# mpieva/mapping-iterative-assembler

Hardware: AMD Instinct MI355X
Metric: reads aligned/sec per iteration (16.5kb mito ref, 100bp reads) (higher is better)
Workload: dtype int32; 1 GPU; configs[1]: 1000000 synthetic 100 bp reads per GPU vs mt311 (16619 bp, circular), matrix flat; step = reiterate_assembly + pop_smp + cull + consensus; pass-1 coordinates = true positions; reads_per_gpu=1000000, total_reads=1000000, consensus_len=16619, bytes_per_read=182

## Files before the change

### mapping-iterative-assembler_amd/csrc/align_route.h

```cpp
#pragma once
#include <stdint.h>

namespace mia {

constexpr int ROUTE_QCH = 8, ROUTE_MAXW = 64;

struct AlignRouteIn {
  int64_t n = 0;
  int max_len = 0, wrap = 0, L = 0;
  int64_t plane_words = 0;
  int64_t kh_entries = 0;
  bool flat = false, ref_mostly_bases = true, ref_few_n = true, bx_ok = false, explicit_win = false, deferred = false, pend_encode = false;
  bool own_umax = false;
  int64_t rejects = 0;
  int use_filter = 1, use_banddp = 1, use_bx = 1, use_lanes = 1, use_fine = 1, use_quick = 1;
  bool bx_serial = false, plan_split = true, use_direct_open = true, no_prep_fuse = false;
  uint32_t ext_events = 31u, dbg = 0, bx_dbg = 0;
};

struct AlignRoute {
  int64_t plane_words = 0;
  int nwords = 0;
  bool bx = false, run_filter = false, fused_prep = false, filtered = false, kocc = false, banded = false;
  bool want_bits = false, new_flow = false, split = false, fork_by_launch = false, fine = false;
  bool many_rejects = false;
  bool planner_head_first = false, direct_open = false;
  int maxw = 0;
  bool quick = false, quick_lds = false, one_launch = false, fork_at_quick = false;
  int qch = 4;
  int quick_phase = 0;
  int full_first = 0, full_last = 0;
  int grid_cap = 0;
  bool three_streams = false, two_streams = false;
  bool values_aside = false;
  bool trace_signals = false;
  bool planner_aside = false;
  bool use_plain = false;
  bool plan_count_late = false;
};

inline unsigned align_route_plan_grid(const AlignRoute& r, int phase, int64_t n) {
  const int64_t g = (n + 255) / 256, cap = (phase == 2 || phase == 3) ? 1024 : r.grid_cap;
  return (unsigned)(cap && g > cap ? cap : g);
}

inline AlignRoute align_route(const AlignRouteIn& in) {
  AlignRoute r;
  const int64_t n = in.n;
  r.nwords = (in.max_len + 63) >> 6;
  r.plane_words = in.plane_words;
  const bool filter_ok = in.flat && in.use_filter && in.ref_mostly_bases;
  r.bx = in.bx_ok && in.use_bx && (in.ref_mostly_bases || in.kh_entries > 0) && in.wrap <= (1 << 22) && !(in.dbg & 128u);
  r.run_filter = filter_ok && !r.bx;
  r.fused_prep = in.pend_encode && r.bx && !in.no_prep_fuse;
  r.filtered = r.run_filter || r.bx;
  r.kocc = r.filtered && in.wrap <= (1 << 22) && !r.bx;
  r.banded = r.bx || (r.filtered && in.use_banddp && r.kocc && !(in.dbg & 128u));
  const bool many = !in.ref_mostly_bases || in.rejects * 20 > n;
  r.many_rejects = r.bx && many;
  r.use_plain = !r.banded || r.many_rejects;
  r.plan_count_late = true;
  if (!r.bx) return r;

  r.want_bits = in.use_quick && (in.kh_entries <= 0 || in.ref_few_n);
  r.new_flow = in.use_lanes && !in.bx_serial && !(in.dbg & 256u) && !in.explicit_win;
  r.split = in.plan_split;
  r.fork_by_launch = (in.ext_events & 1u) && r.new_flow;
  r.fine = r.split && in.use_fine && (in.use_fine > 1 || !in.flat || n >= 4000000 || many);
  r.planner_head_first = r.new_flow && in.deferred && many;
  r.direct_open = r.new_flow && in.deferred && in.use_direct_open && !many && !(in.bx_dbg & (4u | 8u));
  r.maxw = (in.use_lanes && (r.fine || in.use_fine >= 2)) ? ROUTE_MAXW : 32;
  r.quick = r.split && r.new_flow && r.want_bits && !(in.bx_dbg & 32u) && in.own_umax &&
            (!r.fine || n >= 2000000 || in.use_quick > 1);
  r.fork_at_quick = r.quick && r.direct_open && !r.fine;
  r.quick_lds = r.quick && r.plane_words * 24 <= 38 * 1024;
  r.quick_phase = r.quick ? (r.quick_lds ? 5 : 4) : 0;
  r.qch = (r.quick && n >= 4000000 && r.plane_words * 24 <= 16 * 1024) ? ROUTE_QCH : 4;
  r.one_launch = r.quick && !r.fine;
  r.full_first = r.one_launch ? 6 : r.split ? 1 : 0;
  r.full_last = r.one_launch ? 6 : r.split ? (r.fine ? 3 : 2) : 0;
  r.grid_cap = r.one_launch ? 256 : 0;
  r.three_streams = r.new_flow;
  r.two_streams = !r.new_flow && !(in.dbg & 256u);
  r.values_aside = r.three_streams && !(in.deferred && !r.fork_at_quick);
  r.trace_signals = r.three_streams && (in.ext_events & 2u) && !(in.bx_dbg & 8u);
  r.planner_aside = r.three_streams && in.deferred;
  r.plan_count_late = !r.planner_head_first && !r.direct_open;
  return r;
}

}
```

### mapping-iterative-assembler_amd/csrc/mia_hip.hip

```cpp
#include <hip/hip_runtime.h>
#include <atomic>
#include <hip/hip_ext.h>
#include <stdio.h>
#include <stdlib.h>
#include <string.h>

#include <algorithm>
#include <cmath>
#include <chrono>
#include <optional>
#include <string>
#include <thread>
#include <tuple>
#include <vector>

#include "../../include/mia_hip.h"
#include "dev_buf.h"
#include "dev_pool.h"
#include "mia_comm.h"
#include "mia_consensus_kernels.h"
#include "mia_kernels.h"
#include "bandx_kernels.h"
#include "align_route.h"
#include "pass1_route.h"
#include "mia_pass1_kernels.h"
#include "mia_myers_kernels.h"
#include "mia_trim_kernels.h"
#include "mia_peak_kernels.h"
#include "mia_iter_kernels.h"
#include "mia_ma_region_kernels.h"
#include "mia_ma_ace_kernels.h"
#include "mia_ma_sam_kernels.h"
#include "mia_ma_profile_kernels.h"
#include "mia_ma_ends_kernels.h"
#include "mia_ma_cols_kernels.h"
#include "mia_ma_dedup_kernels.h"
#include "mia_ma_damage_kernels.h"
#include "mia_ma_mask_kernels.h"

using namespace mia;

enum Stage { STG_TRACE = 0, STG_PLAIN, STG_FILTER, STG_BAND, STG_BX_PLAN, STG_BX_VALUES, STG_BX_TRACE, STG_TALLY, STG_PASS1, STG_MA_SELECT, STG_MA_RENDER, STG_MA_ACE_LAYOUT, STG_MA_ACE_RENDER, STG_MA_MASK_BOUNDS, STG_MA_MASK_LAYOUT, STG_MA_MASK_APPLY, STG_MA_SAM_LAYOUT, STG_MA_SAM_RENDER, STG_MA_DAMAGE_HITS, STG_MA_DAMAGE_MOLECULES, STG_MA_PROFILE, STG_MA_DEDUP_KEYS, STG_MA_DEDUP_SORT, STG_MA_DEDUP_RUNS, STG_MA_DEDUP_NEXT, STG_MA_DEDUP_ANCHORS, STG_MA_DEDUP_CLUSTERS, STG_MA_TALLY, STG_MA_COLS, STG_MA_ENDS, STG_COUNT };
static const char* const STAGE_NAMES[STG_COUNT] = {"k_align_quad", "k_align_quad_plain", "k_diag_filter", "k_band_align", "k_bx_plan",
                                                   "k_bx_values", "k_bx_trace", "k_tally_binned", "k_pass1", "k_ma_region_select",
                                                   "k_ma_region_render", "k_ma_ace_layout", "k_ma_ace_render", "k_ma_mask_bounds", "k_ma_mask_layout", "k_ma_mask_apply", "k_ma_sam_layout",
                                                   "k_ma_sam_render", "k_ma_damage_hits", "k_ma_damage_molecules", "k_ma_profile", "k_ma_dedup_keys", "k_ma_dedup_sort", "k_ma_dedup_runs",
                                                   "k_ma_dedup_next", "k_ma_dedup_anchors", "k_ma_dedup_clusters", "k_ma_tally", "k_ma_cols", "k_ma_ends"};

constexpr int OPEN_WGS = 1024;
constexpr int64_t OPEN_SLAB_BYTES = (int64_t)MAX_READ * 64 * 12;
constexpr int CTRL_BINS = 0;
constexpr int CTRL_HDR = (3 * N_BINS + 2 + 1) & ~1;
constexpr int CTRL_FILTER = CTRL_HDR + PH_WORDS;
constexpr int CTRL_LKN = CTRL_FILTER + 4, CTRL_CULLF = CTRL_LKN + 1, CTRL_NEV = CTRL_CULLF + 1, CTRL_TFLAGS = CTRL_NEV + 1;
constexpr int CTRL_GENN = CTRL_TFLAGS + 2;
constexpr int CTRL_BXC = (CTRL_GENN + 1 + 63) & ~63;
constexpr int CTRL_WORDS = CTRL_BXC + BXC_WORDS;
constexpr int CTRL_C0 = CTRL_BINS + 3 * N_BINS, CTRL_CN = CTRL_WORDS - CTRL_C0;

#ifdef MIA_HIP_ALT_PATHS
static inline const char* alt_env(const char* name) { return getenv(name); }
#define ALT_KERNEL(k) ((const void*)(k))
#else
static inline const char* alt_env(const char*) { return nullptr; }
#define ALT_KERNEL(k) ((const void*)nullptr)
#endif
static inline std::optional<int> alt_int(const char* name) {
  const char* v = alt_env(name);
  return v ? std::optional<int>(atoi(v)) : std::nullopt;
}

struct mia_hip_ctx {
  int device = 0;
  int cus = 1;
  std::string err;
  DevPool pool;
  unsigned char* h_pin = nullptr; static constexpr size_t PIN_BYTES = 1 << 20, PIN_MISC = 64 << 10;
  DevBuf<int32_t> d_ctrl;
  uint32_t dbg = 0;

  hipStream_t stream = nullptr;
  hipStream_t stream2 = nullptr; hipEvent_t ev_fork = nullptr, ev_join = nullptr;
  hipStream_t stream3 = nullptr; hipEvent_t ev_join3 = nullptr;
  uint32_t ext_events = 31u; bool align_end_signalled = false;
  bool spin_wait = true;
  uint32_t stage_mask = ~0u;
  struct StageTimer { std::vector<std::pair<hipEvent_t, hipEvent_t>> pending; double ms = 0; int64_t launches = 0; };
  StageTimer stg[STG_COUNT];
  std::vector<std::pair<hipEvent_t, hipEvent_t>> ev_free;

  DevBuf<int32_t> d_pssm;
  int max_abs = 0;
  int max_pos = 0;
  bool have_pssm = false;
  bool flat = false;
  PackSet packs;
  ReadSet rs{};
  DevBuf<uint8_t> d_packed; DevBuf<uint32_t> d_roff; DevBuf<uint16_t> d_len;
  DevBuf<uint8_t> d_rc, d_sk;
  DevBuf<int32_t> d_as, d_ae, d_score, d_refstart;
  DevBuf<int16_t> d_abr; DevBuf<uint32_t> d_status; DevBuf<int16_t> d_cols;
  int max_len = 0;
  int min_len = 0;
  std::vector<int32_t> h_len;
  DevBuf<uint64_t> d_rplanes; int rplane_words = 0;
  DevBuf<int32_t> d_umax; bool umax_valid = false;
  DevBuf<uint8_t> d_ref; int L = 0, wrap = 0; int explicit_win = 0; bool have_ref = false; bool aligned = false;
  bool ref_mostly_bases = true;
  bool ref_few_n = true;
  int64_t kh_entries = 0;

  DevBuf<int32_t> d_bin_of, d_list, d_wide_list, d_retry_list;
  int32_t* d_bins = nullptr;
  int32_t* d_plan_hdr = nullptr;
  bool deferred = false;
  DevBuf<unsigned char> d_slabs[N_CPL];
  DevBuf<unsigned char> d_slabs_retry[3];
  DevBuf<unsigned char> d_quad_slabs;
  int quad_wgs = 0;
  int grid_wgs = 0;
  int window_wgs[N_CPL] = {0, 0, 0};
  int64_t plain_retried = 0, plain_total = 0;
  bool wide_to_caller = false;
  DevBuf<int32_t> d_scratch; DevBuf<int64_t> d_scratch_off;
  DevBuf<int32_t> d_open_list; DevBuf<unsigned char> d_slabs_open; bool use_direct_open = true; int64_t direct_open_steps = 0;

  int use_filter = 1;
  DevBuf<int32_t> d_kocc_cnt, d_kocc_pos;
  DevBuf<uint64_t> d_planes;
  uint32_t* d_filter_n = nullptr; int64_t filter_proven = 0, filter_seen = 0;
  int use_banddp = 1;
  DevBuf<int32_t> d_left_list;
  DevBuf<uint32_t> d_band_slabs;
  int64_t band_done = 0;

  bool bx_ok = false;
  int use_bx = 1, use_lanes = 1; bool bx_serial = false; uint32_t bx_dbg = 0;
  DevBuf<int32_t> d_bx_sub, d_bx_mrow; DevBuf<int16_t> d_bx_loss, d_bx_dl;
  int32_t bx_min_m = 0, bx_max_m = 0;
  DevBuf<uint32_t> d_refnib;
  DevBuf<uint32_t> d_khash; DevBuf<int32_t> d_khash_ovf;
  DevBuf<KbPair> d_kbits;
  int use_quick = 1; int64_t quick_steps = 0;
  DevBuf<uint32_t> d_prep_bar; uint32_t prep_bar_count = 0; bool no_prep_fuse = false;
  DevBuf<uint32_t> d_bx_plan; DevBuf<int32_t> d_bx_expect, d_bx_lists;
  DevBuf<BxCandRec> d_bx_cand; bool plan_split = true;
  DevBuf<BxCandRec> d_bx_cand2; int use_fine = 1;
  uint32_t* d_bx_ctr = nullptr;
  DevBuf<uint32_t> d_bx_slabs;
  int bx_values_wgs = 0, bx_trace_wgs = 0;
  DevBuf<uint32_t> d_bx_slabs_late; int bx_late_wgs = 0;
  DevBuf<uint32_t> d_bx_slabs_late2;
  DevBuf<int32_t> d_retry2;
  bool diag_scripts_missing = false;
  int64_t bx_seen = 0, bx_done[3] = {0, 0, 0};
  int64_t bx_launches = 0;
  uint32_t bx_last[BXC_COUNTERS] = {0};

  DevBuf<int64_t> d_slot, d_partial, d_total;
  DevBuf<uint8_t> d_slot_dropped, d_drop_f, d_drop_b; int64_t n_slots = 0;
  DevBuf<int64_t> d_back_slot;
  DevBuf<int64_t> d_front_slot0;
  DevBuf<int32_t> d_link_act;
  RecInfo ri{};
  DevBuf<int32_t> d_ri_flen, d_ri_blen, d_ri_actf, d_ri_trec;
  SlotInfo si{};
  DevBuf<int32_t> d_si_reclen, d_si_recact, d_si_mult; DevBuf<unsigned long long> d_si_writer;
  Links lk{};
  DevBuf<int64_t> d_lk_rec;
  int64_t* d_links_all = nullptr; int32_t n_links_all = 0;
  int32_t* d_n_links_all = nullptr; int64_t links_cap_all = 0; DevBuf<int32_t> d_n_links_gathered;
  DevBuf<int32_t> d_link_len;
  uint32_t* d_cull_flags = nullptr;
  DevBuf<uint32_t> d_cull_sync;
  DevBuf<unsigned long long> d_sums;
  int64_t read_base = 0;
  int64_t slot_base = 0;
  bool culled = false, links_applied = false;
  std::vector<DevBuf<int64_t>> owned_links;
  bool cull_scan = false, tail_scans = false;
  bool cull_with_records = true;
  int64_t pre_cull_records = 0, pre_cull_links = 0; bool pre_cull_valid = false;

  TallyBuf tb{}; DevBuf<int32_t> d_tb_tally, d_ins_off, d_ins_total; DevBuf<uint64_t> d_tb_events;
  DevBuf<int32_t> d_ins_tally; DevBuf<char> d_calls, d_ins_calls;
  int64_t ins_tally_cap = 0;
  int32_t n_events_host = 0; bool tallied = false;
  int64_t ins_total_host = 0;
  bool consensus_done = false;
  bool fake_event_overflow = false;
  bool no_linear_tally = false, sort2_unpacked = false;
  bool tally_linear = false;
  int tally_pk_bias = -1;
  int use_binned_tally = 1;
  DevBuf<int32_t> d_bucket, d_order;
  int bucket_clean_nb = -1;
  int buckets_queued = 0;
  bool no_side_buckets = false;
  DevBuf<int32_t> d_tally_slabs;
  DevBuf<int32_t> d_gen_list;
  bool tally_defer = true;
  bool tally_strand_split = true;
  bool tally_rall = true;
  bool tally_runs = true;
  DevBuf<int32_t> d_order2; DevBuf<uint8_t> d_okey; DevBuf<int32_t> d_sort2;

  bool in_iterate = false;
  const int32_t* abort_if = nullptr;
  bool spec_ok = false, spec_pending = false, spec_filtered = false, spec_bx = false, spec_plain = false;
  int64_t spec_redone = 0;
  bool no_spec = false;
  bool spec_force = false; DevBuf<int32_t> d_one;
  bool pend_encode = false; int32_t pend_L = 0, pend_wl = 0, pend_total = 0;
  bool zero_copy = true;
  const double* dev_cut = nullptr; DevBuf<double> d_cut_buf;
  DevBuf<char> d_ascii; const char* ascii_src = nullptr;
  DevBuf<char> d_cons;
  DevBuf<int32_t> d_cons_pos;
  unsigned char* h_pin2 = nullptr; size_t pin2_bytes = 0;
  int64_t iter_fallbacks = 0;

  double pass1_ms = 0; int64_t pass1_filtered = 0, pass1_anchored = 0;
  double myers_kernel_ms = 0; bool myers_no_lanes = false, myers_no_ond = false;
  int64_t trim_escapes = 0;
  int64_t trim_launches = 0, trim_scratch_bytes = 0;
  bool trim_exact = false;
  bool ma_resident = false; int64_t ma_n = 0, ma_n_ins = 0; int32_t ma_L = 0;
  DevBuf<int32_t> d_ma_start, d_ma_gaps, d_ma_ipos, d_ma_rec_ins, d_ma_ins_list;
  DevBuf<int64_t> d_ma_coff, d_ma_ioff, d_ma_colmap, d_ma_rows;
  DevBuf<char> d_ma_seq, d_ma_ib, d_ma_text;
  DevBuf<unsigned long long> d_ma_ctl;
  struct MaOut {
    bool region_done = false, ace_done = false, sam_done = false, prof_done = false, ends_done = false, cols_done = false, damage_done = false, mask_done = false;
    int32_t first = 0, last = -1; int64_t rows = 0, width = 0, ace_bytes = 0, sam_bytes = 0;
  } ma_out;
  bool ma_ace_gaps_ok = false, ma_ace_cols_ok = false;
  DevBuf<int64_t> d_ace_g, d_ace_af, d_ace_len, d_ace_off; DevBuf<char> d_ace_body;
  bool ma_sam_gaps_ok = false;
  DevBuf<char> d_sam_ref, d_sam_body; DevBuf<int64_t> d_sam_cum, d_sam_cig, d_sam_off; DevBuf<int32_t> d_sam_nm;
  DevBuf<unsigned long long> d_sam_ctl;
  DevBuf<uint8_t> d_ma_rev, d_prof_use; DevBuf<char> d_ma_smp, d_prof_ref; DevBuf<unsigned long long> d_prof_bins;
  int64_t ma_cols = 0; int64_t ma_prof_bins[MA_PROF_BINS] = {0};
  DevBuf<uint8_t> d_ends_seg; DevBuf<unsigned long long> d_ends_bins;
  int64_t ma_ends_bins[MA_ENDS_BINS] = {0};
  DevBuf<uint32_t> d_cols_tab; DevBuf<unsigned long long> d_cols_out;
  std::vector<int32_t> ma_cols_tab;
  struct MaDedup {
    bool done = false; int64_t n = 0, molecules = 0, clusters = 0, orphans = 0;
    DevBuf<int32_t> d_start, d_end, d_score; DevBuf<uint8_t> d_rc, d_keep; DevBuf<int64_t> d_mate, d_rep;
    DevBuf<unsigned long long> d_key[2], d_runkey, d_best, d_ctl, d_hist;
    DevBuf<uint32_t> d_val[2], d_jump[2], d_counts, d_runid, d_first, d_mark, d_cluster, d_anchor;
    int64_t hist[MA_DEDUP_HIST] = {0};
  } dedup;

  struct MaDamage {
    DevBuf<int64_t> d_mate; DevBuf<uint32_t> d_hit; DevBuf<uint8_t> d_pos, d_keep; DevBuf<unsigned long long> d_bins;
    int64_t bins[MA_DMG_BINS] = {0};
  } damage;

  struct MaMask {
    DevBuf<uint32_t> d_lohi; DevBuf<int32_t> d_rec, d_ipos; DevBuf<int64_t> d_off; DevBuf<char> d_seq, d_smp; DevBuf<uint8_t> d_pair_keep;
    DevBuf<unsigned long long> d_ctl, d_bins;
    int64_t bins[MA_MASK_BINS] = {0}, cols_kept = 0; int32_t mode = 0;
  } mask;

  mia_hip_collectives coll{}; bool comm = false; int comm_ranks = 1, comm_rank = 0; std::string coll_name;
  DevBuf<unsigned long long> d_gather;
  std::vector<int64_t> h_gather;
  int64_t ev_pad = 0;
  DevBuf<int64_t> d_lstage, d_lmine, d_lall;
  DevBuf<int32_t> d_scores_all;
};

static void read_alt_switches(mia_hip_ctx* ctx) {
  auto on = [](const char* name) { const char* v = alt_env(name); return v && atoi(v) != 0; };
  if (on("MIA_HIP_NO_DIAG_FILTER")) { ctx->use_filter = 0; ctx->use_bx = 0; }
  if (on("MIA_HIP_NO_BAND_DP")) { ctx->use_banddp = 0; ctx->use_bx = 0; }
  if (on("MIA_HIP_NO_BANDX")) ctx->use_bx = 0;
  if (on("MIA_HIP_NO_LANES")) ctx->use_lanes = 0;
  if (on("MIA_HIP_BX_SERIAL")) ctx->bx_serial = true;
  if (on("MIA_HIP_NO_PLAN_SPLIT")) ctx->plan_split = false;
  if (on("MIA_HIP_NO_FINE")) ctx->use_fine = 0;
  if (const char* v = alt_env("MIA_HIP_FINE")) ctx->use_fine = atoi(v);
  if (on("MIA_HIP_NO_QUICK_PLAN")) ctx->use_quick = 0;
  if (const char* v = alt_env("MIA_HIP_QUICK_PLAN")) ctx->use_quick = atoi(v);
  if (on("MIA_HIP_NO_DIRECT_OPEN")) ctx->use_direct_open = false;
  if (on("MIA_HIP_NO_PREP_FUSE")) ctx->no_prep_fuse = true;
  if (on("MIA_HIP_NO_SPEC")) ctx->no_spec = true;
  if (on("MIA_HIP_SPEC_TEST")) ctx->spec_force = true;
  if (on("MIA_HIP_NO_SIDE_BUCKETS")) ctx->no_side_buckets = true;
  if (on("MIA_HIP_NO_ZERO_COPY")) ctx->zero_copy = false;
  if (on("MIA_HIP_NO_EXT_EVENTS")) ctx->ext_events = 0u;
  if (on("MIA_HIP_FAKE_EVENT_OVERFLOW")) ctx->fake_event_overflow = true;
  if (on("MIA_HIP_CULL_SCAN")) ctx->cull_scan = true;
  if (on("MIA_HIP_TAIL_SCANS")) ctx->tail_scans = true;
  if (on("MIA_HIP_NO_CULL_RECORDS")) ctx->cull_with_records = false;
  if (on("MIA_HIP_NO_BINNED_TALLY")) ctx->use_binned_tally = 0;
  if (on("MIA_HIP_NO_LINEAR_TALLY")) ctx->no_linear_tally = true;
  if (on("MIA_HIP_SORT2_UNPACKED")) ctx->sort2_unpacked = true;
  if (on("MIA_HIP_TALLY_INLINE")) ctx->tally_defer = false;
  if (const char* v = alt_env("MIA_HIP_STRAND_SPLIT")) ctx->tally_strand_split = atoi(v) != 0;
  if (on("MIA_HIP_NO_TALLY_RUNS")) ctx->tally_runs = false;
  if (on("MIA_HIP_NO_TALLY_RALL")) ctx->tally_rall = false;
  if (on("MIA_HIP_MYERS_NO_LANES")) ctx->myers_no_lanes = true;
  if (on("MIA_HIP_MYERS_NO_OND")) ctx->myers_no_ond = true;
  if (on("MIA_HIP_TRIM_EXACT")) ctx->trim_exact = true;
  if (const char* v = alt_env("MIA_HIP_DEBUG_SKIP")) ctx->dbg = (uint32_t)atoi(v);
  if (const char* v = alt_env("MIA_HIP_BX_DEBUG")) ctx->bx_dbg = (uint32_t)atoi(v);
}

#define HIPCHK(call)                                                                                   \
  do {                                                                                                 \
    hipError_t e_ = (call);                                                                            \
    if (e_ != hipSuccess) {                                                                            \
      ctx->err = std::string(#call) + ": " + hipGetErrorString(e_);                                    \
      return MIA_HIP_ERR_DEVICE;                                                                       \
    }                                                                                                  \
  } while (0)

static int dev_nomem(mia_hip_ctx* ctx, hipError_t e) {
  if (e == hipSuccess) return MIA_HIP_OK;
  ctx->err = std::string("hipMalloc: ") + hipGetErrorString(e);
  return MIA_HIP_ERR_NOMEM;
}
template <class T>
static int dev_alloc(mia_hip_ctx* ctx, DevBuf<T>& b, int64_t n) { return dev_nomem(ctx, b.alloc(n)); }
template <class T>
static int dev_ensure(mia_hip_ctx* ctx, DevBuf<T>& b, int64_t need, int64_t alloc_elems) { return dev_nomem(ctx, b.ensure(need, alloc_elems)); }
template <class T>
static int dev_ensure(mia_hip_ctx* ctx, DevBuf<T>& b, int64_t need) { return dev_nomem(ctx, b.ensure(need, need)); }

template <class T>
static int pool_take(mia_hip_ctx* ctx, PoolLease<T>& lease, size_t n) { return dev_nomem(ctx, lease.take(ctx->pool, n)); }

extern "C" const char* mia_hip_last_error(const mia_hip_ctx* ctx) { return ctx ? ctx->err.c_str() : "null context"; }

extern "C" int mia_hip_create(mia_hip_ctx** out, int device_index) {
  if (!out) return MIA_HIP_ERR_ARG;
  *out = nullptr;
  int ndev = 0;
  if (hipGetDeviceCount(&ndev) != hipSuccess || ndev <= 0) return MIA_HIP_ERR_DEVICE;
  if (device_index < 0 || device_index >= ndev) return MIA_HIP_ERR_ARG;
  mia_hip_ctx* ctx = new mia_hip_ctx();
  ctx->device = device_index;
  const unsigned evf = hipEventDisableTiming;
  if (hipSetDevice(device_index) != hipSuccess || hipStreamCreateWithFlags(&ctx->stream, hipStreamNonBlocking) != hipSuccess ||
      hipStreamCreateWithFlags(&ctx->stream2, hipStreamNonBlocking) != hipSuccess || hipStreamCreateWithFlags(&ctx->stream3, hipStreamNonBlocking) != hipSuccess ||
      hipEventCreateWithFlags(&ctx->ev_join3, evf) != hipSuccess ||
      hipEventCreateWithFlags(&ctx->ev_fork, evf) != hipSuccess || hipEventCreateWithFlags(&ctx->ev_join, evf) != hipSuccess) {
    delete ctx;
    return MIA_HIP_ERR_DEVICE;
  }
  {
    hipDeviceProp_t prop;
    if (hipGetDeviceProperties(&prop, device_index) != hipSuccess) { delete ctx; return MIA_HIP_ERR_DEVICE; }
    ctx->cus = prop.multiProcessorCount > 0 ? prop.multiProcessorCount : 1;
    ctx->grid_wgs = prop.multiProcessorCount * 32;
    ctx->quad_wgs = prop.multiProcessorCount * 16;
    read_alt_switches(ctx);
    if (const char* sw = getenv("MIA_HIP_SPIN_WAIT")) ctx->spin_wait = atoi(sw) != 0;
  }
  if (dev_alloc(ctx, ctx->d_pssm, 2 * PSSM_WORDS) || dev_alloc(ctx, ctx->d_ctrl, CTRL_WORDS) ||
      dev_alloc(ctx, ctx->d_total, 1) || dev_alloc(ctx, ctx->d_ins_total, 1) ||
      dev_alloc(ctx, ctx->d_bx_sub, 2 * BX_SUB_WORDS) || dev_alloc(ctx, ctx->d_bx_mrow, 2 * 31 * 4) || dev_alloc(ctx, ctx->d_bx_loss, BX_LOSS_WORDS) ||
      dev_alloc(ctx, ctx->d_bx_dl, BX_DL_WORDS) ||
      dev_alloc(ctx, ctx->d_cut_buf, 2)) {
    delete ctx;
    return MIA_HIP_ERR_NOMEM;
  }
  ctx->d_bins = ctx->d_ctrl + CTRL_BINS;
  ctx->d_plan_hdr = ctx->d_ctrl + CTRL_HDR;
  ctx->d_filter_n = reinterpret_cast<uint32_t*>(ctx->d_ctrl + CTRL_FILTER);
  ctx->lk.n = ctx->d_ctrl + CTRL_LKN;
  ctx->d_cull_flags = reinterpret_cast<uint32_t*>(ctx->d_ctrl + CTRL_CULLF);
  ctx->tb.n_events = ctx->d_ctrl + CTRL_NEV;
  ctx->tb.flags = reinterpret_cast<uint32_t*>(ctx->d_ctrl + CTRL_TFLAGS);
  ctx->d_bx_ctr = reinterpret_cast<uint32_t*>(ctx->d_ctrl + CTRL_BXC);
  if (hipMemset(ctx->d_ctrl, 0, CTRL_WORDS * 4) != hipSuccess) { delete ctx; return MIA_HIP_ERR_DEVICE; }
  {
    const int32_t one = 1;
    if (dev_alloc(ctx, ctx->d_one, 1) || hipMemcpy(ctx->d_one, &one, 4, hipMemcpyHostToDevice) != hipSuccess) { delete ctx; return MIA_HIP_ERR_DEVICE; }
    if (dev_alloc(ctx, ctx->d_prep_bar, 1) || hipMemset(ctx->d_prep_bar, 0, 4) != hipSuccess) { delete ctx; return MIA_HIP_ERR_DEVICE; }
  }
  if (hipHostMalloc((void**)&ctx->h_pin, mia_hip_ctx::PIN_BYTES, hipHostMallocDefault) != hipSuccess) ctx->h_pin = nullptr;
  if (ctx->h_pin) memset(ctx->h_pin, 0, mia_hip_ctx::PIN_MISC);
  else ctx->no_prep_fuse = true;
  *out = ctx;
  return MIA_HIP_OK;
}

extern "C" int mia_hip_comm_destroy(mia_hip_ctx* ctx);
extern "C" void mia_hip_destroy(mia_hip_ctx* ctx) {
  if (!ctx) return;
  (void)hipSetDevice(ctx->device);
  (void)hipStreamSynchronize(ctx->stream);
  (void)mia_hip_comm_destroy(ctx);
  if (ctx->h_pin) (void)hipHostFree(ctx->h_pin);
  if (ctx->h_pin2) (void)hipHostFree(ctx->h_pin2);
  for (auto& e : ctx->ev_free) { (void)hipEventDestroy(e.first); (void)hipEventDestroy(e.second); }
  for (auto& t : ctx->stg) for (auto& e : t.pending) { (void)hipEventDestroy(e.first); (void)hipEventDestroy(e.second); }
  (void)hipStreamDestroy(ctx->stream);
  if (ctx->stream2) (void)hipStreamDestroy(ctx->stream2);
  if (ctx->stream3) (void)hipStreamDestroy(ctx->stream3);
  if (ctx->ev_join3) (void)hipEventDestroy(ctx->ev_join3);
  if (ctx->ev_fork) (void)hipEventDestroy(ctx->ev_fork);
  if (ctx->ev_join) (void)hipEventDestroy(ctx->ev_join);
  delete ctx;
}

extern "C" int mia_hip_sync(mia_hip_ctx* ctx) {
  if (!ctx) return MIA_HIP_ERR_ARG;
  HIPCHK(hipSetDevice(ctx->device));
  HIPCHK(hipStreamSynchronize(ctx->stream));
  return MIA_HIP_OK;
}

extern "C" int mia_hip_set_pssm(mia_hip_ctx* ctx, const int32_t* fwd, const int32_t* rc) {
  if (!ctx || !fwd || !rc) return MIA_HIP_ERR_ARG;
  HIPCHK(hipSetDevice(ctx->device));
  int m = 0;
  for (int i = 0; i < PSSM_WORDS; i++) {
    int a = fwd[i] < 0 ? -fwd[i] : fwd[i], b = rc[i] < 0 ? -rc[i] : rc[i];
    if (a > m) m = a;
    if (b > m) m = b;
  }
  if (m > 32000) { ctx->err = "PSSM entries beyond +-32000 do not fit the int16 substitution table"; return MIA_HIP_ERR_RANGE; }
  ctx->max_abs = m;
  {
    int lo = 0, hi = 0;
    for (int k = 0; k < PSSM_WORDS; k++) { lo = std::min(lo, std::min((int)fwd[k], (int)rc[k])); hi = std::max(hi, std::max((int)fwd[k], (int)rc[k])); }
    ctx->tally_pk_bias = -lo + hi <= 2047 ? -lo : -1;
  }
  ctx->max_pos = 0;
  for (int i = 0; i < PSSM_WORDS; i++) { if (fwd[i] > ctx->max_pos) ctx->max_pos = fwd[i]; if (rc[i] > ctx->max_pos) ctx->max_pos = rc[i]; }
  const int cpls[N_CPL] = {4, 8, 12};
  for (int c = 0; c < N_CPL; c++) ctx->packs.ok[c] = make_pack_params(64 * cpls[c], m, &ctx->packs.p[c]) ? 1 : 0;
  HIPCHK(hipMemcpyAsync(ctx->d_pssm, fwd, PSSM_WORDS * 4, hipMemcpyHostToDevice, ctx->stream));
  HIPCHK(hipMemcpyAsync(ctx->d_pssm + PSSM_WORDS, rc, PSSM_WORDS * 4, hipMemcpyHostToDevice, ctx->stream));
  HIPCHK(hipStreamSynchronize(ctx->stream));
  ctx->have_pssm = true;
  ctx->flat = pssm_is_flat(fwd, rc);
  ctx->tally_linear = true;
  for (int d = 0; d < 2 * PSSM_DEPTH + 1; d++)
    for (int x = 0; x < 4; x++)
      for (int b = 0; b < 5; b++)
        if (fwd[(d * 5 + x) * 5 + b] != fwd[x * 5 + b] || rc[(d * 5 + x) * 5 + b] != fwd[x * 5 + b]) ctx->tally_linear = false;
  if (ctx->no_linear_tally) ctx->tally_linear = false;
  {
    std::vector<int32_t> sub(2 * BX_SUB_WORDS, 0), mrow(2 * 31 * 4, 0);
    std::vector<int16_t> loss(BX_LOSS_WORDS, 0), dl(BX_DL_WORDS, 0);
    ctx->bx_ok = bx_make_tables(fwd, rc, sub.data(), mrow.data(), loss.data(), dl.data(), &ctx->bx_min_m, &ctx->bx_max_m);
    if (ctx->bx_ok) {
      for (int k = 0; k < BX_SUB_WORDS; k++) sub[(size_t)BX_SUB_WORDS + k] = sub[(size_t)k] * 256;
      HIPCHK(hipMemcpyAsync(ctx->d_bx_sub, sub.data(), sub.size() * 4, hipMemcpyHostToDevice, ctx->stream));
      HIPCHK(hipMemcpyAsync(ctx->d_bx_mrow, mrow.data(), mrow.size() * 4, hipMemcpyHostToDevice, ctx->stream));
      HIPCHK(hipMemcpyAsync(ctx->d_bx_loss, loss.data(), loss.size() * 2, hipMemcpyHostToDevice, ctx->stream));
      HIPCHK(hipMemcpyAsync(ctx->d_bx_dl, dl.data(), dl.size() * 2, hipMemcpyHostToDevice, ctx->stream));
      HIPCHK(hipStreamSynchronize(ctx->stream));
    }
    ctx->umax_valid = false;
    if (ctx->bx_ok && ctx->d_umax && ctx->rs.n > 0) {
      hipLaunchKernelGGL(k_bx_umax, dim3((unsigned)((ctx->rs.n + 255) / 256)), dim3(256), 0, ctx->stream, ctx->rs, ctx->d_bx_mrow, ctx->d_umax);
      HIPCHK(hipGetLastError());
      ctx->umax_valid = true;
    }
  }
  return MIA_HIP_OK;
}

static inline uint8_t base_code(char b) {
  switch (b) { case 'A': return 0; case 'C': return 1; case 'G': return 2; case 'T': return 3; default: return 4; }
}

static void pack_reads(int64_t n, const char* bases, const int64_t* offsets, const uint32_t* roff, const uint16_t* len, uint8_t* packed) {
  uint8_t lut[256];
  for (int c = 0; c < 256; c++) lut[c] = base_code((char)c);
  auto range = [&](int64_t lo, int64_t hi) {
    for (int64_t i = lo; i < hi; i++) {
      const unsigned char* s = reinterpret_cast<const unsigned char*>(bases) + offsets[i];
      uint8_t* d = packed + roff[i];
      const int l = len[i];
      int k = 0;
      for (; k + 1 < l; k += 2) d[k >> 1] = (uint8_t)(lut[s[k]] | (lut[s[k + 1]] << 4));
      if (k < l) d[k >> 1] = lut[s[k]];
    }
  };
  int T = (int)std::thread::hardware_concurrency();
  if (const char* e = getenv("MIA_HIP_THREADS")) T = atoi(e);
  T = std::max(1, std::min(std::min(T, 32), (int)(n / 16384) + 1));
  if (T == 1) { range(0, n); return; }
  std::vector<std::thread> th;
  for (int t = 1; t < T; t++) th.emplace_back(range, n * t / T, n * (t + 1) / T);
  range(0, n / T);
  for (auto& x : th) x.join();
}

extern "C" int mia_hip_upload_reads(mia_hip_ctx* ctx, int64_t n, const char* bases, const int64_t* offsets, const uint8_t* rc,
                                    const uint8_t* strand_known, const int32_t* as, const int32_t* ae) {
  if (!ctx || n < 0 || (n > 0 && (!bases || !offsets || !rc || !strand_known || !as || !ae))) return MIA_HIP_ERR_ARG;
  if (n >= (int64_t)1 << 31) { ctx->err = "more than 2^31 reads per context"; return MIA_HIP_ERR_ARG; }
  HIPCHK(hipSetDevice(ctx->device));
  std::vector<uint32_t> roff((size_t)n);
  std::vector<uint16_t> len((size_t)n);
  uint64_t total = 0;
  int max_len = 1;
  for (int64_t i = 0; i < n; i++) {
    int64_t l = offsets[i + 1] - offsets[i];
    if (l < 1 || l > MIA_HIP_MAX_READ) { ctx->err = "read length outside 1..256 (INIT_ALN_SEQ_LEN)"; return MIA_HIP_ERR_ARG; }
    roff[i] = (uint32_t)total;
    len[i] = (uint16_t)l;
    if (l > max_len) max_len = (int)l;
    total += (uint64_t)(((l + 1) / 2 + 3) & ~3);
    if (total >= ((uint64_t)1 << 32)) { ctx->err = "packed read store exceeds 4 GiB per context"; return MIA_HIP_ERR_ARG; }
  }
  std::vector<uint8_t> packed((size_t)total + 8, 0);
  pack_reads(n, bases, offsets, roff.data(), len.data(), packed.data());
  ctx->max_len = max_len;
  ctx->min_len = max_len;
  ctx->h_len.assign(len.begin(), len.end());
  for (int64_t i = 0; i < n; i++) if ((int)len[(size_t)i] < ctx->min_len) ctx->min_len = len[(size_t)i];
  const int stride = (max_len + 3) & ~3;
  int nomem = 0;
  nomem |= dev_alloc(ctx, ctx->d_packed, packed.size());
  nomem |= dev_alloc(ctx, ctx->d_roff, n);
  nomem |= dev_alloc(ctx, ctx->d_len, n);
  nomem |= dev_alloc(ctx, ctx->d_rc, n);
  nomem |= dev_alloc(ctx, ctx->d_sk, n);
  nomem |= dev_alloc(ctx, ctx->d_as, n);
  nomem |= dev_alloc(ctx, ctx->d_ae, n);
  nomem |= dev_alloc(ctx, ctx->d_score, n);
  nomem |= dev_alloc(ctx, ctx->d_refstart, n);
  nomem |= dev_alloc(ctx, ctx->d_abr, n);
  nomem |= dev_alloc(ctx, ctx->d_status, n);
  nomem |= dev_alloc(ctx, ctx->d_cols, n * stride);
  nomem |= dev_alloc(ctx, ctx->d_bin_of, n);
  nomem |= dev_alloc(ctx, ctx->d_umax, n);
  ctx->rplane_words = (max_len + 63) >> 6;
  nomem |= dev_alloc(ctx, ctx->d_rplanes, n * 2 * ctx->rplane_words + 2);
  nomem |= dev_alloc(ctx, ctx->d_list, n + 4 * N_BINS);
  nomem |= dev_alloc(ctx, ctx->d_wide_list, n);
  nomem |= dev_alloc(ctx, ctx->d_retry_list, n);
  nomem |= dev_alloc(ctx, ctx->d_slot, n);
  nomem |= dev_alloc(ctx, ctx->d_partial, (size_t)(n / 256 + n / 4096 + 8));
  nomem |= dev_alloc(ctx, ctx->d_drop_f, n);
  nomem |= dev_alloc(ctx, ctx->d_drop_b, n);
  nomem |= dev_alloc(ctx, ctx->d_slot_dropped, 2 * n + 16);
  ctx->n_slots = ctx->d_slot_dropped.cap;
  nomem |= dev_alloc(ctx, ctx->d_back_slot, n) | dev_alloc(ctx, ctx->d_front_slot0, n);
  nomem |= dev_alloc(ctx, ctx->d_ri_flen, n) | dev_alloc(ctx, ctx->d_ri_blen, n) | dev_alloc(ctx, ctx->d_ri_actf, n) |
         dev_alloc(ctx, ctx->d_ri_trec, n * 16);
  const int64_t slot_cap = 2 * n + 16;
  nomem |= dev_alloc(ctx, ctx->d_si_reclen, slot_cap) | dev_alloc(ctx, ctx->d_si_recact, slot_cap) | dev_alloc(ctx, ctx->d_si_writer, slot_cap) |
         dev_alloc(ctx, ctx->d_si_mult, slot_cap);
  ctx->lk.cap = (int32_t)std::min<int64_t>(n + 16, (int64_t)1 << 20);
  if (ctx->lk.cap > (int32_t)LINK_NONE - 1) ctx->lk.cap = (int32_t)LINK_NONE - 1;
  nomem |= dev_alloc(ctx, ctx->d_lk_rec, (size_t)ctx->lk.cap * 4);
  ctx->ri.flen = ctx->d_ri_flen; ctx->ri.blen = ctx->d_ri_blen; ctx->ri.actf = ctx->d_ri_actf; ctx->ri.trec = ctx->d_ri_trec;
// ... 196 lines not shown
  if (plain_launches) *plain_launches = ctx->stg[STG_PLAIN].launches;
  if (reads_in) *reads_in = ctx->plain_total;
  if (reads_retried) *reads_retried = ctx->plain_retried;
  if (reset) { ctx->stg[STG_PLAIN].ms = 0; ctx->stg[STG_PLAIN].launches = 0; ctx->plain_total = 0; ctx->plain_retried = 0; }
  return MIA_HIP_OK;
}

template <int CPL>
static hipError_t launch_window(mia_hip_ctx* ctx, int ci, const int32_t* list, int count, const int32_t* dev_range = nullptr, hipStream_t on = nullptr,
                                bool own_slabs = false, hipEvent_t stop = nullptr) {
  const int64_t slab = (int64_t)MAX_READ * 64 * CPL;
  if (!ctx->window_wgs[ci]) {
    int occ = 0;
    const int cus = ctx->cus;
    if (hipOccupancyMaxActiveBlocksPerMultiprocessor(&occ, (const void*)k_align_window<CPL>, 64, 0) != hipSuccess || occ < 1) occ = 1;
    const int per_cu = ctx->grid_wgs / cus;
    ctx->window_wgs[ci] = cus * (occ < per_cu ? occ : per_cu);
  }
  int grid = (dev_range || count >= ctx->window_wgs[ci]) ? ctx->window_wgs[ci] : count;
  unsigned char* slabs = nullptr;
  if (own_slabs) {
    grid = std::min(grid, 1024);
    if (!ctx->d_slabs_retry[ci] && dev_alloc(ctx, ctx->d_slabs_retry[ci], slab * 1024)) return hipErrorOutOfMemory;
    slabs = ctx->d_slabs_retry[ci];
  } else {
    if (!ctx->d_slabs[ci] && dev_alloc(ctx, ctx->d_slabs[ci], slab * ctx->grid_wgs)) return hipErrorOutOfMemory;
    slabs = ctx->d_slabs[ci];
  }
  RefInfo ref{ctx->d_ref, ctx->L, ctx->wrap, ctx->explicit_win};
  if (stage_begin(ctx, STG_TRACE, on)) return hipErrorOutOfMemory;
  launch_k(k_align_window<CPL>, dim3(grid), dim3(64), 0, on ? on : ctx->stream, stop, ctx->rs, ref, ctx->d_pssm, ctx->packs.p[ci], list,
           count, slabs, slab, ctx->d_wide_list, ctx->d_bins + 3 * N_BINS, ctx->dbg, dev_range);
  stage_end(ctx, STG_TRACE, on);
  return hipGetLastError();
}

static hipError_t launch_window_class(mia_hip_ctx* ctx, int ci, const int32_t* list, int count, const int32_t* dev_range = nullptr, hipStream_t on = nullptr,
                                      bool own_slabs = false, hipEvent_t stop = nullptr) {
  return ci == 0 ? launch_window<4>(ctx, ci, list, count, dev_range, on, own_slabs, stop)
       : ci == 1 ? launch_window<8>(ctx, ci, list, count, dev_range, on, own_slabs, stop)
                 : launch_window<12>(ctx, ci, list, count, dev_range, on, own_slabs, stop);
}

static int align_all(mia_hip_ctx* ctx);
static bool tally_is_binned(const mia_hip_ctx* ctx);
static int comm_pre_cull_enqueue(mia_hip_ctx* ctx, const int32_t* d_wide_count);
static bool comm_pre_cull_collect(mia_hip_ctx* ctx);

extern "C" int mia_hip_realign(mia_hip_ctx* ctx, const char* new_ref, int32_t ref_len, int circular) {
  if (!ctx || !new_ref || ref_len <= 0) return MIA_HIP_ERR_ARG;
  if (!ctx->have_pssm || !ctx->d_packed) { ctx->err = "set_pssm and upload_reads must precede realign"; return MIA_HIP_ERR_STATE; }
  HIPCHK(hipSetDevice(ctx->device));
  const int L = ref_len, wl = circular ? (L < MAX_READ ? L : MAX_READ) : 0, wrap = L + wl;
  std::vector<uint8_t> codes((size_t)wrap + 64, 4);
  int64_t n_other = 0;
  for (int i = 0; i < L; i++) { codes[i] = base_code(new_ref[i]); n_other += codes[i] > 3; }
  for (int i = 0; i < wl; i++) codes[L + i] = codes[i];
  ctx->ref_mostly_bases = n_other * 50 <= L;
  ctx->ref_few_n = n_other * 500 <= L;
  ctx->kh_entries = 0;
  if (n_other) {
    ctx->kh_entries = kh_wild_entries(codes.data(), wrap, BX_WILD);
    if (ctx->kh_entries > ((int64_t)1 << 24)) ctx->kh_entries = 0;
  }
  if (dev_ensure(ctx, ctx->d_ref, (int64_t)codes.size(), (int64_t)codes.size() * 2)) return MIA_HIP_ERR_NOMEM;
  if (ctx->h_pin && codes.size() <= mia_hip_ctx::PIN_BYTES - mia_hip_ctx::PIN_MISC) {
    HIPCHK(hipStreamSynchronize(ctx->stream));
    memcpy(ctx->h_pin + mia_hip_ctx::PIN_MISC, codes.data(), codes.size());
    HIPCHK(hipMemcpyAsync(ctx->d_ref, ctx->h_pin + mia_hip_ctx::PIN_MISC, codes.size(), hipMemcpyHostToDevice, ctx->stream));
  } else {
    HIPCHK(hipMemcpyAsync(ctx->d_ref, codes.data(), codes.size(), hipMemcpyHostToDevice, ctx->stream));
  }
  ctx->L = L; ctx->wrap = wrap; ctx->have_ref = true; ctx->explicit_win = 0;
  return align_all(ctx);
}

static int run_wide(mia_hip_ctx* ctx, const RefInfo& ref, int32_t n_wide) {
    if (ctx->wide_to_caller) {
      hipLaunchKernelGGL(k_mark_status, dim3((n_wide + 255) / 256), dim3(256), 0, ctx->stream, ctx->d_wide_list, n_wide, ctx->rs.status, ST_ESCAPE);
      HIPCHK(hipGetLastError());
      return MIA_HIP_OK;
    }
    std::vector<int32_t> wl((size_t)n_wide), as((size_t)n_wide), ae((size_t)n_wide);
    std::vector<uint16_t> ln((size_t)n_wide);
    HIPCHK(hipMemcpy(wl.data(), ctx->d_wide_list, (size_t)n_wide * 4, hipMemcpyDeviceToHost));
    std::vector<int64_t> soff((size_t)n_wide);
    int64_t total = 0;
    for (int t = 0; t < n_wide; t++) {
      HIPCHK(hipMemcpy(&as[t], ctx->rs.as + wl[t], 4, hipMemcpyDeviceToHost));
      HIPCHK(hipMemcpy(&ae[t], ctx->rs.ae + wl[t], 4, hipMemcpyDeviceToHost));
      HIPCHK(hipMemcpy(&ln[t], ctx->rs.len + wl[t], 2, hipMemcpyDeviceToHost));
      int s, n1;
      read_window(ref, as[t], ae[t], ln[t], &s, &n1);
      soff[t] = total;
      total += (int64_t)ln[t] * n1 + 5 * (int64_t)n1 + 16;
    }
    if (dev_ensure(ctx, ctx->d_scratch, total) || dev_ensure(ctx, ctx->d_scratch_off, n_wide)) return MIA_HIP_ERR_NOMEM;
    HIPCHK(hipMemcpyAsync(ctx->d_scratch_off, soff.data(), (size_t)n_wide * 8, hipMemcpyHostToDevice, ctx->stream));
    hipLaunchKernelGGL(k_align_wide, dim3((n_wide + 63) / 64), dim3(64), 0, ctx->stream, ctx->rs, ref, ctx->d_pssm, ctx->d_wide_list,
                       n_wide, ctx->d_scratch_off, ctx->d_scratch);
    HIPCHK(hipGetLastError());
    HIPCHK(hipStreamSynchronize(ctx->stream));
  return MIA_HIP_OK;
}

static void encode_now(mia_hip_ctx* ctx) {
  if (!ctx->pend_encode) return;
  ctx->pend_encode = false;
  hipLaunchKernelGGL(k_ref_encode, dim3((unsigned)((ctx->pend_total + 255) / 256)), dim3(256), 0, ctx->stream, ctx->ascii_src, ctx->pend_L, ctx->pend_wl,
                     ctx->d_ref, ctx->pend_total);
}

static void align_counters_collect(mia_hip_ctx* ctx, const int32_t* hb, bool filtered, bool bx, bool plain) {
  constexpr int C0 = CTRL_C0;
  const int32_t* h_hdr = hb + (CTRL_HDR - C0);
  const uint32_t* h_filter = reinterpret_cast<const uint32_t*>(hb + (CTRL_FILTER - C0));
  const uint32_t* h_bxc = reinterpret_cast<const uint32_t*>(hb + (CTRL_BXC - C0));
  ctx->filter_seen += ctx->rs.n;
  if (filtered) {
    ctx->filter_proven += h_filter[0];
    ctx->band_done += h_filter[2];
    if (bx) {
      ctx->filter_proven += h_bxc[BXC_DONE_PLAN * BXC_STRIDE];
      for (int k = 0; k < 3; k++) ctx->bx_done[k] += h_bxc[(BXC_DONE_PLAN + k) * BXC_STRIDE];
      ctx->bx_seen += h_bxc[BXC_SEEN * BXC_STRIDE];
    }
  }
  for (int k = 0; k < BXC_COUNTERS; k++) ctx->bx_last[k] = bx ? h_bxc[k * BXC_STRIDE] : 0;
  if (bx) ctx->bx_last[BXC_CUR_VALUES] = h_filter[1];
  if (plain) ctx->plain_retried += h_hdr[PH_RETRIED_PLAIN];
}

static_assert(ROUTE_QCH == BX_QCH && ROUTE_MAXW == BX_MAXW, "align_route.h carries copies of the two");
static_assert(P1_ROUTE_WILD == BX_WILD, "pass1_route.h carries a copy");

struct AlignCall {
  AlignRoute r;
  RefInfo ref; RefPlanes rp{nullptr, nullptr, nullptr}; KmerOcc ko{nullptr, nullptr}; KmerHash kh{};
  uint32_t kslots = 0; int64_t nib_words = 0;
  BxDev bd; int64_t slab_words = 0;
  int gb = 0;
  int32_t *d_count, *d_off, *d_cursor, *d_wide_count;
  hipStream_t ps = nullptr;
  bool pending_join = false;
  bool planner_end_signalled = false;
  bool dbg_steps = false;
};

static AlignRouteIn align_route_in(const mia_hip_ctx* ctx) {
  AlignRouteIn in;
  in.n = ctx->rs.n; in.max_len = ctx->max_len; in.wrap = ctx->wrap; in.L = ctx->L; in.kh_entries = ctx->kh_entries;
  in.plane_words = plane_words((int64_t)ctx->wrap + 64);
  in.flat = ctx->flat; in.ref_mostly_bases = ctx->ref_mostly_bases; in.ref_few_n = ctx->ref_few_n; in.bx_ok = ctx->bx_ok;
  in.explicit_win = ctx->explicit_win != 0; in.deferred = ctx->deferred; in.pend_encode = ctx->pend_encode;
  in.own_umax = ctx->umax_valid && ctx->rs.roff == ctx->d_roff;
  for (int k = 1; k < BXF_KINDS; k++) in.rejects += ctx->bx_last[BXC_FAIL0 + k];
  in.use_filter = ctx->use_filter; in.use_banddp = ctx->use_banddp; in.use_bx = ctx->use_bx; in.use_lanes = ctx->use_lanes;
  in.use_fine = ctx->use_fine; in.use_quick = ctx->use_quick; in.bx_serial = ctx->bx_serial; in.plan_split = ctx->plan_split;
  in.use_direct_open = ctx->use_direct_open; in.no_prep_fuse = ctx->no_prep_fuse;
  in.ext_events = ctx->ext_events; in.dbg = ctx->dbg; in.bx_dbg = ctx->bx_dbg;
  return in;
}

static void align_ck(mia_hip_ctx* ctx, const AlignCall& c, const char* what) {
  if (!c.dbg_steps) return;
  hipError_t e = hipStreamSynchronize(c.ps);
  fprintf(stderr, "[align_all deferred] %s: %s\n", what, hipGetErrorString(e)); fflush(stderr);
}

static int align_ensure_buffers(mia_hip_ctx* ctx, AlignCall& c) {
  const AlignRoute& r = c.r;
  const int64_t n = ctx->rs.n;
  const int wrap = ctx->wrap;
  if (!r.filtered) return MIA_HIP_OK;
  if (dev_ensure(ctx, ctx->d_planes, r.plane_words * 3)) return MIA_HIP_ERR_NOMEM;
  if (r.kocc && !ctx->d_kocc_cnt && (dev_alloc(ctx, ctx->d_kocc_cnt, DF_KTAB) || dev_alloc(ctx, ctx->d_kocc_pos, (int64_t)DF_KTAB * DF_KCAP)))
    return MIA_HIP_ERR_NOMEM;
  if (((r.run_filter && r.banded) || r.quick) && dev_ensure(ctx, ctx->d_left_list, n)) return MIA_HIP_ERR_NOMEM;
  if (!r.bx) {
    c.slab_words = (int64_t)ctx->max_len * BAND_ROW_WORDS;
    const int64_t words = c.slab_words * std::min<int64_t>((n + 63) / 64, 3072);
    return r.banded ? dev_ensure(ctx, ctx->d_band_slabs, words) : MIA_HIP_OK;
  }
  c.nib_words = bx_nib_words((int64_t)wrap + 64);
  if (dev_ensure(ctx, ctx->d_refnib, c.nib_words, c.nib_words * 2)) return MIA_HIP_ERR_NOMEM;
  c.kslots = kh_slots_for_entries(wrap, ctx->kh_entries);
  if (dev_ensure(ctx, ctx->d_khash, (int64_t)c.kslots * 4) || dev_ensure(ctx, ctx->d_khash_ovf, (int64_t)c.kslots * 2)) return MIA_HIP_ERR_NOMEM;
  if (r.want_bits && !ctx->d_kbits && dev_alloc(ctx, ctx->d_kbits, KB_WORDS)) return MIA_HIP_ERR_NOMEM;
  if (dev_ensure(ctx, ctx->d_bx_plan, n) || dev_ensure(ctx, ctx->d_bx_expect, n) || dev_ensure(ctx, ctx->d_bx_lists, n * 4 * BX_NCLS)) return MIA_HIP_ERR_NOMEM;
  if (!ctx->bx_values_wgs) {
    int occ = 0;
    if (hipOccupancyMaxActiveBlocksPerMultiprocessor(&occ, ctx->use_lanes ? (const void*)k_bxl_values : ALT_KERNEL(k_bx_values), 256, 0) != hipSuccess || occ < 1) occ = 1;
    ctx->bx_values_wgs = ctx->cus * std::min(occ, 4);
    if (hipOccupancyMaxActiveBlocksPerMultiprocessor(&occ, ctx->use_lanes ? (const void*)k_bxl_trace : ALT_KERNEL(k_bx_trace), 256, 0) != hipSuccess || occ < 1) occ = 1;
    ctx->bx_trace_wgs = ctx->cus * std::min(occ, 4);
  }
  c.slab_words = ctx->use_lanes ? (int64_t)((ctx->max_len + 3) & ~3) * BXL_SLAB_ROW_WORDS : (int64_t)ctx->max_len * BX_SLAB_ROW_WORDS;
  const int64_t trace_words = c.slab_words * ctx->bx_trace_wgs * 4;
  if (dev_ensure(ctx, ctx->d_bx_slabs, trace_words)) return MIA_HIP_ERR_NOMEM;
  if (r.new_flow) {
    if (dev_ensure(ctx, ctx->d_retry2, n)) return MIA_HIP_ERR_NOMEM;
    if (!ctx->bx_late_wgs) ctx->bx_late_wgs = ctx->cus;
    const int64_t late_words = (int64_t)((ctx->max_len + 3) & ~3) * BXL_SLAB_ROW_WORDS * ctx->bx_late_wgs * 4;
    if (dev_ensure(ctx, ctx->d_bx_slabs_late, late_words) || dev_ensure(ctx, ctx->d_bx_slabs_late2, late_words)) return MIA_HIP_ERR_NOMEM;
  }
  if (r.split && dev_ensure(ctx, ctx->d_bx_cand, n)) return MIA_HIP_ERR_NOMEM;
  if (r.fine && dev_ensure(ctx, ctx->d_bx_cand2, n)) return MIA_HIP_ERR_NOMEM;
  if (r.direct_open) {
    if (dev_ensure(ctx, ctx->d_open_list, n)) return MIA_HIP_ERR_NOMEM;
    if (!ctx->d_slabs_open && dev_alloc(ctx, ctx->d_slabs_open, OPEN_SLAB_BYTES * OPEN_WGS)) return MIA_HIP_ERR_NOMEM;
  }
  return MIA_HIP_OK;
}

static int align_ref_prep(mia_hip_ctx* ctx, AlignCall& c) {
  const AlignRoute& r = c.r;
  const int wrap = ctx->wrap;
  const int64_t words = r.plane_words, pstride = ctx->d_planes.cap / 3;
  if (!r.fused_prep) {
    encode_now(ctx);
    HIPCHK(hipMemsetAsync(ctx->d_ctrl, 0, (size_t)CTRL_WORDS * 4, ctx->stream));
  }
  if (!r.filtered) return MIA_HIP_OK;
  c.rp = RefPlanes{ctx->d_planes, ctx->d_planes + pstride, ctx->d_planes + 2 * pstride};
  if (!r.fused_prep)
    hipLaunchKernelGGL(k_ref_planes, dim3((unsigned)((words + 3) / 4 < 4096 ? (words + 3) / 4 : 4096)), dim3(256), 0, ctx->stream, ctx->d_ref, (int64_t)wrap + 64, words,
                       ctx->d_planes, ctx->d_planes + pstride, ctx->d_planes + 2 * pstride);
  if (r.kocc) {
    HIPCHK(hipMemsetAsync(ctx->d_kocc_cnt, 0, (size_t)DF_KTAB * 4, ctx->stream));
    hipLaunchKernelGGL(k_kmer_occ, dim3((unsigned)((wrap + 255) / 256)), dim3(256), 0, ctx->stream, ctx->d_ref, (int64_t)wrap, ctx->d_kocc_cnt, ctx->d_kocc_pos, 0);
    c.ko.cnt = ctx->d_kocc_cnt; c.ko.pos = ctx->d_kocc_pos;
  }
  if (!r.bx) return MIA_HIP_OK;
  const int64_t nw = c.nib_words;
  const uint32_t kslots = c.kslots;
  if (!r.fused_prep)
    hipLaunchKernelGGL(k_ref_nibbles, dim3((unsigned)((nw + 255) / 256)), dim3(256), 0, ctx->stream, ctx->d_ref, (int64_t)wrap, nw, ctx->d_refnib);
  c.kh = KmerHash{ctx->d_khash, ctx->d_khash_ovf, kslots - 1, kh_shift_for(kslots), ctx->kh_entries > 0 ? BX_WILD : 0};
  const KmerHash& kh = c.kh;
  if (!r.fused_prep) {
    HIPCHK(hipMemsetAsync(ctx->d_khash, 0xFF, (size_t)kslots * 16, ctx->stream));
    hipLaunchKernelGGL(k_kmer_hash, dim3((unsigned)((wrap + 255) / 256)), dim3(256), 0, ctx->stream, ctx->d_ref, (int64_t)wrap, ctx->d_khash, ctx->d_khash_ovf,
                       kh.mask, kh.shift, kh.wild);
    if (r.want_bits) {
      HIPCHK(hipMemsetAsync(ctx->d_kbits, 0, (size_t)KB_WORDS * sizeof(KbPair), ctx->stream));
      hipLaunchKernelGGL(k_kmer_bits, dim3((unsigned)((ctx->L + 255) / 256)), dim3(256), 0, ctx->stream, ctx->d_ref, (int64_t)wrap, (int64_t)ctx->L, ctx->d_kbits);
    }
    return MIA_HIP_OK;
  }
  RefPrep rp2;
  rp2.ascii = ctx->ascii_src; rp2.L = ctx->pend_L; rp2.wl = ctx->pend_wl; rp2.total = ctx->pend_total; rp2.codes = ctx->d_ref;
  rp2.ctrl = ctx->d_ctrl; rp2.ctrl_words = CTRL_WORDS;
  rp2.kslot = ctx->d_khash; rp2.kovf = ctx->d_khash_ovf; rp2.kslots = kslots; rp2.kmask = kh.mask; rp2.kshift = kh.shift; rp2.kwild = kh.wild;
  rp2.plane_words = words; rp2.plo = ctx->d_planes; rp2.phi = ctx->d_planes + pstride; rp2.pok = ctx->d_planes + 2 * pstride;
  rp2.nib_words = nw; rp2.nib = ctx->d_refnib;
  const int64_t want = ((int64_t)wrap + (kh.wild > 0 ? 63 : 255)) / (kh.wild > 0 ? 64 : 256);
  const unsigned grid = (unsigned)std::max<int64_t>(1, std::min<int64_t>(want, ctx->cus));
  rp2.bar = ctx->d_prep_bar; rp2.bar_target = ctx->prep_bar_count + grid;
  rp2.stuck = ctx->h_pin ? reinterpret_cast<uint32_t*>(ctx->h_pin + (62 << 10)) : nullptr;
  rp2.kbits = r.want_bits ? ctx->d_kbits : nullptr;
  hipLaunchKernelGGL(k_ref_prep, dim3(grid), dim3(256), 0, ctx->stream, rp2);
  HIPCHK(hipGetLastError());
  ctx->prep_bar_count += grid;
  ctx->pend_encode = false;
  return MIA_HIP_OK;
}

static void align_bx_dev(mia_hip_ctx* ctx, AlignCall& c) {
  const AlignRoute& r = c.r;
  BxDev& bd = c.bd;
  bd.tab.sub = ctx->d_bx_sub; bd.tab.mrow = ctx->d_bx_mrow; bd.tab.loss = ctx->d_bx_loss; bd.tab.dl = ctx->d_bx_dl;
  bd.dbg = ctx->bx_dbg & (3u | 32u | 64u | 128u | 512u);
  bd.retry = ctx->d_retry2; bd.retry_n = ctx->d_plan_hdr + PH_RETRY2 + 1;
  bd.listed_mark = r.new_flow ? -5 : 0;
  bd.tab.min_m = ctx->bx_min_m; bd.tab.max_m = ctx->bx_max_m;
  bd.tab.maxw = r.maxw;
  bd.sub256 = ctx->d_bx_sub + BX_SUB_WORDS;
  bd.refnib = ctx->d_refnib;
  bd.umax = (ctx->umax_valid && ctx->rs.roff == ctx->d_roff) ? ctx->d_umax : nullptr;
  bd.rplanes = bd.umax ? ctx->d_rplanes : nullptr;
  bd.rplane_words = ctx->rplane_words;
  bd.plan = ctx->d_bx_plan; bd.expect = ctx->d_bx_expect; bd.lists = ctx->d_bx_lists; bd.list_stride = ctx->d_bx_lists.cap / (4 * BX_NCLS); bd.ctr = ctx->d_bx_ctr;
  bd.cand = r.split ? ctx->d_bx_cand : nullptr; bd.cand_n = ctx->d_bx_ctr + (size_t)BXC_CAND * BXC_STRIDE;
  bd.cand2 = r.fine ? ctx->d_bx_cand2 : nullptr; bd.cand2_n = ctx->d_bx_ctr + (size_t)BXC_CAND2 * BXC_STRIDE;
  bd.open = r.direct_open ? ctx->d_open_list : nullptr; bd.open_n = ctx->d_bx_ctr + (size_t)BXC_OPEN * BXC_STRIDE;
  bd.qlist = r.quick ? ctx->d_left_list : nullptr; bd.qlist_n = ctx->d_filter_n + 1; bd.mark_all = 0; bd.to_late = 0; bd.qch = r.qch;
  bd.kb = KmerBits{r.quick ? ctx->d_kbits : nullptr, ctx->L};
  bd.plane_words = (int32_t)(r.quick_lds ? r.plane_words : 0);
}

using PlanKernel = decltype(&k_bx_plan<1, 0>);
template <int PH>
static PlanKernel plan_kernel_nw(int nwords) {
  switch (nwords) { case 1: return k_bx_plan<1, PH>; case 2: return k_bx_plan<2, PH>; case 3: return k_bx_plan<3, PH>; default: return k_bx_plan<4, PH>; }
}
static PlanKernel plan_kernel(int nwords, int phase) {
  switch (phase) {
    case 0: return plan_kernel_nw<0>(nwords); case 1: return plan_kernel_nw<1>(nwords); case 2: return plan_kernel_nw<2>(nwords); case 3: return plan_kernel_nw<3>(nwords);
    case 4: return plan_kernel_nw<4>(nwords); case 5: return plan_kernel_nw<5>(nwords); default: return plan_kernel_nw<6>(nwords);
  }
}

static int align_plan_launches(mia_hip_ctx* ctx, AlignCall& c) {
  const AlignRoute& r = c.r;
  const int64_t n = ctx->rs.n, wrap = ctx->wrap;
  BxDev& bd = c.bd;
  const dim3 pb(256);
  const uint32_t* in_n = (const uint32_t*)(ctx->d_filter_n + 1);
  ctx->diag_scripts_missing = true;
  if (r.direct_open) ctx->direct_open_steps++;
  if (r.quick) ctx->quick_steps++;
  if (stage_begin(ctx, STG_BX_PLAN)) return MIA_HIP_ERR_NOMEM;
  if (r.quick) {
    const dim3 pg((unsigned)((n + 256 * bd.qch - 1) / (256 * bd.qch)));
    const size_t lds = (size_t)(bx_quick_lds_words(bd.qch) * 8 + (r.quick_phase == 5 ? r.plane_words * 24 : 0));
    launch_k(plan_kernel(r.nwords, r.quick_phase), pg, pb, lds, ctx->stream, (r.fork_at_quick && r.fork_by_launch) ? ctx->ev_fork : nullptr, ctx->rs, c.ref, c.rp, c.kh, wrap, bd,
             (const int32_t*)nullptr, in_n, n, ctx->d_bin_of);
    bd.mark_all = 1;
    if (r.fork_at_quick) {
      if (!r.fork_by_launch) HIPCHK(hipEventRecord(ctx->ev_fork, ctx->stream));
      bd.to_late = 1;
    }
  }
  const int32_t* in_list = r.quick ? ctx->d_left_list : nullptr;
  for (int phase = r.full_first; phase <= r.full_last; phase++) {
    hipEvent_t done = (r.fork_by_launch && phase == r.full_last && !r.planner_head_first && !r.fork_at_quick) ? ctx->ev_fork : nullptr;
    launch_k(plan_kernel(r.nwords, phase), dim3(align_route_plan_grid(r, phase, n)), pb, 0, ctx->stream, done, ctx->rs, c.ref, c.rp, c.kh, wrap, bd, in_list, in_n, n, ctx->d_bin_of);
  }
  bd.to_late = 0;
  stage_end(ctx, STG_BX_PLAN);
  HIPCHK(hipGetLastError());
  if (r.planner_head_first) {
    hipLaunchKernelGGL(k_plan_count, dim3(c.gb), dim3(256), 0, ctx->stream, ctx->rs, c.ref, ctx->packs, 1, 1, 1, ctx->d_bin_of, c.d_count, ctx->d_filter_n);
    hipLaunchKernelGGL(k_plan_scan, dim3(1), dim3(512), 0, ctx->stream, c.d_count, c.d_off, ctx->d_plan_hdr, 0, ctx->d_list);
    launch_k(k_plan_fill, dim3(c.gb), dim3(256), 0, ctx->stream, r.fork_by_launch ? ctx->ev_fork : nullptr, n, (const int32_t*)ctx->d_bin_of, (const int32_t*)c.d_off, c.d_cursor, ctx->d_list);
    HIPCHK(hipGetLastError());
  }
  return MIA_HIP_OK;
}

static int align_band_dps(mia_hip_ctx* ctx, AlignCall& c) {
  const AlignRoute& r = c.r;
  const BxDev& bd = c.bd;
  hipStream_t vs = r.values_aside ? ctx->stream2 : ctx->stream;
  if (r.fork_at_quick) {
    if (stage_launch(ctx, STG_BX_VALUES, k_bxl_trace_late2, dim3((unsigned)ctx->bx_late_wgs), dim3(256), 0, ctx->stream, ctx->rs, c.ref, bd, ctx->d_bx_slabs_late2, c.slab_words, ctx->d_bin_of))
      return MIA_HIP_ERR_NOMEM;
  }
  if (!r.fork_by_launch && !r.fork_at_quick) HIPCHK(hipEventRecord(ctx->ev_fork, ctx->stream));
  HIPCHK(hipStreamWaitEvent(ctx->stream2, ctx->ev_fork, 0));
  HIPCHK(hipStreamWaitEvent(ctx->stream3, ctx->ev_fork, 0));
  if (stage_begin(ctx, STG_BX_TRACE, ctx->stream3)) return MIA_HIP_ERR_NOMEM;
  if (!(ctx->bx_dbg & 8u))
    launch_k(k_bxl_trace, dim3((unsigned)ctx->bx_trace_wgs), dim3(256), 0, ctx->stream3, r.trace_signals ? ctx->ev_join3 : nullptr, ctx->rs, c.ref, bd, ctx->d_bx_slabs, c.slab_words, ctx->d_bin_of);
  stage_end(ctx, STG_BX_TRACE, ctx->stream3);
  if (!r.trace_signals) HIPCHK(hipEventRecord(ctx->ev_join3, ctx->stream3));
  if (!(ctx->bx_dbg & 4u)) {
    if (stage_launch(ctx, STG_BX_VALUES, k_bxl_values, dim3((unsigned)ctx->bx_values_wgs), dim3(256), 0, vs, ctx->rs, c.ref, bd, ctx->d_bin_of)) return MIA_HIP_ERR_NOMEM;
    if (stage_launch(ctx, STG_BX_VALUES, k_bxl_trace_late, dim3((unsigned)ctx->bx_late_wgs), dim3(256), 0, vs, ctx->rs, c.ref, bd, ctx->d_bx_slabs_late, c.slab_words, ctx->d_bin_of))
      return MIA_HIP_ERR_NOMEM;
  }
  if (r.values_aside) HIPCHK(hipEventRecord(ctx->ev_join, ctx->stream2));
  HIPCHK(hipGetLastError());
  c.pending_join = true;
  return MIA_HIP_OK;
}

static int align_band_dps_serial(mia_hip_ctx* ctx, AlignCall& c) {
  const BxDev& bd = c.bd;
  HIPCHK(hipEventRecord(ctx->ev_fork, ctx->stream));
  HIPCHK(hipStreamWaitEvent(ctx->stream2, ctx->ev_fork, 0));
  if (stage_begin(ctx, STG_BX_TRACE, ctx->stream2)) return MIA_HIP_ERR_NOMEM;
  if (ctx->bx_dbg & 8u) {}
  else if (ctx->use_lanes) hipLaunchKernelGGL(k_bxl_trace, dim3((unsigned)ctx->bx_trace_wgs), dim3(256), 0, ctx->stream2, ctx->rs, c.ref, bd, ctx->d_bx_slabs, c.slab_words, ctx->d_bin_of);
#ifdef MIA_HIP_ALT_PATHS
  else hipLaunchKernelGGL(k_bx_trace, dim3((unsigned)ctx->bx_trace_wgs), dim3(256), 0, ctx->stream2, ctx->rs, c.ref, bd, ctx->d_bx_slabs, c.slab_words, ctx->d_bin_of);
#endif
  stage_end(ctx, STG_BX_TRACE, ctx->stream2);
  HIPCHK(hipEventRecord(ctx->ev_join, ctx->stream2));
  if (stage_begin(ctx, STG_BX_VALUES)) return MIA_HIP_ERR_NOMEM;
  if (ctx->bx_dbg & 4u) {}
  else if (ctx->use_lanes) hipLaunchKernelGGL(k_bxl_values, dim3((unsigned)ctx->bx_values_wgs), dim3(256), 0, ctx->stream, ctx->rs, c.ref, bd, ctx->d_bin_of);
#ifdef MIA_HIP_ALT_PATHS
  else hipLaunchKernelGGL(k_bx_values, dim3((unsigned)ctx->bx_values_wgs), dim3(256), 0, ctx->stream, ctx->rs, c.ref, bd, ctx->d_bin_of);
#endif
  stage_end(ctx, STG_BX_VALUES);
  HIPCHK(hipStreamWaitEvent(ctx->stream, ctx->ev_join, 0));
  HIPCHK(hipGetLastError());
  return MIA_HIP_OK;
}

static int align_round1(mia_hip_ctx* ctx, AlignCall& c) {
  const AlignRoute& r = c.r;
  const int64_t n = ctx->rs.n, wrap = ctx->wrap;
  if (r.run_filter) {
    if (stage_begin(ctx, STG_FILTER)) return MIA_HIP_ERR_NOMEM;
    hipLaunchKernelGGL(k_diag_filter, dim3((unsigned)((n + 255) / 256)), dim3(256), 0, ctx->stream, ctx->rs, c.ref, c.rp, c.ko, wrap, ctx->d_bin_of, ctx->dbg,
                       r.banded ? ctx->d_left_list : nullptr, ctx->d_filter_n + 1);
    stage_end(ctx, STG_FILTER);
    HIPCHK(hipGetLastError());
  }
  if (!r.banded) return MIA_HIP_OK;
  const int grid = (int)std::min<int64_t>((n + 63) / 64, 3072);
  if (stage_begin(ctx, STG_BAND)) return MIA_HIP_ERR_NOMEM;
  hipLaunchKernelGGL(k_band_align, dim3(grid), dim3(64), 0, ctx->stream, ctx->rs, c.ref, c.rp, c.ko, wrap, ctx->d_left_list, ctx->d_filter_n + 1,
                     ctx->d_band_slabs, c.slab_words, ctx->d_bin_of, ctx->d_filter_n + 2, ctx->d_filter_n + 3, ctx->dbg);
  stage_end(ctx, STG_BAND);
  HIPCHK(hipGetLastError());
  return MIA_HIP_OK;
}

static int bx_join_and_retry(mia_hip_ctx* ctx, AlignCall& c) {
  if (!c.pending_join) return MIA_HIP_OK;
  c.pending_join = false;
  const int32_t* range = ctx->d_plan_hdr + PH_RETRY2;
  const int cols = ctx->max_len + 2 * REALIGN_BUFFER + 2;
  const bool aside = c.r.planner_aside;
  if (c.r.values_aside) HIPCHK(hipStreamWaitEvent(ctx->stream, ctx->ev_join, 0));
  HIPCHK(hipStreamWaitEvent(ctx->stream, ctx->ev_join3, 0));
  hipEvent_t stop = (aside && (ctx->ext_events & 8u)) ? ctx->ev_fork : nullptr;
  ctx->align_end_signalled = stop != nullptr;
  if (c.r.direct_open) {
    if (stage_begin(ctx, STG_TRACE)) return MIA_HIP_ERR_NOMEM;
    launch_k(k_align_open, dim3(OPEN_WGS), dim3(64), 0, ctx->stream, stop, ctx->rs, c.ref, (const int32_t*)ctx->d_pssm, ctx->packs, (const int32_t*)ctx->d_open_list,
             (const uint32_t*)(ctx->d_bx_ctr + (size_t)BXC_OPEN * BXC_STRIDE), ctx->d_slabs_open, (int64_t)OPEN_SLAB_BYTES, ctx->d_wide_list, c.d_wide_count, ctx->dbg,
             (const int32_t*)ctx->d_retry2, (const uint32_t*)(range + 1));
    stage_end(ctx, STG_TRACE);
    hipError_t e = hipGetLastError();
    if (e != hipSuccess) { ctx->err = std::string("k_align_open launch: ") + hipGetErrorString(e); return MIA_HIP_ERR_DEVICE; }
    return MIA_HIP_OK;
  }
  hipError_t e = launch_window_class(ctx, cols <= 64 * 4 ? 0 : cols <= 64 * 8 ? 1 : 2, ctx->d_retry2, 0, range, nullptr, aside, stop);
  if (e != hipSuccess) { ctx->err = std::string("k_align_window (band retry list) launch: ") + hipGetErrorString(e); return MIA_HIP_ERR_DEVICE; }
  if (aside) {
    if (!c.planner_end_signalled) HIPCHK(hipEventRecord(ctx->ev_join, ctx->stream2));
    HIPCHK(hipStreamWaitEvent(ctx->stream, ctx->ev_join, 0));
  }
  return MIA_HIP_OK;
}

static int align_window_classes(mia_hip_ctx* ctx, AlignCall& c) {
  for (int ci = 0; ci < N_CPL; ci++) {
    hipError_t e = launch_window_class(ctx, ci, ctx->d_list, 0, ctx->d_plan_hdr + PH_WIN + 2 * ci, c.ps);
    if (e != hipSuccess) { ctx->err = std::string("k_align_window launch: ") + hipGetErrorString(e); return MIA_HIP_ERR_DEVICE; }
  }
  align_ck(ctx, c, "window classes");
  return MIA_HIP_OK;
}

static int align_planner_deferred(mia_hip_ctx* ctx, AlignCall& c) {
  const AlignRoute& r = c.r;
  const int64_t n = ctx->rs.n;
  hipStream_t ps = c.ps;
  int32_t* hdr = ctx->d_plan_hdr;
  align_ck(ctx, c, "plan_count");
  if (r.direct_open) return MIA_HIP_OK;
  if (!r.planner_head_first) {
    hipLaunchKernelGGL(k_plan_scan, dim3(1), dim3(512), 0, ps, c.d_count, c.d_off, hdr, 0, ctx->d_list);
    hipLaunchKernelGGL(k_plan_fill, dim3(c.gb), dim3(256), 0, ps, n, ctx->d_bin_of, c.d_off, c.d_cursor, ctx->d_list);
  }
  align_ck(ctx, c, "memsets");
  hipLaunchKernelGGL(k_wide_seed, dim3(1), dim3(256), 0, ps, ctx->d_list, hdr, ctx->d_wide_list, c.d_wide_count,
                     r.use_plain ? c.d_count : (int32_t*)nullptr, c.d_cursor);
  align_ck(ctx, c, "scan fill seed");
  const size_t quad_lds = (size_t)Q_G * q_sub_bytes(ctx->max_len) + 16;
  if (r.use_plain) {
    if (stage_begin(ctx, STG_PLAIN, ps)) return MIA_HIP_ERR_NOMEM;
    hipLaunchKernelGGL(k_align_quad_plain, dim3(ctx->quad_wgs), dim3(64), quad_lds, ps, ctx->rs, c.ref, ctx->d_pssm, ctx->d_list, 0, ctx->d_bin_of,
                       (const int32_t*)(hdr + PH_QUAD));
    stage_end(ctx, STG_PLAIN, ps);
    align_ck(ctx, c, "quad plain");
    if (int rcw = align_window_classes(ctx, c)) return rcw;
    hipLaunchKernelGGL(k_plan_recount, dim3(c.gb), dim3(256), 0, ps, n, ctx->d_bin_of, c.d_count);
    hipLaunchKernelGGL(k_plan_scan, dim3(1), dim3(512), 0, ps, c.d_count, c.d_off, hdr, 1, ctx->d_list);
    hipLaunchKernelGGL(k_plan_fill, dim3(c.gb), dim3(256), 0, ps, n, ctx->d_bin_of, c.d_off, c.d_cursor, ctx->d_list);
    align_ck(ctx, c, "replan");
  }
  const int64_t slab = (int64_t)Q_G * MAX_READ * Q_TRACE_STRIDE;
  if (!ctx->d_quad_slabs && dev_alloc(ctx, ctx->d_quad_slabs, slab * ctx->quad_wgs)) return MIA_HIP_ERR_NOMEM;
  if (c.dbg_steps) {
    int32_t hh[PH_WORDS];
    (void)hipMemcpy(hh, hdr, sizeof hh, hipMemcpyDeviceToHost);
    fprintf(stderr, "[align_all deferred] hdr:");
    for (int k = 0; k < PH_WORDS; k++) fprintf(stderr, " %d", hh[k]);
    fprintf(stderr, "  n=%lld max_len=%d quad_lds=%zu\n", (long long)n, ctx->max_len, quad_lds);
  }
  if (stage_begin(ctx, STG_TRACE, ps)) return MIA_HIP_ERR_NOMEM;
  hipLaunchKernelGGL(k_align_quad, dim3(ctx->quad_wgs), dim3(64), quad_lds, ps, ctx->rs, c.ref, ctx->d_pssm, ctx->packs.p[0], ctx->d_list, 0,
                     ctx->d_quad_slabs, slab, ctx->d_wide_list, c.d_wide_count, ctx->d_retry_list, hdr + PH_RETRY + 1, 1, ctx->dbg,
                     (const int32_t*)(hdr + PH_QUAD));
  stage_end(ctx, STG_TRACE, ps);
  HIPCHK(hipGetLastError());
  align_ck(ctx, c, "quad trace");
  if (!r.use_plain) { if (int rcw = align_window_classes(ctx, c)) return rcw; }
  const bool sig = r.planner_aside && c.pending_join && (ctx->ext_events & 4u);
  hipError_t e = launch_window_class(ctx, 0, ctx->d_retry_list, 0, hdr + PH_RETRY, ps, false, sig ? ctx->ev_join : nullptr);
  c.planner_end_signalled = sig && e == hipSuccess;
  if (e != hipSuccess) { ctx->err = std::string("k_align_window retry launch: ") + hipGetErrorString(e); return MIA_HIP_ERR_DEVICE; }
  return MIA_HIP_OK;
}

static int align_close(mia_hip_ctx* ctx) {
  ctx->aligned = true; ctx->culled = false; ctx->tallied = false; ctx->pre_cull_valid = false;
  return MIA_HIP_OK;
}

static int align_finish_deferred(mia_hip_ctx* ctx, AlignCall& c) {
  const AlignRoute& r = c.r;
  align_ck(ctx, c, "retry");
  if (int rcj = bx_join_and_retry(ctx, c)) return rcj;
  align_ck(ctx, c, "band join");
  constexpr int C0 = CTRL_C0, CN = CTRL_CN;
  std::vector<int32_t> pageable;
  int32_t* hb;
  if (ctx->h_pin) hb = reinterpret_cast<int32_t*>(ctx->h_pin);
  else { pageable.resize(CN); hb = pageable.data(); }
  const bool pre_cull = ctx->in_iterate && ctx->comm;
  if (pre_cull) { if (int rcp = comm_pre_cull_enqueue(ctx, c.d_wide_count)) return rcp; }
  const bool spec = ctx->spec_ok && ctx->h_pin && !pre_cull && !c.dbg_steps;
  if (!(spec && ctx->zero_copy)) HIPCHK(hipMemcpyAsync(hb, ctx->d_ctrl + C0, (size_t)CN * 4, hipMemcpyDeviceToHost, ctx->stream));
  if (spec) {
    ctx->spec_pending = true; ctx->spec_filtered = r.filtered; ctx->spec_bx = r.bx; ctx->spec_plain = r.use_plain;
    ctx->abort_if = ctx->spec_force ? ctx->d_one : c.d_wide_count;
    return align_close(ctx);
  }
  HIPCHK(hipStreamSynchronize(ctx->stream));
  align_counters_collect(ctx, hb, r.filtered, r.bx, r.use_plain);
  const int32_t n_wide = hb[0];
  if (n_wide > 0) { if (int rcw = run_wide(ctx, c.ref, n_wide)) return rcw; }
  if (pre_cull && comm_pre_cull_collect(ctx)) {
    if (int rcp = comm_pre_cull_enqueue(ctx, nullptr)) return rcp;
    HIPCHK(hipStreamSynchronize(ctx->stream));
    (void)comm_pre_cull_collect(ctx);
  }
  return align_close(ctx);
}

struct HostPlan {
  int32_t local_buf[4 * N_BINS + 16];
  int32_t *h_count, *h_off, *h_count2, *h_off2, *h_misc;
  std::vector<uint32_t> bxc_pageable;
  uint32_t* h_bxc;
  bool bx_counters_later = false;
  int n_quads = 0, quad_begin = 0;
  bool wide_known = false;
};

static void host_take_bx_counters(mia_hip_ctx* ctx, const HostPlan& h) {
  ctx->filter_proven += h.h_bxc[BXC_DONE_PLAN * BXC_STRIDE];
  for (int k = 0; k < 3; k++) ctx->bx_done[k] += h.h_bxc[(BXC_DONE_PLAN + k) * BXC_STRIDE];
  ctx->bx_seen += h.h_bxc[BXC_SEEN * BXC_STRIDE];
  for (int k = 0; k < BXC_COUNTERS; k++) ctx->bx_last[k] = h.h_bxc[k * BXC_STRIDE];
}

static int align_planner_host_fill(mia_hip_ctx* ctx, AlignCall& c, HostPlan& h) {
  const AlignRoute& r = c.r;
  const int64_t n = ctx->rs.n;
  int32_t* hb = ctx->h_pin ? reinterpret_cast<int32_t*>(ctx->h_pin) : h.local_buf;
  h.h_count = hb; h.h_off = hb + N_BINS; h.h_count2 = hb + 2 * N_BINS; h.h_off2 = hb + 3 * N_BINS; h.h_misc = hb + 4 * N_BINS;
  int32_t *h_count = h.h_count, *h_off = h.h_off, *h_misc = h.h_misc;
  h_misc[0] = 0;
  h_misc[6] = 0;
  if (ctx->h_pin) h.h_bxc = reinterpret_cast<uint32_t*>(ctx->h_pin + (24 << 10));
  else { h.bxc_pageable.resize(BXC_WORDS); h.h_bxc = h.bxc_pageable.data(); }
  for (int k = 0; k < BXC_COUNTERS; k++) h.h_bxc[k * BXC_STRIDE] = 0;
  if (r.filtered) {
    HIPCHK(hipMemcpyAsync(&h_misc[0], ctx->d_filter_n, 4, hipMemcpyDeviceToHost, ctx->stream));
    HIPCHK(hipMemcpyAsync(&h_misc[6], ctx->d_filter_n + 2, 4, hipMemcpyDeviceToHost, ctx->stream));
    if (r.bx) HIPCHK(hipMemcpyAsync(h.h_bxc, ctx->d_bx_ctr, BXC_WORDS * 4, hipMemcpyDeviceToHost, ctx->stream));
  }
  HIPCHK(hipMemcpyAsync(h_count, c.d_count, (size_t)N_BINS * 4, hipMemcpyDeviceToHost, ctx->stream));
  HIPCHK(hipStreamSynchronize(ctx->stream));
  ctx->filter_proven += (uint32_t)h_misc[0];
  ctx->band_done += (uint32_t)h_misc[6];
  ctx->filter_seen += n;
  h.bx_counters_later = c.pending_join;
  if (!h.bx_counters_later) host_take_bx_counters(ctx, h);
  int run = 0;
  for (int b = 0; b < N_BINS; b++) {
    h_off[b] = run;
    run += b >= BIN_QUAD0 ? ((h_count[b] + 3) & ~3) : h_count[b];
  }
  h.quad_begin = h_off[BIN_QUAD0]; h.n_quads = (run - h.quad_begin) / 4;
  if (h.n_quads > 0) HIPCHK(hipMemsetAsync(ctx->d_list + h.quad_begin, 0xFF, (size_t)(run - h.quad_begin) * 4, ctx->stream));
  HIPCHK(hipMemcpyAsync(c.d_off, h_off, (size_t)N_BINS * 4, hipMemcpyHostToDevice, ctx->stream));
  hipLaunchKernelGGL(k_plan_fill, dim3(c.gb), dim3(256), 0, ctx->stream, n, ctx->d_bin_of, c.d_off, c.d_cursor, ctx->d_list);
  const int n_wide0 = h_count[BIN_WIDE];
  if (n_wide0 > 0) {
    HIPCHK(hipMemcpyAsync(ctx->d_wide_list, ctx->d_list + h_off[BIN_WIDE], (size_t)n_wide0 * 4, hipMemcpyDeviceToDevice, ctx->stream));
    HIPCHK(hipMemcpyAsync(c.d_wide_count, &h_count[BIN_WIDE], 4, hipMemcpyHostToDevice, ctx->stream));
  }
  for (int ci = 0; ci < N_CPL; ci++) {
    if (h_count[ci] == 0) continue;
    hipError_t e = launch_window_class(ctx, ci, ctx->d_list + h_off[ci], h_count[ci]);
    if (e != hipSuccess) { ctx->err = std::string("k_align_window launch: ") + hipGetErrorString(e); return MIA_HIP_ERR_DEVICE; }
  }
  return MIA_HIP_OK;
}

static int align_planner_host_plain(mia_hip_ctx* ctx, AlignCall& c, HostPlan& h) {
  const int64_t n = ctx->rs.n;
  if (h.n_quads > 0) {
    const int grid = h.n_quads < ctx->quad_wgs ? h.n_quads : ctx->quad_wgs;
    const size_t quad_lds = (size_t)Q_G * q_sub_bytes(ctx->max_len) + 16;
    if (stage_begin(ctx, STG_PLAIN)) return MIA_HIP_ERR_NOMEM;
    hipLaunchKernelGGL(k_align_quad_plain, dim3(grid), dim3(64), quad_lds, ctx->stream, ctx->rs, c.ref, ctx->d_pssm, ctx->d_list + h.quad_begin,
                       h.n_quads, ctx->d_bin_of, (const int32_t*)nullptr);
    stage_end(ctx, STG_PLAIN);
    HIPCHK(hipGetLastError());
  }
  HIPCHK(hipMemsetAsync(c.d_count, 0, (size_t)N_BINS * 4, ctx->stream));
  HIPCHK(hipMemsetAsync(c.d_cursor, 0, (size_t)N_BINS * 4, ctx->stream));
  hipLaunchKernelGGL(k_plan_recount, dim3(c.gb), dim3(256), 0, ctx->stream, n, ctx->d_bin_of, c.d_count);
  HIPCHK(hipMemcpyAsync(h.h_count2, c.d_count, (size_t)N_BINS * 4, hipMemcpyDeviceToHost, ctx->stream));
  HIPCHK(hipStreamSynchronize(ctx->stream));
  int run2 = 0;
  for (int b = 0; b < N_BINS; b++) { h.h_off2[b] = run2; run2 += b >= BIN_QUAD0 ? ((h.h_count2[b] + 3) & ~3) : 0; }
  ctx->plain_total += (int64_t)h.n_quads * 4;
  for (int b = BIN_QUAD0; b < N_BINS; b++) ctx->plain_retried += h.h_count2[b];
  h.n_quads = run2 / 4;
  h.quad_begin = 0;
  if (h.n_quads > 0) {
    HIPCHK(hipMemsetAsync(ctx->d_list, 0xFF, (size_t)run2 * 4, ctx->stream));
    HIPCHK(hipMemcpyAsync(c.d_off, h.h_off2, (size_t)N_BINS * 4, hipMemcpyHostToDevice, ctx->stream));
    hipLaunchKernelGGL(k_plan_fill, dim3(c.gb), dim3(256), 0, ctx->stream, n, ctx->d_bin_of, c.d_off, c.d_cursor, ctx->d_list);
  }
  return MIA_HIP_OK;
}

static int align_planner_host_trace(mia_hip_ctx* ctx, AlignCall& c, HostPlan& h) {
  const int64_t slab = (int64_t)Q_G * MAX_READ * Q_TRACE_STRIDE;
  const int grid = h.n_quads < ctx->quad_wgs ? h.n_quads : ctx->quad_wgs;
  if (!ctx->d_quad_slabs && dev_alloc(ctx, ctx->d_quad_slabs, slab * ctx->quad_wgs)) return MIA_HIP_ERR_NOMEM;
  const size_t quad_lds = (size_t)Q_G * q_sub_bytes(ctx->max_len) + 16;
  if (stage_begin(ctx, STG_TRACE)) return MIA_HIP_ERR_NOMEM;
  hipLaunchKernelGGL(k_align_quad, dim3(grid), dim3(64), quad_lds, ctx->stream, ctx->rs, c.ref, ctx->d_pssm, ctx->packs.p[0], ctx->d_list + h.quad_begin,
                     h.n_quads, ctx->d_quad_slabs, slab, ctx->d_wide_list, c.d_wide_count, ctx->d_retry_list, c.d_wide_count + 1, 1,
                     ctx->dbg, (const int32_t*)nullptr);
  stage_end(ctx, STG_TRACE);
  HIPCHK(hipGetLastError());
  HIPCHK(hipMemcpyAsync(&h.h_misc[2], c.d_wide_count, 8, hipMemcpyDeviceToHost, ctx->stream));
  HIPCHK(hipStreamSynchronize(ctx->stream));
  const int32_t n_retry = h.h_misc[3];
  if (n_retry > 0) {
    hipError_t e = launch_window_class(ctx, 0, ctx->d_retry_list, n_retry);
    if (e != hipSuccess) { ctx->err = std::string("k_align_window retry launch: ") + hipGetErrorString(e); return MIA_HIP_ERR_DEVICE; }
  } else {
    h.wide_known = true;
  }
  return MIA_HIP_OK;
}

static int align_planner_host(mia_hip_ctx* ctx, AlignCall& c) {
  const AlignRoute& r = c.r;
  HostPlan h;
  if (int rc = align_planner_host_fill(ctx, c, h)) return rc;
  if ((h.n_quads > 0 || r.filtered) && r.use_plain) { if (int rc = align_planner_host_plain(ctx, c, h)) return rc; }
  if (h.n_quads > 0) { if (int rc = align_planner_host_trace(ctx, c, h)) return rc; }
  if (c.pending_join) { if (int rcj = bx_join_and_retry(ctx, c)) return rcj; h.wide_known = false; }
  if (!h.wide_known) {
    HIPCHK(hipMemcpyAsync(&h.h_misc[2], c.d_wide_count, 4, hipMemcpyDeviceToHost, ctx->stream));
    if (h.bx_counters_later) HIPCHK(hipMemcpyAsync(h.h_bxc, ctx->d_bx_ctr, BXC_WORDS * 4, hipMemcpyDeviceToHost, ctx->stream));
    HIPCHK(hipStreamSynchronize(ctx->stream));
    if (h.bx_counters_later) host_take_bx_counters(ctx, h);
  }
  const int32_t n_wide = h.h_misc[2];
  if (n_wide > 0) { if (int rcw = run_wide(ctx, c.ref, n_wide)) return rcw; }
  return align_close(ctx);
}

static int align_all(mia_hip_ctx* ctx) {
  const int64_t n = ctx->rs.n;
  if (!ctx->spec_ok) { ctx->spec_pending = false; ctx->abort_if = nullptr; }
  ctx->align_end_signalled = false;
  ctx->buckets_queued = 0;
  if (n == 0) { ctx->aligned = true; return MIA_HIP_OK; }
  AlignCall c;
  c.r = align_route(align_route_in(ctx));
  const AlignRoute& r = c.r;
  c.ref = RefInfo{ctx->d_ref, ctx->L, ctx->wrap, ctx->explicit_win};
  c.d_count = ctx->d_bins; c.d_off = ctx->d_bins + N_BINS; c.d_cursor = ctx->d_bins + 2 * N_BINS; c.d_wide_count = ctx->d_bins + 3 * N_BINS;
  c.gb = (int)((n + (int64_t)256 * PLAN_PER - 1) / ((int64_t)256 * PLAN_PER));
  c.dbg_steps = ctx->deferred && alt_env("MIA_HIP_ITER_DEBUG") != nullptr;
  if (int rc = align_ensure_buffers(ctx, c)) return rc;
  if (int rc = align_ref_prep(ctx, c)) return rc;
  if (r.bx) {
    align_bx_dev(ctx, c);
    if (int rc = align_plan_launches(ctx, c)) return rc;
    if (r.three_streams) { if (int rc = align_band_dps(ctx, c)) return rc; }
    else if (r.two_streams) { if (int rc = align_band_dps_serial(ctx, c)) return rc; }
    ctx->bx_launches++;
  } else if (r.filtered) {
    if (int rc = align_round1(ctx, c)) return rc;
  }
  c.ps = r.planner_aside ? ctx->stream2 : ctx->stream;
  if (r.plan_count_late)
    hipLaunchKernelGGL(k_plan_count, dim3(c.gb), dim3(256), 0, c.ps, ctx->rs, c.ref, ctx->packs, 1, (int)r.filtered, (int)(r.filtered && r.use_plain), ctx->d_bin_of,
                       c.d_count, ctx->d_filter_n);
  if (!ctx->deferred) return align_planner_host(ctx, c);
  if (int rc = align_planner_deferred(ctx, c)) return rc;
  return align_finish_deferred(ctx, c);
}

extern "C" int mia_hip_align_windows(mia_hip_ctx* ctx, const char* ref, int64_t ref_len, const int64_t* win_start, const int32_t* win_len) {
  if (!ctx || !ref || !win_start || !win_len || ref_len <= 0) return MIA_HIP_ERR_ARG;
  if (!ctx->have_pssm || !ctx->d_packed) { ctx->err = "set_pssm and upload_reads must precede align_windows"; return MIA_HIP_ERR_STATE; }
  if (ref_len > INT32_MAX - 128) { ctx->err = "align_windows: the reference string must stay below 2^31 characters"; return MIA_HIP_ERR_ARG; }
  HIPCHK(hipSetDevice(ctx->device));
  const int64_t n = ctx->rs.n;
  std::vector<int32_t> as((size_t)n), ae((size_t)n);
  for (int64_t i = 0; i < n; i++) {
    if (win_len[i] <= 0 || win_start[i] < 0 || win_start[i] + win_len[i] > ref_len) {
      ctx->err = "align_windows: window " + std::to_string(i) + " is empty or leaves the reference string";
      return MIA_HIP_ERR_ARG;
    }
    as[(size_t)i] = (int32_t)win_start[i];
    ae[(size_t)i] = (int32_t)(win_start[i] + win_len[i] - 1);
  }
  std::vector<uint8_t> codes((size_t)ref_len + 64, 4);
  for (int64_t i = 0; i < ref_len; i++) codes[(size_t)i] = base_code(ref[i]);
  if (dev_ensure(ctx, ctx->d_ref, (int64_t)codes.size())) return MIA_HIP_ERR_NOMEM;
  HIPCHK(hipMemcpyAsync(ctx->d_ref, codes.data(), codes.size(), hipMemcpyHostToDevice, ctx->stream));
  if (n) {
    HIPCHK(hipMemcpyAsync(ctx->d_as, as.data(), (size_t)n * 4, hipMemcpyHostToDevice, ctx->stream));
    HIPCHK(hipMemcpyAsync(ctx->d_ae, ae.data(), (size_t)n * 4, hipMemcpyHostToDevice, ctx->stream));
  }
  ctx->L = (int)ref_len; ctx->wrap = (int)ref_len; ctx->have_ref = false; ctx->explicit_win = 1; ctx->ref_mostly_bases = true; ctx->kh_entries = 0;
  const int rcode = align_all(ctx);
  HIPCHK(hipStreamSynchronize(ctx->stream));
  return rcode;
}

extern "C" int mia_hip_get_alignments(mia_hip_ctx* ctx, int32_t* score, int32_t* as, int32_t* ae) {
  if (!ctx) return MIA_HIP_ERR_ARG;
  if (!ctx->aligned) { ctx->err = "realign first"; return MIA_HIP_ERR_STATE; }
  HIPCHK(hipSetDevice(ctx->device));
  const size_t n = (size_t)ctx->rs.n;
  if (score) HIPCHK(hipMemcpyAsync(score, ctx->d_score, n * 4, hipMemcpyDeviceToHost, ctx->stream));
  if (as) HIPCHK(hipMemcpyAsync(as, ctx->d_as, n * 4, hipMemcpyDeviceToHost, ctx->stream));
  if (ae) HIPCHK(hipMemcpyAsync(ae, ctx->d_ae, n * 4, hipMemcpyDeviceToHost, ctx->stream));
  HIPCHK(hipStreamSynchronize(ctx->stream));
  return MIA_HIP_OK;
}

extern "C" int mia_hip_get_scripts(mia_hip_ctx* ctx, int16_t* cols, int32_t stride, int32_t* ref_start) {
  if (!ctx || (cols && stride < ctx->max_len)) return MIA_HIP_ERR_ARG;
  if (!ctx->aligned) { ctx->err = "realign first"; return MIA_HIP_ERR_STATE; }
  HIPCHK(hipSetDevice(ctx->device));
  const size_t n = (size_t)ctx->rs.n;
  if (cols) {
    if (ctx->diag_scripts_missing && n > 0) {
      hipLaunchKernelGGL(k_diag_scripts, dim3((unsigned)((n + 255) / 256)), dim3(256), 0, ctx->stream, ctx->rs);
      HIPCHK(hipGetLastError());
      ctx->diag_scripts_missing = false;
    }
    HIPCHK(hipMemcpy2DAsync(cols, (size_t)stride * 2, ctx->d_cols, (size_t)ctx->rs.stride * 2, (size_t)ctx->max_len * 2, n,
                            hipMemcpyDeviceToHost, ctx->stream));
  }
  if (ref_start) HIPCHK(hipMemcpyAsync(ref_start, ctx->d_refstart, n * 4, hipMemcpyDeviceToHost, ctx->stream));
  HIPCHK(hipStreamSynchronize(ctx->stream));
  return MIA_HIP_OK;
}

static int finish_params(mia_hip_ctx* ctx);
static int finish_cull(mia_hip_ctx* ctx) {
  const int64_t nl = ctx->links_cap_all;
  if (dev_ensure(ctx, ctx->d_link_len, nl, nl + 64) || dev_ensure(ctx, ctx->d_link_act, nl, nl + 64)) return MIA_HIP_ERR_NOMEM;
  hipLaunchKernelGGL(k_links_apply, dim3(32), dim3(256), 0, ctx->stream, ctx->d_links_all, ctx->d_n_links_all, (int32_t)ctx->links_cap_all, ctx->si,
                     ctx->d_slot_dropped, ctx->n_slots, ctx->d_link_len, ctx->d_link_act, ctx->d_cull_flags, ctx->abort_if);
  ctx->links_applied = true;
  return finish_params(ctx);
}

static int finish_params(mia_hip_ctx* ctx) {
  const int64_t n = ctx->rs.n;
  hipLaunchKernelGGL(k_rec_params, dim3((int)((n + 255) / 256)), dim3(256), 0, ctx->stream, ctx->rs, ctx->L, ctx->d_slot, ctx->d_slot_dropped,
                     ctx->n_slots, ctx->d_back_slot, ctx->ri, ctx->si, ctx->d_links_all, ctx->d_link_len, ctx->d_link_act, ctx->d_n_links_all,
                     (int32_t)ctx->links_cap_all, ctx->read_base, ctx->d_drop_f, ctx->d_drop_b, ctx->d_cull_flags, ctx->abort_if,
                     (ctx->umax_valid && ctx->rs.roff == ctx->d_roff && ctx->d_rplanes && ctx->d_umax) ? ctx->d_umax : (const int32_t*)nullptr,
                     (ctx->cull_with_records && ctx->d_n_links_all == ctx->lk.n) ? 1 : 0);
  HIPCHK(hipGetLastError());
  return MIA_HIP_OK;
}

static int check_cull_flags(mia_hip_ctx* ctx, uint32_t fl) {
  if (fl & 8u) { ctx->err = "more formerly split reads than the link list holds"; return MIA_HIP_ERR_RANGE; }
  if (fl & 4u) {
    ctx->err = "a formerly split read points at an AlnSeq slot that holds no record of this iteration (the reference would show "
               "the slot's content from an earlier iteration); not reproduced";
    return MIA_HIP_ERR_RANGE;
  }
  return MIA_HIP_OK;
}

extern "C" int mia_hip_cull(mia_hip_ctx* ctx, int32_t hard_cut, double slope, double intercept, int64_t slot_base) {
  if (!ctx) return MIA_HIP_ERR_ARG;
  if (!ctx->aligned) { ctx->err = "realign first"; return MIA_HIP_ERR_STATE; }
  if (ctx->explicit_win) { ctx->err = "the last alignment ran on caller-supplied windows (align_windows): realign first"; return MIA_HIP_ERR_STATE; }
  HIPCHK(hipSetDevice(ctx->device));
  const int64_t n = ctx->rs.n;
  if (n == 0) return MIA_HIP_OK;
  const int nb = (int)((n + 255) / 256);
  if (!ctx->d_cull_sync) {
    if (dev_alloc(ctx, ctx->d_cull_sync, 4)) return MIA_HIP_ERR_NOMEM;
    HIPCHK(hipMemsetAsync(ctx->d_cull_sync, 0, 16, ctx->stream));
  }
  hipLaunchKernelGGL(k_slot_count, dim3((unsigned)((n + 4095) / 4096)), dim3(256), 0, ctx->stream, ctx->rs, ctx->L, ctx->d_partial, nb, slot_base, ctx->d_total, (uint32_t*)nullptr, ctx->abort_if);
  if (ctx->cull_scan) hipLaunchKernelGGL(k_scan_partials, dim3(1), dim3(256), 0, ctx->stream, ctx->d_partial, nb, slot_base, ctx->d_total, ctx->abort_if);
  if (slot_base + 2 * n + 16 > ctx->n_slots) {
    DevBuf<uint8_t> nd;
    const int64_t ns = slot_base + 2 * n + 16;
    if (dev_alloc(ctx, nd, ns)) return MIA_HIP_ERR_NOMEM;
    HIPCHK(hipMemsetAsync(nd, 0, (size_t)ns, ctx->stream));
    HIPCHK(hipMemcpyAsync(nd, ctx->d_slot_dropped, (size_t)ctx->n_slots, hipMemcpyDeviceToDevice, ctx->stream));
    HIPCHK(hipStreamSynchronize(ctx->stream));
    ctx->d_slot_dropped = std::move(nd);
    ctx->n_slots = ns;
  }
  ctx->slot_base = slot_base;
  ctx->si.base = slot_base;
  ctx->si.n_local_p = ctx->d_total;
  if (!ctx->in_iterate) HIPCHK(hipMemsetAsync(ctx->lk.n, 0, 8, ctx->stream));
  hipLaunchKernelGGL(k_cull_records, dim3((unsigned)nb), dim3(256), 0, ctx->stream, ctx->rs, ctx->L, (const int64_t*)ctx->d_partial, ctx->d_slot, ctx->ri, ctx->si,
                     ctx->read_base, ctx->d_cull_flags, ctx->d_slot_dropped, ctx->n_slots, hard_cut, slope, intercept, ctx->d_back_slot,
                     (const int64_t*)ctx->d_front_slot0, ctx->lk, ctx->dev_cut, ctx->abort_if, ctx->cull_scan ? 0 : nb, slot_base, ctx->d_total,
                     ctx->cull_with_records ? 1 : 0, ctx->d_drop_f, ctx->d_drop_b,
                     (ctx->umax_valid && ctx->rs.roff == ctx->d_roff && ctx->d_rplanes && ctx->d_umax) ? ctx->d_umax : (const int32_t*)nullptr);
  HIPCHK(hipGetLastError());
  ctx->d_links_all = ctx->lk.rec;
  ctx->d_n_links_all = ctx->lk.n;
  ctx->links_cap_all = ctx->lk.cap;
  ctx->culled = true;
// ... 174 lines not shown
  const int64_t n = ctx->rs.n;
  if (n > 0) {
    int grid = (int)std::min<int64_t>((n + 255) / 256, (int64_t)ctx->cus);
    hipLaunchKernelGGL(k_score_sums, dim3(grid), dim3(256), 0, ctx->stream, ctx->rs, ctx->d_sums, ctx->L, ctx->d_back_slot, ctx->d_front_slot0);
    HIPCHK(hipGetLastError());
  }
  int64_t local7[7];
  int64_t* stage = ctx->h_pin ? reinterpret_cast<int64_t*>(ctx->h_pin + (16 << 10)) : local7;
  HIPCHK(hipMemcpyAsync(stage, ctx->d_sums, 56, hipMemcpyDeviceToHost, ctx->stream));
  HIPCHK(hipStreamSynchronize(ctx->stream));
  memcpy(sums5, stage, 40);
  ctx->pre_cull_records = stage[5];
  ctx->pre_cull_links = stage[6];
  ctx->pre_cull_valid = true;
  return MIA_HIP_OK;
}

extern "C" int mia_hip_pre_cull_counts(mia_hip_ctx* ctx, int64_t* n_records, int64_t* n_links) {
  if (!ctx) return MIA_HIP_ERR_ARG;
  if (!ctx->pre_cull_valid) { ctx->err = "score_sums (after the last realign) first"; return MIA_HIP_ERR_STATE; }
  if (n_records) *n_records = ctx->pre_cull_records;
  if (n_links) *n_links = ctx->pre_cull_links;
  return MIA_HIP_OK;
}

extern "C" int mia_hip_score_cut_from_sums(const int64_t* sums5, double* slope, double* intercept) {
  const int64_t sx = sums5[0], sy = sums5[1], j = sums5[2];
  if (!(j > 0 && sums5[3] == sums5[4])) return 1;
  double xbar = (double)sx, ybar = (double)sy;
  xbar /= (double)(size_t)j;
  ybar /= (double)(size_t)j;
  const double zero = 0.0;
  const double slope_bf = zero / zero;
  const double intercept_bf = ybar - slope_bf * xbar;
  const double max_delta = 0;
  *intercept = intercept_bf;
  if ((slope_bf - max_delta) > 0) *slope = slope_bf - (max_delta * 2.0);
  else *slope = (double)(slope_bf * (80 / 100.0));
  return 0;
}

extern "C" int mia_hip_num_records(mia_hip_ctx* ctx, int64_t* n_records) {
  if (!ctx || !n_records) return MIA_HIP_ERR_ARG;
  if (!ctx->aligned) { ctx->err = "realign first"; return MIA_HIP_ERR_STATE; }
  HIPCHK(hipSetDevice(ctx->device));
  const int64_t n = ctx->rs.n;
  *n_records = 0;
  if (n == 0) return MIA_HIP_OK;
  const int nb = (int)((n + 4095) / 4096);
  hipLaunchKernelGGL(k_scan_blocks, dim3(nb), dim3(256), 0, ctx->stream, ctx->rs, ctx->L, ctx->d_partial);
  hipLaunchKernelGGL(k_scan_partials, dim3(1), dim3(256), 0, ctx->stream, ctx->d_partial, nb, (int64_t)0, ctx->d_total);
  HIPCHK(hipMemcpyAsync(n_records, ctx->d_total, 8, hipMemcpyDeviceToHost, ctx->stream));
  HIPCHK(hipStreamSynchronize(ctx->stream));
  return MIA_HIP_OK;
}

static int ensure_events(mia_hip_ctx* ctx, int64_t elems) {
  const int rc = dev_alloc(ctx, ctx->d_tb_events, elems);
  ctx->tb.events = ctx->d_tb_events;
  ctx->tb.cap_events = (int32_t)std::min<int64_t>(ctx->d_tb_events.cap, INT32_MAX);
  return rc;
}

static int ensure_tally(mia_hip_ctx* ctx) {
  const int Lp = ctx->L + 1;
  int rc = dev_ensure(ctx, ctx->d_tb_tally, (int64_t)(TALLY_WORDS + 1) * Lp + 256);
  rc |= dev_ensure(ctx, ctx->d_ins_off, Lp);
  rc |= dev_ensure(ctx, ctx->d_calls, Lp);
  if (rc) return MIA_HIP_ERR_NOMEM;
  if (!ctx->tb.events && ensure_events(ctx, std::min<int64_t>(ctx->rs.n * 32 + 4096, (int64_t)1 << 30))) return MIA_HIP_ERR_NOMEM;
  ctx->tb.tally = ctx->d_tb_tally;
  ctx->tb.Lp = Lp;
  ctx->tb.gaps = ctx->tb.tally + (size_t)TALLY_WORDS * Lp;
  return MIA_HIP_OK;
}

static bool tally_rall(const mia_hip_ctx* ctx) { return ctx->max_len > 128 && ctx->max_len <= 256 && ctx->tally_runs && ctx->tally_rall; }
static int tally_split(const mia_hip_ctx* ctx) {
  return (!ctx->tally_linear && ctx->tally_strand_split && (ctx->max_len <= 128 || tally_rall(ctx))) ? 1 : 0;
}
static int tally_nb(const mia_hip_ctx* ctx) { return (ctx->wrap / TALLY_BUCKET + 1) << tally_split(ctx); }
static bool tally_is_binned(const mia_hip_ctx* ctx) {
  const int nb = ctx->wrap / TALLY_BUCKET + 1;
  return ctx->rs.n > 0 && ctx->use_binned_tally && nb <= 4096 && ctx->max_abs <= 32767;
}
static int tally_chunk(const mia_hip_ctx* ctx) { return ctx->tally_linear ? TALLY_CHUNK_LINEAR : TALLY_CHUNK; }
static int bucket_launch(mia_hip_ctx* ctx, hipStream_t on) {
  int rc = ensure_tally(ctx);
  if (rc) return rc;
  const int Lp = ctx->tb.Lp;
  const int64_t tally_words = (int64_t)(TALLY_WORDS + 1) * Lp + 256;
  const int64_t n = ctx->rs.n;
  const int nb = tally_nb(ctx), split = tally_split(ctx);
  const int chunk = tally_chunk(ctx);
  const int grid = (int)(n / chunk) + nb + 1;
  if (4 * (nb + 1) + 4 * grid > ctx->d_bucket.cap) {
    if (dev_alloc(ctx, ctx->d_bucket, (int64_t)(4 * (nb + 1) + 4 * grid) * 2)) return MIA_HIP_ERR_NOMEM;
    ctx->bucket_clean_nb = -1;
  }
  if (!ctx->d_order && dev_alloc(ctx, ctx->d_order, n)) return MIA_HIP_ERR_NOMEM;
  int32_t *d_cnt = ctx->d_bucket, *d_off = d_cnt + (nb + 1), *d_wgoff = d_off + (nb + 1), *d_cur = d_wgoff + (nb + 1), *d_wgb = d_cur + (nb + 1);
  if (ctx->bucket_clean_nb != nb) { HIPCHK(hipMemsetAsync(d_cnt, 0, (size_t)(nb + 1) * 4, on)); ctx->bucket_clean_nb = nb; }
  const int gb = (int)((n + 256 * BUCKET_PER - 1) / (256 * BUCKET_PER));
  hipLaunchKernelGGL(k_bucket_count, dim3(gb), dim3(256), (size_t)nb * 4, on, ctx->rs, nb, d_cnt, ctx->tb.tally, tally_words, ctx->abort_if, split);
  hipLaunchKernelGGL(k_bucket_scan, dim3(1), dim3(256), 0, on, d_cnt, nb, d_off, d_wgoff, d_cur, d_wgb, ctx->abort_if, chunk);
  const bool sigb = on != ctx->stream && (ctx->ext_events & 16u);
  if (!split) launch_k(k_bucket_fill, dim3(gb), dim3(256), (size_t)nb * 8, on, sigb ? ctx->ev_join : nullptr, ctx->rs, nb, d_off, d_cur, ctx->d_order, ctx->abort_if, split, (uint8_t*)nullptr, 0);
  else {
    const int64_t words2 = (int64_t)nb * SORT2_KEYS * 2;
    if (dev_ensure(ctx, ctx->d_sort2, words2)) return MIA_HIP_ERR_NOMEM;
    if (!ctx->d_order2 && dev_alloc(ctx, ctx->d_order2, n)) return MIA_HIP_ERR_NOMEM;
    if (!ctx->d_okey && dev_alloc(ctx, ctx->d_okey, n + 64)) return MIA_HIP_ERR_NOMEM;
    HIPCHK(hipMemsetAsync(ctx->d_sort2, 0, (size_t)words2 * 4, on));
    const int32_t packed = (n < (1 << 24) && !ctx->sort2_unpacked) ? 1 : 0;
    hipLaunchKernelGGL(k_bucket_fill, dim3(gb), dim3(256), (size_t)nb * 8, on, ctx->rs, nb, (const int32_t*)d_off, d_cur, ctx->d_order, ctx->abort_if, split, ctx->d_okey, packed);
    hipLaunchKernelGGL(k_sort2_count, dim3(grid), dim3(256), 0, on, nb, (const int32_t*)d_wgoff, (const int32_t*)d_wgb, (const int32_t*)ctx->d_order, (const uint8_t*)ctx->d_okey, packed,
                       ctx->d_sort2, ctx->abort_if);
    launch_k(k_sort2_fill, dim3(grid), dim3(256), 0, on, sigb ? ctx->ev_join : nullptr, nb, (const int32_t*)d_off, (const int32_t*)d_wgoff, (const int32_t*)d_wgb,
             (const int32_t*)ctx->d_order, (const uint8_t*)ctx->d_okey, packed, (const int32_t*)ctx->d_sort2, ctx->d_sort2 + (int64_t)nb * SORT2_KEYS, ctx->d_order2, ctx->abort_if);
  }
  HIPCHK(hipGetLastError());
  if (on != ctx->stream && !sigb) HIPCHK(hipEventRecord(ctx->ev_join, on));
  ctx->buckets_queued = on != ctx->stream ? 2 : 1;
  return MIA_HIP_OK;
}

static int tally_launch(mia_hip_ctx* ctx) {
  if (!ctx->aligned) { ctx->err = "realign first"; return MIA_HIP_ERR_STATE; }
  if (!ctx->culled) { ctx->err = "cull first (the dropped bits and record parameters are its output)"; return MIA_HIP_ERR_STATE; }
  HIPCHK(hipSetDevice(ctx->device));
  int rc = ensure_tally(ctx);
  if (rc) return rc;
  const int Lp = ctx->tb.Lp;
  const int64_t tally_words = (int64_t)(TALLY_WORDS + 1) * Lp + 256;
  if (!ctx->in_iterate) HIPCHK(hipMemsetAsync(ctx->tb.n_events, 0, 8, ctx->stream));
  const int64_t n = ctx->rs.n;
  const bool binned = tally_is_binned(ctx);
  if (!binned) HIPCHK(hipMemsetAsync(ctx->tb.tally, 0, (size_t)tally_words * 4, ctx->stream));
  if (n > 0) {
    RefInfo ref{ctx->d_ref, ctx->L, ctx->wrap};
    const int nb = tally_nb(ctx), split = tally_split(ctx);
    if (binned) {
      if (!ctx->buckets_queued) { if (int rcb = bucket_launch(ctx, ctx->stream)) return rcb; }
      if (ctx->buckets_queued == 2) HIPCHK(hipStreamWaitEvent(ctx->stream, ctx->ev_join, 0));
      ctx->buckets_queued = 0;
      const int chunk = tally_chunk(ctx);
      const int grid = (int)(n / chunk) + nb + 1;
      int32_t *d_cnt = ctx->d_bucket, *d_off = d_cnt + (nb + 1), *d_wgoff = d_off + (nb + 1), *d_cur = d_wgoff + (nb + 1), *d_wgb = d_cur + (nb + 1);
      const int64_t slab_words = (int64_t)grid * (TALLY_WORDS - 1) * TALLY_WIN;
      if (dev_ensure(ctx, ctx->d_tally_slabs, slab_words)) return MIA_HIP_ERR_NOMEM;
      const bool planes_ok = ctx->umax_valid && ctx->rs.roff == ctx->d_roff && ctx->d_rplanes && ctx->d_umax;
      const bool defer = ctx->tally_defer;
      if (defer && dev_ensure(ctx, ctx->d_gen_list, n)) return MIA_HIP_ERR_NOMEM;
      int32_t* n_gen = ctx->d_ctrl + CTRL_GENN;
      if (defer && !ctx->in_iterate) HIPCHK(hipMemsetAsync(n_gen, 0, 4, ctx->stream));
#define MIA_TALLY_ARGS(PL, RW, UM, BIAS)                                                                                                              \
  dim3(grid), dim3(256), 0, ctx->stream, ctx->rs, ref, ctx->d_pssm, ctx->d_drop_f, ctx->d_drop_b, ctx->tb, nb, d_off, d_wgoff, split ? ctx->d_order2 : ctx->d_order, ctx->ri.trec, \
      ctx->ri.actf, ctx->d_tally_slabs, ctx->dbg, PL, RW, UM, d_wgb, BIAS, ctx->abort_if, chunk, defer ? ctx->d_gen_list : (int32_t*)nullptr, n_gen, split | ((split && ctx->tally_runs) ? 2 : 0)
      const uint64_t* pl_arg = planes_ok ? ctx->d_rplanes : nullptr;
      const int32_t* um_arg = planes_ok ? ctx->d_umax : nullptr;
      int rct;
      if (ctx->tally_linear)
        rct = defer ? stage_launch(ctx, STG_TALLY, k_tally_binned<true, true>, MIA_TALLY_ARGS(pl_arg, ctx->rplane_words, um_arg, -1))
                    : stage_launch(ctx, STG_TALLY, k_tally_binned<true, false>, MIA_TALLY_ARGS(pl_arg, ctx->rplane_words, um_arg, -1));
      else if (split && tally_rall(ctx))
        rct = defer ? stage_launch(ctx, STG_TALLY, k_tally_binned<false, true, true>, MIA_TALLY_ARGS(pl_arg, ctx->rplane_words, um_arg, ctx->tally_pk_bias))
                    : stage_launch(ctx, STG_TALLY, k_tally_binned<false, false, true>, MIA_TALLY_ARGS(pl_arg, ctx->rplane_words, um_arg, ctx->tally_pk_bias));
      else
        rct = defer ? stage_launch(ctx, STG_TALLY, k_tally_binned<false, true>, MIA_TALLY_ARGS(split ? pl_arg : nullptr, ctx->rplane_words, split ? um_arg : nullptr, ctx->tally_pk_bias))
                    : stage_launch(ctx, STG_TALLY, k_tally_binned<false, false>, MIA_TALLY_ARGS(split ? pl_arg : nullptr, ctx->rplane_words, split ? um_arg : nullptr, ctx->tally_pk_bias));
#undef MIA_TALLY_ARGS
      if (rct) return MIA_HIP_ERR_NOMEM;
      GenReads gen{ctx->rs, ref, ctx->d_pssm, ctx->d_drop_f, ctx->d_drop_b, ctx->ri.trec, ctx->ri.actf, defer ? ctx->d_gen_list : nullptr, n_gen};
      hipLaunchKernelGGL(k_tally_reduce, dim3((Lp + 255) / 256 + (defer ? TALLY_GEN_BLOCKS : 0), TALLY_WORDS - 1, TALLY_REDUCE_SHARES), dim3(256), 0, ctx->stream, ctx->tb, nb, d_wgoff,
                         ctx->d_tally_slabs, ctx->abort_if, gen, split);
    } else {
      hipLaunchKernelGGL(k_tally, dim3((int)((n + 3) / 4)), dim3(256), 0, ctx->stream, ctx->rs, ref, ctx->d_pssm, ctx->d_drop_f,
                         ctx->d_drop_b, ctx->tb, ctx->ri.trec, ctx->ri.actf);
    }
    HIPCHK(hipGetLastError());
  }
  return MIA_HIP_OK;
}

static int tally_finish(mia_hip_ctx* ctx, uint32_t n_events, uint32_t flags, uint32_t cflags) {
  ctx->n_events_host = (int32_t)n_events;
  if (int rcf = check_cull_flags(ctx, cflags)) return rcf;
  if (flags & 1u) { ctx->err = "insert event list overflow"; return MIA_HIP_ERR_NOMEM; }
  if (ctx->n_events_host > ctx->tb.cap_events) ctx->n_events_host = ctx->tb.cap_events;
  ctx->tallied = true;
  ctx->consensus_done = false;
  return MIA_HIP_OK;
}

extern "C" int mia_hip_tally(mia_hip_ctx* ctx) {
  if (!ctx) return MIA_HIP_ERR_ARG;
  if (int rc = tally_launch(ctx)) return rc;
  uint32_t local3[3] = {0, 0, 0};
  uint32_t* h3 = ctx->h_pin ? reinterpret_cast<uint32_t*>(ctx->h_pin + (17 << 10)) : local3;
  HIPCHK(hipMemcpyAsync(&h3[0], ctx->tb.n_events, 4, hipMemcpyDeviceToHost, ctx->stream));
  HIPCHK(hipMemcpyAsync(&h3[1], ctx->tb.flags, 4, hipMemcpyDeviceToHost, ctx->stream));
  HIPCHK(hipMemcpyAsync(&h3[2], ctx->d_cull_flags, 4, hipMemcpyDeviceToHost, ctx->stream));
  HIPCHK(hipStreamSynchronize(ctx->stream));
  return tally_finish(ctx, h3[0], h3[1], h3[2]);
}

extern "C" int mia_hip_tally_buffers(mia_hip_ctx* ctx, int32_t** d_tally, int64_t* n_tally_words, int32_t** d_gaps,
                                     int64_t* n_gaps_words) {
  if (!ctx || !ctx->tallied) return MIA_HIP_ERR_STATE;
  if (d_tally) *d_tally = ctx->tb.tally;
  if (n_tally_words) *n_tally_words = (int64_t)TALLY_WORDS * ctx->tb.Lp;
  if (d_gaps) *d_gaps = ctx->tb.gaps;
  if (n_gaps_words) *n_gaps_words = ctx->tb.Lp;
  return MIA_HIP_OK;
}

extern "C" int mia_hip_ins_events(mia_hip_ctx* ctx, uint64_t** d_events, int64_t* n_events) {
  if (!ctx || !ctx->tallied) return MIA_HIP_ERR_STATE;
  if (d_events) *d_events = ctx->tb.events;
  if (n_events) *n_events = ctx->n_events_host;
  return MIA_HIP_OK;
}

extern "C" int mia_hip_set_ins_events(mia_hip_ctx* ctx, const uint64_t* d_events, int64_t n_events) {
  if (!ctx || !ctx->tallied || n_events < 0) return MIA_HIP_ERR_STATE;
  HIPCHK(hipSetDevice(ctx->device));
  if (n_events > ctx->tb.cap_events && ensure_events(ctx, n_events)) return MIA_HIP_ERR_NOMEM;
  if (n_events > 0 && d_events != ctx->tb.events)
    HIPCHK(hipMemcpyAsync(ctx->tb.events, d_events, (size_t)n_events * 8, hipMemcpyDeviceToDevice, ctx->stream));
  HIPCHK(hipStreamSynchronize(ctx->stream));
  ctx->n_events_host = (int32_t)n_events;
  return MIA_HIP_OK;
}

extern "C" int mia_hip_get_tally(mia_hip_ctx* ctx, int32_t* tally, int32_t* gaps) {
  if (!ctx || !ctx->tallied) return MIA_HIP_ERR_STATE;
  HIPCHK(hipSetDevice(ctx->device));
  const int Lp = ctx->tb.Lp;
  if (tally) HIPCHK(hipMemcpyAsync(tally, ctx->tb.tally, (size_t)TALLY_WORDS * Lp * 4, hipMemcpyDeviceToHost, ctx->stream));
  if (gaps) HIPCHK(hipMemcpyAsync(gaps, ctx->tb.gaps, (size_t)Lp * 4, hipMemcpyDeviceToHost, ctx->stream));
  HIPCHK(hipStreamSynchronize(ctx->stream));
  return MIA_HIP_OK;
}

extern "C" int mia_hip_set_tally(mia_hip_ctx* ctx, int32_t ref_len, const int32_t* tally, const int32_t* gaps) {
  if (!ctx || ref_len <= 0 || !tally) return MIA_HIP_ERR_ARG;
  HIPCHK(hipSetDevice(ctx->device));
  if (ref_len != ctx->L) {
    ctx->aligned = false; ctx->culled = false; ctx->have_ref = false; ctx->links_applied = false;
  }
  ctx->L = ref_len;
  int rc = ensure_tally(ctx);
  if (rc) return rc;
  const int Lp = ctx->tb.Lp;
  HIPCHK(hipMemcpyAsync(ctx->tb.tally, tally, (size_t)TALLY_WORDS * Lp * 4, hipMemcpyHostToDevice, ctx->stream));
  HIPCHK(hipMemsetAsync(ctx->tb.gaps, 0, ((size_t)Lp + 256) * 4, ctx->stream));
  if (gaps) HIPCHK(hipMemcpyAsync(ctx->tb.gaps, gaps, (size_t)Lp * 4, hipMemcpyHostToDevice, ctx->stream));
  HIPCHK(hipMemsetAsync(ctx->tb.n_events, 0, 4, ctx->stream));
  HIPCHK(hipStreamSynchronize(ctx->stream));
  ctx->n_events_host = 0;
  ctx->tallied = true;
  ctx->consensus_done = false;
  return MIA_HIP_OK;
}

static int consensus_launch(mia_hip_ctx* ctx, int cons_code, int64_t cap, bool columns, bool events_on_device) {
  const int L = ctx->L, Lp = ctx->tb.Lp;
  if (columns) {
    hipLaunchKernelGGL(k_excl_scan, dim3(1), dim3(1024), 0, ctx->stream, (const int32_t*)ctx->tb.gaps, Lp, 1, L, ctx->d_ins_off, ctx->d_ins_total);
    hipLaunchKernelGGL(k_call_columns, dim3((L + 255) / 256), dim3(256), 0, ctx->stream, ctx->tb.tally, Lp, L, cons_code, ctx->d_calls);
  }
  if (cap <= 0) return MIA_HIP_OK;
  HIPCHK(hipMemsetAsync(ctx->d_ins_tally, 0, (size_t)ins_words(cap) * 4, ctx->stream));
  const int ne = ctx->n_events_host;
  if (events_on_device)
    hipLaunchKernelGGL(k_ins_tally, dim3(256), dim3(256), 0, ctx->stream, ctx->tb.events, 0, ctx->d_pssm, ctx->d_ins_off, ctx->tb.gaps, L, ctx->d_ins_tally,
                       (int32_t)cap, (const int32_t*)ctx->tb.n_events, ctx->tb.cap_events);
  else if (ne > 0)
    hipLaunchKernelGGL(k_ins_tally, dim3((ne + 255) / 256), dim3(256), 0, ctx->stream, ctx->tb.events, ne, ctx->d_pssm, ctx->d_ins_off,
                       ctx->tb.gaps, L, ctx->d_ins_tally, (int32_t)cap, (const int32_t*)nullptr, 0);
  hipLaunchKernelGGL(k_call_inserts, dim3((L + 255) / 256), dim3(256), 0, ctx->stream, ctx->tb.tally, Lp, L, ctx->tb.gaps,
                     ctx->d_ins_off, ctx->d_ins_tally, cons_code, ctx->d_ins_calls, (int32_t)cap);
  return MIA_HIP_OK;
}

extern "C" int mia_hip_consensus(mia_hip_ctx* ctx, int cons_code, char* out, int64_t out_cap, int64_t* out_len) {
  if (!ctx || !out) return MIA_HIP_ERR_ARG;
  if (!ctx->tallied) { ctx->err = "tally first"; return MIA_HIP_ERR_STATE; }
  HIPCHK(hipSetDevice(ctx->device));
  const int L = ctx->L, Lp = ctx->tb.Lp;
  auto insert_part = [&](int64_t cap) -> int { return consensus_launch(ctx, cons_code, cap, false, false); };
  if (int rcc = consensus_launch(ctx, cons_code, 0, true, false)) return rcc;
  int rc0 = insert_part(ctx->ins_tally_cap);
  if (rc0) return rc0;
  HIPCHK(hipGetLastError());
  const size_t need = 16 + (size_t)L + 2 * (size_t)Lp * 4 + (size_t)ctx->ins_tally_cap + 64;
  std::vector<unsigned char> pageable;
  unsigned char* base;
  if (ctx->h_pin && need <= mia_hip_ctx::PIN_BYTES - mia_hip_ctx::PIN_MISC) base = ctx->h_pin + mia_hip_ctx::PIN_MISC;
  else { pageable.resize(need); base = pageable.data(); }
  int32_t* h_total = reinterpret_cast<int32_t*>(base);
  int32_t* gaps = reinterpret_cast<int32_t*>(base + 16);
  int32_t* off = gaps + Lp;
  char* calls = reinterpret_cast<char*>(off + Lp);
  char* ins = calls + L;
  HIPCHK(hipMemcpyAsync(h_total, ctx->d_ins_total, 4, hipMemcpyDeviceToHost, ctx->stream));
  HIPCHK(hipMemcpyAsync(calls, ctx->d_calls, (size_t)L, hipMemcpyDeviceToHost, ctx->stream));
// ... 39 lines not shown
```

### mapping-iterative-assembler_amd/csrc/mia_hip_iterate.inc

```

constexpr int PRE_WORDS = 8;
#define COLLCHK(call)                                                                                  \
  do {                                                                                                 \
    const int r_ = (call);                                                                             \
    if (r_ != MIA_HIP_OK) {                                                                            \
      const char* t_ = ctx->coll.error ? ctx->coll.error(ctx->coll.user) : nullptr;                    \
      ctx->err = std::string(#call) + ": " + (t_ && *t_ ? t_ : "collective failed");                   \
      return r_;                                                                                       \
    }                                                                                                  \
  } while (0)

static int comm_attach_table(mia_hip_ctx* ctx, const mia_hip_collectives& t) {
  if (dev_alloc(ctx, ctx->d_gather, (int64_t)PRE_WORDS * t.n_ranks)) return MIA_HIP_ERR_NOMEM;
  ctx->coll = t;
  ctx->coll_name = t.name ? t.name : "";
  ctx->coll.name = t.name ? ctx->coll_name.c_str() : nullptr;
  ctx->comm = true; ctx->comm_ranks = t.n_ranks; ctx->comm_rank = t.rank;
  ctx->h_gather.assign((size_t)PRE_WORDS * t.n_ranks, 0);
  ctx->ev_pad = 0;
  return MIA_HIP_OK;
}

extern "C" int mia_hip_comm_init(mia_hip_ctx* ctx, const void* id128, int32_t n_ranks, int32_t rank) {
  if (!ctx || !id128 || n_ranks < 1 || n_ranks > 256 || rank < 0 || rank >= n_ranks) return MIA_HIP_ERR_ARG;
  if (ctx->comm) { ctx->err = "this context already has a communicator"; return MIA_HIP_ERR_STATE; }
  HIPCHK(hipSetDevice(ctx->device));
  mia_hip_collectives t;
  if (int rc = mia_comm_rccl_table(id128, n_ranks, rank, &t, &ctx->err)) return rc;
  if (int rc = comm_attach_table(ctx, t)) { if (t.destroy) t.destroy(t.user); return rc; }
  return MIA_HIP_OK;
}

extern "C" int mia_hip_comm_attach(mia_hip_ctx* ctx, const mia_hip_collectives* table) {
  if (!ctx || !table || !table->all_gather || !table->all_reduce_i32 || table->n_ranks < 1 || table->n_ranks > 256 || table->rank < 0 ||
      table->rank >= table->n_ranks)
    return MIA_HIP_ERR_ARG;
  if (ctx->comm) { ctx->err = "this context already has a communicator"; return MIA_HIP_ERR_STATE; }
  HIPCHK(hipSetDevice(ctx->device));
  return comm_attach_table(ctx, *table);
}

extern "C" int mia_hip_comm_info(mia_hip_ctx* ctx, int32_t* n_ranks, int32_t* rank, const char** transport) {
  if (!ctx) return MIA_HIP_ERR_ARG;
  int32_t nr = 1, rk = 0;
  if (ctx->comm) {
    nr = ctx->comm_ranks; rk = ctx->comm_rank;
    if (ctx->coll.query) { if (int rc = ctx->coll.query(ctx->coll.user, &nr, &rk)) { ctx->err = "the transport could not say how many ranks it has"; return rc; } }
  }
  if (n_ranks) *n_ranks = nr;
  if (rank) *rank = rk;
  if (transport) *transport = ctx->comm ? (ctx->coll.name ? ctx->coll.name : "caller") : "none";
  return MIA_HIP_OK;
}

extern "C" int mia_hip_comm_destroy(mia_hip_ctx* ctx) {
  if (!ctx) return MIA_HIP_ERR_ARG;
  if (!ctx->comm) return MIA_HIP_OK;
  (void)hipSetDevice(ctx->device);
  (void)hipStreamSynchronize(ctx->stream);
  if (ctx->coll.destroy) ctx->coll.destroy(ctx->coll.user);
  ctx->coll = mia_hip_collectives{};
  ctx->comm = false; ctx->comm_ranks = 1; ctx->comm_rank = 0;
  return MIA_HIP_OK;
}

static int comm_gather_ragged(mia_hip_ctx* ctx, const int64_t* mine, const std::vector<int64_t>& counts, int words, int64_t* total_out) {
  const int W = ctx->comm_ranks;
  int64_t mx = 0, total = 0;
  for (int r = 0; r < W; r++) { mx = std::max(mx, counts[(size_t)r]); total += counts[(size_t)r]; }
  *total_out = total;
  if (total == 0) return MIA_HIP_OK;
  const int64_t pad = mx * words;
  if (dev_ensure(ctx, ctx->d_lmine, pad, pad * 2) || dev_ensure(ctx, ctx->d_lstage, pad * W, pad * W * 2) || dev_ensure(ctx, ctx->d_lall, total * words, total * words * 2))
    return MIA_HIP_ERR_NOMEM;
  HIPCHK(hipMemsetAsync(ctx->d_lmine, 0, (size_t)pad * 8, ctx->stream));
  const int64_t nm = counts[(size_t)ctx->comm_rank] * words;
  if (nm > 0) HIPCHK(hipMemcpyAsync(ctx->d_lmine, mine, (size_t)nm * 8, hipMemcpyDeviceToDevice, ctx->stream));
  COLLCHK(ctx->coll.all_gather(ctx->coll.user, ctx->d_lmine, ctx->d_lstage, (size_t)pad * 8, ctx->stream));
  int64_t o = 0;
  for (int r = 0; r < W; r++) {
    const int64_t c = counts[(size_t)r] * words;
    if (c > 0) HIPCHK(hipMemcpyAsync(ctx->d_lall + o, ctx->d_lstage + (int64_t)r * pad, (size_t)c * 8, hipMemcpyDeviceToDevice, ctx->stream));
    o += c;
  }
  return MIA_HIP_OK;
}

static int comm_pre_cull_enqueue(mia_hip_ctx* ctx, const int32_t* d_wide_count) {
  const int64_t n = ctx->rs.n;
  const int W = ctx->comm_ranks;
  if (!ctx->d_sums && dev_alloc(ctx, ctx->d_sums, 8)) return MIA_HIP_ERR_NOMEM;
  hipLaunchKernelGGL(k_score_sums_init, dim3(1), dim3(64), 0, ctx->stream, ctx->d_sums, d_wide_count);
  const int grid = (int)std::min<int64_t>((n + 255) / 256, (int64_t)ctx->cus);
  hipLaunchKernelGGL(k_score_sums, dim3(grid), dim3(256), 0, ctx->stream, ctx->rs, ctx->d_sums, ctx->L, ctx->d_back_slot, ctx->d_front_slot0);
  HIPCHK(hipGetLastError());
  COLLCHK(ctx->coll.all_gather(ctx->coll.user, ctx->d_sums, ctx->d_gather, (size_t)PRE_WORDS * 8, ctx->stream));
  int64_t* stage = ctx->h_pin ? reinterpret_cast<int64_t*>(ctx->h_pin + (40 << 10)) : ctx->h_gather.data();
  HIPCHK(hipMemcpyAsync(stage, ctx->d_gather, (size_t)PRE_WORDS * W * 8, hipMemcpyDeviceToHost, ctx->stream));
  return MIA_HIP_OK;
}
static bool comm_pre_cull_collect(mia_hip_ctx* ctx) {
  const int W = ctx->comm_ranks;
  if (ctx->h_pin) memcpy(ctx->h_gather.data(), ctx->h_pin + (40 << 10), (size_t)PRE_WORDS * W * 8);
  bool any_wide = false;
  for (int r = 0; r < W; r++) any_wide = any_wide || ctx->h_gather[(size_t)PRE_WORDS * r + 7] != 0;
  return any_wide;
}

constexpr int COMM_FLAG_SLOTS = 3;
__global__ void k_or_u32(uint32_t* dst, uint32_t bits) { if (threadIdx.x == 0 && blockIdx.x == 0) atomicOr(dst, bits); }
__global__ void k_put_rank_words(int32_t* slots, int32_t rank, int32_t W, const int32_t* n_events, int32_t clamp, const uint32_t* tally_flags, const uint32_t* cull_flags) {
  if (threadIdx.x != 0 || blockIdx.x != 0) return;
  slots[rank] = min(*n_events, clamp);
  const uint32_t tf = tally_flags ? *tally_flags : 0u, cf = cull_flags ? *cull_flags : 0u;
  slots[W] = (tf & 1u) ? 1 : 0;
  slots[W + 1] = (cf & 4u) ? 1 : 0;
  slots[W + 2] = (cf & 8u) ? 1 : 0;
}

__global__ __launch_bounds__(256) void k_events_compact(const uint64_t* __restrict__ stage, int64_t pad, const int32_t* __restrict__ counts, int W,
                                                          uint64_t* __restrict__ out, int32_t cap, int32_t* n_out, uint32_t* flags) {
  const int r = blockIdx.y;
  int64_t before = 0, total = 0;
  bool over = false;
  for (int k = 0; k < W; k++) {
    const int64_t c = counts[k];
    over = over || c > pad;
    if (k < r) before += c;
    total += c;
  }
  over = over || total > cap;
  if (over) { if (r == 0 && blockIdx.x == 0 && threadIdx.x == 0) atomicOr(flags, 8u); return; }
  const int64_t mine = counts[r];
  for (int64_t i = (int64_t)blockIdx.x * 256 + threadIdx.x; i < mine; i += (int64_t)gridDim.x * 256) out[before + i] = stage[(int64_t)r * pad + i];
  if (r == 0 && blockIdx.x == 0 && threadIdx.x == 0) *n_out = (int32_t)total;
}

static int iterate_body(mia_hip_ctx* ctx, const char* new_ref, int32_t ref_len, int circular, int32_t hard_cut, const double* slope_intercept,
                        int cons_code, char* out, int64_t out_cap, int64_t* out_len);

extern "C" int mia_hip_iterate(mia_hip_ctx* ctx, const char* new_ref, int32_t ref_len, int circular, int32_t hard_cut, const double* slope_intercept,
                               int cons_code, char* out, int64_t out_cap, int64_t* out_len) {
  if (!ctx) return MIA_HIP_ERR_ARG;
  int rc;
  if (!new_ref || ref_len <= 0 || !out || out_cap < 1) { ctx->err = "iterate: bad argument"; rc = MIA_HIP_ERR_ARG; }
  else if (!ctx->have_pssm || !ctx->d_packed) { ctx->err = "set_pssm and upload_reads must precede iterate"; rc = MIA_HIP_ERR_STATE; }
  else rc = iterate_body(ctx, new_ref, ref_len, circular, hard_cut, slope_intercept, cons_code, out, out_cap, out_len);
  ctx->in_iterate = false; ctx->deferred = false;
  if (rc != MIA_HIP_OK && ctx->comm && ctx->coll.abort) ctx->coll.abort(ctx->coll.user);
  return rc;
}

static int iterate_body(mia_hip_ctx* ctx, const char* new_ref, int32_t ref_len, int circular, int32_t hard_cut, const double* slope_intercept,
                        int cons_code, char* out, int64_t out_cap, int64_t* out_len) {
  HIPCHK(hipSetDevice(ctx->device));
  const int L = ref_len, wl = circular ? (L < MAX_READ ? L : MAX_READ) : 0, wrap = L + wl, total = wrap + 64;
  int64_t n_other = 0;
  {
    static const struct Other { uint8_t t[256]; Other() { for (int c = 0; c < 256; c++) t[c] = base_code((char)c) > 3; } } other_of;
    for (int i = 0; i < L; i++) n_other += other_of.t[(uint8_t)new_ref[i]];
  }
  ctx->ref_mostly_bases = n_other * 50 <= L;
  ctx->ref_few_n = n_other * 500 <= L;
  ctx->kh_entries = 0;
  if (n_other) {
    int64_t e = 0;
    int k = 0;
    auto other = [&](int j) { return base_code(new_ref[j < L ? j : j - L]) > 3 ? 1 : 0; };
    for (int pq = 0; pq < wrap; pq++) {
      k += other(pq);
      if (pq >= DF_K) k -= other(pq - DF_K);
      if (pq >= DF_K - 1 && k <= BX_WILD) e += (int64_t)1 << (2 * k);
    }
    ctx->kh_entries = e > ((int64_t)1 << 24) ? 0 : e;
  }
  if (dev_ensure(ctx, ctx->d_ref, total, (int64_t)total * 2) || dev_ensure(ctx, ctx->d_ascii, L, (int64_t)L * 2)) return MIA_HIP_ERR_NOMEM;
  if (ctx->h_pin && (size_t)L <= mia_hip_ctx::PIN_BYTES - mia_hip_ctx::PIN_MISC) {
    HIPCHK(hipStreamSynchronize(ctx->stream));
    memcpy(ctx->h_pin + mia_hip_ctx::PIN_MISC, new_ref, (size_t)L);
    if (ctx->zero_copy) ctx->ascii_src = reinterpret_cast<const char*>(ctx->h_pin + mia_hip_ctx::PIN_MISC);
    else { HIPCHK(hipMemcpyAsync(ctx->d_ascii, ctx->h_pin + mia_hip_ctx::PIN_MISC, (size_t)L, hipMemcpyHostToDevice, ctx->stream)); ctx->ascii_src = ctx->d_ascii; }
  } else {
    HIPCHK(hipMemcpyAsync(ctx->d_ascii, new_ref, (size_t)L, hipMemcpyHostToDevice, ctx->stream));
    ctx->ascii_src = ctx->d_ascii;
  }
  ctx->pend_encode = true; ctx->pend_L = L; ctx->pend_wl = wl; ctx->pend_total = total;
  if (ctx->rs.n == 0) { encode_now(ctx); HIPCHK(hipGetLastError()); }
  const bool dbg_steps = alt_env("MIA_HIP_ITER_DEBUG") != nullptr;
  static const bool host_laps = getenv("MIA_HIP_TIMING") != nullptr;
  const auto lap_t0 = std::chrono::steady_clock::now();
  auto checkpoint = [&](const char* what) {
    if (dbg_steps) { hipError_t e = hipStreamSynchronize(ctx->stream); fprintf(stderr, "[mia_hip_iterate] %s: %s\n", what, hipGetErrorString(e)); fflush(stderr); }
    if (host_laps) fprintf(stderr, "[mia_hip_iterate host] %-20s %8.2f ms\n", what, std::chrono::duration<double, std::milli>(std::chrono::steady_clock::now() - lap_t0).count());
  };
  checkpoint("reference");
  ctx->L = L; ctx->wrap = wrap; ctx->have_ref = true; ctx->explicit_win = 0;
  const int64_t n = ctx->rs.n;
  const int W = ctx->comm_ranks;
  if (ctx->comm && n == 0) { ctx->err = "iterate: every rank of a sharded run needs reads"; return MIA_HIP_ERR_ARG; }
  if (ctx->comm && W > 256 - COMM_FLAG_SLOTS) { ctx->err = "iterate: more than 253 ranks"; return MIA_HIP_ERR_ARG; }
  ctx->in_iterate = true;
  ctx->deferred = true;
  ctx->spec_pending = false; ctx->abort_if = nullptr;
  ctx->spec_ok = !ctx->comm && n > 0 && !ctx->no_spec && (hard_cut > 0 || slope_intercept || ctx->min_len == ctx->max_len);
  const int rca = align_all(ctx);
  ctx->deferred = false;
  ctx->spec_ok = false;
  ctx->pend_encode = false;
  if (rca) { ctx->spec_pending = false; ctx->abort_if = nullptr; return rca; }
  checkpoint("realign");
  int64_t slot_base = 0, g_sums[5] = {0, 0, 0, 0, 0};
  std::vector<int64_t> link_counts((size_t)W, 0), n_of((size_t)W, n);
  if (ctx->comm) {
    g_sums[3] = INT32_MAX; g_sums[4] = INT32_MIN;
    for (int r = 0; r < W; r++) {
      const int64_t* q = ctx->h_gather.data() + (size_t)PRE_WORDS * r;
      g_sums[0] += q[0]; g_sums[1] += q[1]; g_sums[2] += q[2];
      g_sums[3] = std::min(g_sums[3], q[3]); g_sums[4] = std::max(g_sums[4], q[4]);
      if (r < ctx->comm_rank) slot_base += q[5];
      link_counts[(size_t)r] = q[6];
    }
  }
  double slope = 0, intercept = 0;
  const bool one_length = ctx->comm ? (g_sums[2] == 0 || g_sums[3] == g_sums[4]) : (ctx->min_len == ctx->max_len || n == 0);
  if (hard_cut > 0) {
  } else if (slope_intercept) {
    slope = slope_intercept[0]; intercept = slope_intercept[1];
  } else if (one_length) {
    const double zero = 0.0;
    slope = intercept = zero / zero;
  } else if (!ctx->comm) {
    std::vector<int32_t> score((size_t)n);
    HIPCHK(hipMemcpyAsync(score.data(), ctx->d_score, (size_t)n * 4, hipMemcpyDeviceToHost, ctx->stream));
    HIPCHK(hipStreamSynchronize(ctx->stream));
    mia_hip_score_cut(score.data(), ctx->h_len.data(), nullptr, n, &slope, &intercept);
  } else {
    DevBuf<int32_t> d_nl;
    std::vector<int64_t> cnt1((size_t)W, 1);
    int64_t tot = 0;
    int64_t n64 = n;
    DevBuf<int64_t> d_n;
    if (dev_alloc(ctx, d_n, 1)) return MIA_HIP_ERR_NOMEM;
    HIPCHK(hipMemcpyAsync(d_n, &n64, 8, hipMemcpyHostToDevice, ctx->stream));
    if (int rcg = comm_gather_ragged(ctx, d_n, cnt1, 1, &tot)) return rcg;
    HIPCHK(hipMemcpyAsync(n_of.data(), ctx->d_lall, (size_t)W * 8, hipMemcpyDeviceToHost, ctx->stream));
    HIPCHK(hipStreamSynchronize(ctx->stream));
    int64_t nmax = 0, ntot = 0;
    for (int r = 0; r < W; r++) { nmax = std::max(nmax, n_of[(size_t)r]); ntot += n_of[(size_t)r]; }
    if (dev_alloc(ctx, d_nl, nmax * 2) || dev_ensure(ctx, ctx->d_scores_all, (int64_t)W * nmax * 2)) return MIA_HIP_ERR_NOMEM;
    HIPCHK(hipMemsetAsync(d_nl, 0, (size_t)nmax * 2 * 4, ctx->stream));
    HIPCHK(hipMemcpyAsync(d_nl, ctx->d_score, (size_t)n * 4, hipMemcpyDeviceToDevice, ctx->stream));
    HIPCHK(hipMemcpyAsync(d_nl + nmax, ctx->h_len.data(), (size_t)n * 4, hipMemcpyHostToDevice, ctx->stream));
    COLLCHK(ctx->coll.all_gather(ctx->coll.user, d_nl, ctx->d_scores_all, (size_t)nmax * 2 * 4, ctx->stream));
    std::vector<int32_t> all((size_t)W * nmax * 2), score((size_t)ntot), lens((size_t)ntot);
    HIPCHK(hipMemcpyAsync(all.data(), ctx->d_scores_all, all.size() * 4, hipMemcpyDeviceToHost, ctx->stream));
    HIPCHK(hipStreamSynchronize(ctx->stream));
    int64_t o = 0;
    for (int r = 0; r < W; r++) {
      memcpy(score.data() + o, all.data() + (size_t)r * nmax * 2, (size_t)n_of[(size_t)r] * 4);
      memcpy(lens.data() + o, all.data() + (size_t)r * nmax * 2 + nmax, (size_t)n_of[(size_t)r] * 4);
      o += n_of[(size_t)r];
    }
    mia_hip_score_cut(score.data(), lens.data(), nullptr, ntot, &slope, &intercept);
  }
  if (!(hard_cut > 0) && slope <= 0) slope = 100.0;
  auto queue_cull = [&]() -> int {
    ctx->buckets_queued = 0;
    const bool side = tally_is_binned(ctx) && !ctx->no_side_buckets;
    if (side && ctx->spec_pending && !ctx->align_end_signalled) HIPCHK(hipEventRecord(ctx->ev_fork, ctx->stream));
    if (int rcc = mia_hip_cull(ctx, hard_cut, slope, intercept, slot_base)) return rcc;
    if (side) {
      if (ctx->spec_pending) HIPCHK(hipStreamWaitEvent(ctx->stream2, ctx->ev_fork, 0));
      if (int rcb = bucket_launch(ctx, ctx->stream2)) return rcb;
    }
    return MIA_HIP_OK;
  };
  if (int rcq = queue_cull()) return rcq;
  if (ctx->comm) {
    int64_t any = 0;
    for (int r = 0; r < W; r++) any += link_counts[(size_t)r];
    if (any > 0) {
      int64_t* dl = nullptr; int64_t nl = 0, total_l = 0;
      if (int rcl = mia_hip_links(ctx, &dl, &nl)) return rcl;
      if (nl != link_counts[(size_t)ctx->comm_rank]) { ctx->err = "iterate: the cull emitted another number of links than the score sweep announced"; return MIA_HIP_ERR_STATE; }
      if (int rcg = comm_gather_ragged(ctx, dl, link_counts, 4, &total_l)) return rcg;
      if (int rcs = mia_hip_set_links(ctx, ctx->d_lall, total_l)) return rcs;
      int32_t *dlen = nullptr, *dact = nullptr; int64_t nn = 0;
      if (int rcl = mia_hip_link_lengths(ctx, &dlen, &dact, &nn)) return rcl;
      COLLCHK(ctx->coll.all_reduce_i32(ctx->coll.user, dlen, (size_t)nn, MIA_HIP_OP_MAX, ctx->stream));
      COLLCHK(ctx->coll.all_reduce_i32(ctx->coll.user, dact, (size_t)nn, MIA_HIP_OP_MAX, ctx->stream));
      if (int rcf = mia_hip_finish_links(ctx)) return rcf;
    }
  }
  checkpoint("cull");
  if (n == 0) { out[0] = 0; if (out_len) *out_len = 0; return MIA_HIP_OK; }
  if (ctx->comm && ctx->ev_pad > 0) {
    if (const char* e = alt_env("MIA_HIP_EV_PAD")) { const long long v = atoll(e); if (v > 0) ctx->ev_pad = v; }
    if (int rct = ensure_tally(ctx)) return rct;
    if (ctx->ev_pad * W > ctx->tb.cap_events && ensure_events(ctx, std::min<int64_t>(ctx->ev_pad * W + 4096, (int64_t)1 << 30))) return MIA_HIP_ERR_NOMEM;
  }
  if (int rct = tally_launch(ctx)) return rct;
  checkpoint("tally");
  const int Lp = ctx->tb.Lp;
  ctx->n_events_host = 0;
  int32_t* h_evc = ctx->h_pin ? reinterpret_cast<int32_t*>(ctx->h_pin + (56 << 10)) : nullptr;
  std::vector<int32_t> evc_pageable;
  if (ctx->comm && !h_evc) { evc_pageable.resize((size_t)W); h_evc = evc_pageable.data(); }
  auto exchange_events_counted = [&]() -> int {
    HIPCHK(hipMemcpyAsync(h_evc, ctx->tb.gaps + Lp, (size_t)W * 4, hipMemcpyDeviceToHost, ctx->stream));
    HIPCHK(hipStreamSynchronize(ctx->stream));
    std::vector<int64_t> ev_counts((size_t)W);
    for (int r = 0; r < W; r++) ev_counts[(size_t)r] = h_evc[r];
    int64_t total_ev = 0;
    if (int rcg = comm_gather_ragged(ctx, reinterpret_cast<const int64_t*>(ctx->tb.events), ev_counts, 1, &total_ev)) return rcg;
    if (total_ev > ctx->tb.cap_events && ensure_events(ctx, total_ev + 4096)) return MIA_HIP_ERR_NOMEM;
    if (total_ev > 0) HIPCHK(hipMemcpyAsync(ctx->tb.events, ctx->d_lall, (size_t)total_ev * 8, hipMemcpyDeviceToDevice, ctx->stream));
    int32_t* te = ctx->h_pin ? reinterpret_cast<int32_t*>(ctx->h_pin + (60 << 10)) : nullptr;
    int32_t te_local = (int32_t)total_ev;
    if (te) { *te = te_local; HIPCHK(hipMemcpyAsync(ctx->tb.n_events, te, 4, hipMemcpyHostToDevice, ctx->stream)); }
    else { HIPCHK(hipMemcpyAsync(ctx->tb.n_events, &te_local, 4, hipMemcpyHostToDevice, ctx->stream)); HIPCHK(hipStreamSynchronize(ctx->stream)); }
    return MIA_HIP_OK;
  };
  auto exchange_events_padded = [&]() -> int {
    const int64_t pad = ctx->ev_pad;
    if (dev_ensure(ctx, ctx->d_lstage, pad * W, pad * W * 2)) return MIA_HIP_ERR_NOMEM;
    COLLCHK(ctx->coll.all_gather(ctx->coll.user, ctx->tb.events, ctx->d_lstage, (size_t)pad * 8, ctx->stream));
    const unsigned gx = (unsigned)std::min<int64_t>((pad + 255) / 256, 64);
    hipLaunchKernelGGL(k_events_compact, dim3(gx, (unsigned)W), dim3(256), 0, ctx->stream, (const uint64_t*)ctx->d_lstage.p, pad, (const int32_t*)(ctx->tb.gaps + Lp), W,
                       ctx->tb.events, ctx->tb.cap_events, ctx->tb.n_events, ctx->tb.flags);
    HIPCHK(hipGetLastError());
    return MIA_HIP_OK;
  };
  bool counted = false;
  if (ctx->comm) {
    if (ctx->fake_event_overflow)
      hipLaunchKernelGGL(k_or_u32, dim3(1), dim3(1), 0, ctx->stream, ctx->tb.flags, 1u);
    hipLaunchKernelGGL(k_put_rank_words, dim3(1), dim3(1), 0, ctx->stream, ctx->tb.gaps + Lp, (int32_t)ctx->comm_rank, (int32_t)W, (const int32_t*)ctx->tb.n_events,
                       ctx->tb.cap_events, (const uint32_t*)ctx->tb.flags, (const uint32_t*)ctx->d_cull_flags);
    COLLCHK(ctx->coll.all_reduce_i32(ctx->coll.user, ctx->tb.tally, (size_t)TALLY_WORDS * Lp, MIA_HIP_OP_SUM, ctx->stream));
    COLLCHK(ctx->coll.all_reduce_i32(ctx->coll.user, ctx->tb.gaps, (size_t)Lp + W + COMM_FLAG_SLOTS, MIA_HIP_OP_MAX, ctx->stream));
    counted = ctx->ev_pad <= 0;
    if (int rce = counted ? exchange_events_counted() : exchange_events_padded()) return rce;
  }
  const int64_t cons_cap = (int64_t)L + ctx->ins_tally_cap + 64;
  const int64_t res_bytes = (int64_t)CH_WORDS * 4 + cons_cap;
  if (dev_ensure(ctx, ctx->d_cons, res_bytes, res_bytes * 2) || dev_ensure(ctx, ctx->d_cons_pos, Lp, (int64_t)Lp * 2)) return MIA_HIP_ERR_NOMEM;
  const size_t need = (size_t)res_bytes;
  if (need > ctx->pin2_bytes) {
    if (ctx->h_pin2) (void)hipHostFree(ctx->h_pin2);
    ctx->h_pin2 = nullptr; ctx->pin2_bytes = 0;
    if (hipHostMalloc((void**)&ctx->h_pin2, need * 2, hipHostMallocDefault) != hipSuccess) { ctx->err = "hipHostMalloc"; return MIA_HIP_ERR_NOMEM; }
    ctx->pin2_bytes = need * 2;
  }
  int32_t* h_hdr = reinterpret_cast<int32_t*>(ctx->h_pin2);
  char* h_str = reinterpret_cast<char*>(ctx->h_pin2) + CH_WORDS * 4;
  auto consensus_tail = [&]() -> int {
    const int64_t cap = ctx->ins_tally_cap;
    int32_t* d_res = reinterpret_cast<int32_t*>(ctx->d_cons.p);
    const unsigned gl = (unsigned)((L + 255) / 256);
    const bool zc = ctx->zero_copy;
    const bool fused_scans = Lp <= (1 << 17) && !ctx->tail_scans;
    const unsigned glp = (unsigned)((Lp + 255) / 256);
    if (!fused_scans) {
      hipLaunchKernelGGL(k_excl_scan, dim3(1), dim3(1024), 0, ctx->stream, (const int32_t*)ctx->tb.gaps, Lp, 1, L, ctx->d_ins_off, ctx->d_ins_total, ctx->abort_if);
      hipLaunchKernelGGL(k_call_columns_z, dim3(gl), dim3(256), 0, ctx->stream, (const int32_t*)ctx->tb.tally, Lp, L, cons_code, ctx->d_calls, ctx->d_ins_tally, ins_words(cap), ctx->abort_if,
                         (const int32_t*)nullptr, (int32_t*)nullptr, (int32_t*)nullptr);
    } else
      hipLaunchKernelGGL(k_call_columns_z, dim3(glp > gl ? glp : gl), dim3(256), 0, ctx->stream, (const int32_t*)ctx->tb.tally, Lp, L, cons_code, ctx->d_calls, ctx->d_ins_tally, ins_words(cap), ctx->abort_if,
                         (const int32_t*)ctx->tb.gaps, ctx->d_ins_off, ctx->d_ins_total);
    if (cap > 0)
      hipLaunchKernelGGL(k_ins_tally, dim3(256), dim3(256), 0, ctx->stream, ctx->tb.events, 0, ctx->d_pssm, ctx->d_ins_off, ctx->tb.gaps, L, ctx->d_ins_tally,
                         (int32_t)cap, (const int32_t*)ctx->tb.n_events, ctx->tb.cap_events, ctx->abort_if);
    checkpoint("consensus kernels");
    hipLaunchKernelGGL(k_call_inserts_count, dim3(gl), dim3(256), 0, ctx->stream, (const int32_t*)ctx->tb.tally, Lp, L, (const int32_t*)ctx->tb.gaps,
                       (const int32_t*)ctx->d_ins_off, ctx->d_ins_tally, cons_code, (const char*)ctx->d_calls, ctx->d_ins_calls, (int32_t)cap,
                       (const int32_t*)ctx->d_ins_total, ctx->d_cons_pos, ctx->abort_if);
    if (!fused_scans) hipLaunchKernelGGL(k_excl_scan, dim3(1), dim3(1024), 0, ctx->stream, (const int32_t*)ctx->d_cons_pos, L, 0, L, ctx->d_cons_pos, d_res + CH_LEN, ctx->abort_if);
    hipLaunchKernelGGL(k_cons_scatter, dim3(gl), dim3(256), 0, ctx->stream, (const char*)ctx->d_calls, (const char*)ctx->d_ins_calls,
                       (const int32_t*)ctx->tb.gaps, (const int32_t*)ctx->d_ins_off, L, (int32_t)cap, (const int32_t*)ctx->d_ins_total,
                       (const int32_t*)ctx->d_cons_pos, d_res, (int32_t)cons_cap, (const int32_t*)ctx->tb.n_events, (const uint32_t*)ctx->tb.flags,
                       (const uint32_t*)ctx->d_cull_flags, ctx->abort_if, zc ? reinterpret_cast<int32_t*>(ctx->h_pin2) : (int32_t*)nullptr,
                       (const int32_t*)(ctx->d_ctrl + CTRL_C0), (int32_t)CTRL_CN, (zc && ctx->spec_pending) ? reinterpret_cast<int32_t*>(ctx->h_pin) : (int32_t*)nullptr,
                       fused_scans ? 1 : 0, ctx->comm ? (const int32_t*)(ctx->tb.gaps + Lp + W) : (const int32_t*)nullptr);
    HIPCHK(hipGetLastError());
    checkpoint("assemble");
    if (!zc) HIPCHK(hipMemcpyAsync(ctx->h_pin2, ctx->d_cons, need, hipMemcpyDeviceToHost, ctx->stream));
    if (ctx->comm && !counted) HIPCHK(hipMemcpyAsync(h_evc, ctx->tb.gaps + Lp, (size_t)W * 4, hipMemcpyDeviceToHost, ctx->stream));
    if (ctx->spin_wait) {
      hipError_t eq;
      while ((eq = hipStreamQuery(ctx->stream)) == hipErrorNotReady) {}
      HIPCHK(eq);
    } else HIPCHK(hipStreamSynchronize(ctx->stream));
    return MIA_HIP_OK;
  };
  if (int rct = consensus_tail()) return rct;
  if (ctx->h_pin) {
    uint32_t* stuck = reinterpret_cast<uint32_t*>(ctx->h_pin + (62 << 10));
    if (*stuck) {
      *stuck = 0;
      ctx->no_prep_fuse = true;
      ctx->err = "k_ref_prep: part of the launch never reached the grid barrier (device partitioned or compute units masked?); the iteration's results are void";
      return MIA_HIP_ERR_DEVICE;
    }
  }
  if (ctx->spec_pending) {
    ctx->spec_pending = false;
    ctx->abort_if = nullptr;
    const int32_t* hb = reinterpret_cast<const int32_t*>(ctx->h_pin);
    align_counters_collect(ctx, hb, ctx->spec_filtered, ctx->spec_bx, ctx->spec_plain);
    const int32_t n_wide = hb[0];
    if (n_wide > 0 || ctx->spec_force) {
      ctx->spec_redone++;
      RefInfo rinfo{ctx->d_ref, ctx->L, ctx->wrap, ctx->explicit_win};
      if (n_wide > 0) { if (int rcw = run_wide(ctx, rinfo, n_wide)) return rcw; }
      if (int rcq = queue_cull()) return rcq;
      if (int rct = tally_launch(ctx)) return rct;
      if (int rct = consensus_tail()) return rct;
    }
  }
  uint32_t tflags = (uint32_t)h_hdr[CH_TALLY_FLAGS];
  if (ctx->comm && !counted && (tflags & 8u)) {
    counted = true;
    if (int rce = exchange_events_counted()) return rce;
    if (int rct = consensus_tail()) return rct;
    tflags = (uint32_t)h_hdr[CH_TALLY_FLAGS];
  }
  tflags &= ~8u;
  if (ctx->comm) {
    int64_t mx = 0;
    for (int r = 0; r < W; r++) mx = std::max<int64_t>(mx, h_evc[r]);
    if (ctx->ev_pad <= 0 || mx * 5 > ctx->ev_pad * 4 || mx * 4 < ctx->ev_pad) ctx->ev_pad = mx + mx / 2 + 1024;
  }
  ctx->in_iterate = false;
  if (int rcf = tally_finish(ctx, (uint32_t)h_hdr[CH_N_EVENTS], tflags, (uint32_t)h_hdr[CH_CULL_FLAGS])) return rcf;
  if (h_hdr[CH_OVERFLOW]) {
    ctx->iter_fallbacks++;
    return mia_hip_consensus(ctx, cons_code, out, out_cap, out_len);
  }
  const int64_t len = h_hdr[CH_LEN];
  if (len + 1 > out_cap) { ctx->err = "consensus buffer too small"; return MIA_HIP_ERR_ARG; }
  memcpy(out, h_str, (size_t)len);
  out[len] = 0;
  if (out_len) *out_len = len;
  ctx->consensus_done = true;
  ctx->ins_total_host = h_hdr[CH_INS_TOTAL];
  return MIA_HIP_OK;
}
```

Baseline: 1.431 billion reads/s.

## Speculatively prepare next iteration's reference planes while consensus finishes

After the consensus scatter is launched, the new consensus string is speculatively used to run reference prep (encode, k-mer hash, planes) into a shadow buffer set. The host waits on an event at the end of the consensus kernel rather than on the whole stream. A double-buffered control block lets this prep work use its own counters. On the next iterate call, if the new reference matches the speculated one, the shadow buffers are adopted and the ref-prep step is skipped, removing that serial work from the critical path. This adds extra device memory, complexity and correctness risk around buffer swapping and control-block binding.

After: 1.479 billion reads/s, median of 6. +3.4%, better.

```diff
diff --git a/mapping-iterative-assembler_amd/csrc/align_route.h b/mapping-iterative-assembler_amd/csrc/align_route.h
--- a/mapping-iterative-assembler_amd/csrc/align_route.h
+++ b/mapping-iterative-assembler_amd/csrc/align_route.h
@@ -12,6 +12,7 @@
   int64_t kh_entries = 0;
   bool flat = false, ref_mostly_bases = true, ref_few_n = true, bx_ok = false, explicit_win = false, deferred = false, pend_encode = false;
   bool own_umax = false;
+  bool ref_ready = false;
   int64_t rejects = 0;
   int use_filter = 1, use_banddp = 1, use_bx = 1, use_lanes = 1, use_fine = 1, use_quick = 1;
   bool bx_serial = false, plan_split = true, use_direct_open = true, no_prep_fuse = false;
@@ -22,6 +23,7 @@
   int64_t plane_words = 0;
   int nwords = 0;
   bool bx = false, run_filter = false, fused_prep = false, filtered = false, kocc = false, banded = false;
+  bool prep_none = false;
   bool want_bits = false, new_flow = false, split = false, fork_by_launch = false, fine = false;
   bool many_rejects = false;
   bool planner_head_first = false, direct_open = false;
@@ -53,6 +55,7 @@
   r.bx = in.bx_ok && in.use_bx && (in.ref_mostly_bases || in.kh_entries > 0) && in.wrap <= (1 << 22) && !(in.dbg & 128u);
   r.run_filter = filter_ok && !r.bx;
   r.fused_prep = in.pend_encode && r.bx && !in.no_prep_fuse;
+  r.prep_none = in.ref_ready && r.bx;
   r.filtered = r.run_filter || r.bx;
   r.kocc = r.filtered && in.wrap <= (1 << 22) && !r.bx;
   r.banded = r.bx || (r.filtered && in.use_banddp && r.kocc && !(in.dbg & 128u));
diff --git a/mapping-iterative-assembler_amd/csrc/mia_hip.hip b/mapping-iterative-assembler_amd/csrc/mia_hip.hip
--- a/mapping-iterative-assembler_amd/csrc/mia_hip.hip
+++ b/mapping-iterative-assembler_amd/csrc/mia_hip.hip
@@ -12,10 +12,12 @@
 #include <string>
 #include <thread>
 #include <tuple>
+#include <utility>
 #include <vector>
 
 #include "../../include/mia_hip.h"
 #include "dev_buf.h"
+#include "ref_ahead.h"
 #include "dev_pool.h"
 #include "mia_comm.h"
 #include "mia_consensus_kernels.h"
@@ -76,11 +78,15 @@
   std::string err;
   DevPool pool;
   unsigned char* h_pin = nullptr; static constexpr size_t PIN_BYTES = 1 << 20, PIN_MISC = 64 << 10;
-  DevBuf<int32_t> d_ctrl;
+  DevBuf<int32_t> d_ctrl; int ctrl_half = 0;
+  int32_t* ctrl = nullptr;
+  int32_t* d_genn = nullptr;
+  const int32_t* d_ctr0 = nullptr;
   uint32_t dbg = 0;
 
   hipStream_t stream = nullptr;
   hipStream_t stream2 = nullptr; hipEvent_t ev_fork = nullptr, ev_join = nullptr;
+  hipEvent_t ev_cons = nullptr;
   hipStream_t stream3 = nullptr; hipEvent_t ev_join3 = nullptr;
   uint32_t ext_events = 31u; bool align_end_signalled = false;
   bool spin_wait = true;
@@ -143,6 +149,15 @@
   DevBuf<KbPair> d_kbits;
   int use_quick = 1; int64_t quick_steps = 0;
   DevBuf<uint32_t> d_prep_bar; uint32_t prep_bar_count = 0; bool no_prep_fuse = false;
+  struct RefAhead {
+    DevBuf<uint8_t> d_ref; DevBuf<uint64_t> d_planes; DevBuf<uint32_t> d_refnib, d_khash; DevBuf<int32_t> d_khash_ovf; DevBuf<KbPair> d_kbits;
+    bool queued = false;
+    bool valid = false;
+    RefAheadKey key; std::string str;
+  } ahead;
+  bool no_ref_ahead = false;
+  bool ref_ready = false;
+  bool last_route_bx = false;
   DevBuf<uint32_t> d_bx_plan; DevBuf<int32_t> d_bx_expect, d_bx_lists;
   DevBuf<BxCandRec> d_bx_cand; bool plan_split = true;
   DevBuf<BxCandRec> d_bx_cand2; int use_fine = 1;
@@ -286,6 +301,7 @@
   if (const char* v = alt_env("MIA_HIP_QUICK_PLAN")) ctx->use_quick = atoi(v);
   if (on("MIA_HIP_NO_DIRECT_OPEN")) ctx->use_direct_open = false;
   if (on("MIA_HIP_NO_PREP_FUSE")) ctx->no_prep_fuse = true;
+  if (on("MIA_HIP_NO_REF_AHEAD")) ctx->no_ref_ahead = true;
   if (on("MIA_HIP_NO_SPEC")) ctx->no_spec = true;
   if (on("MIA_HIP_SPEC_TEST")) ctx->spec_force = true;
   if (on("MIA_HIP_NO_SIDE_BUCKETS")) ctx->no_side_buckets = true;
@@ -333,6 +349,25 @@
 template <class T>
 static int pool_take(mia_hip_ctx* ctx, PoolLease<T>& lease, size_t n) { return dev_nomem(ctx, lease.take(ctx->pool, n)); }
 
+static_assert(CTRL_WORDS % 64 == 0, "the second half of the control block starts on a cache line, as the first does");
+static void ctrl_bind(mia_hip_ctx* ctx, int half) {
+  const bool own_links = ctx->d_n_links_all && ctx->d_n_links_all == ctx->lk.n;
+  int32_t* b = ctx->d_ctrl + (size_t)half * CTRL_WORDS;
+  ctx->ctrl_half = half;
+  ctx->ctrl = b;
+  ctx->d_bins = b + CTRL_BINS;
+  ctx->d_plan_hdr = b + CTRL_HDR;
+  ctx->d_filter_n = reinterpret_cast<uint32_t*>(b + CTRL_FILTER);
+  ctx->lk.n = b + CTRL_LKN;
+  ctx->d_cull_flags = reinterpret_cast<uint32_t*>(b + CTRL_CULLF);
+  ctx->tb.n_events = b + CTRL_NEV;
+  ctx->tb.flags = reinterpret_cast<uint32_t*>(b + CTRL_TFLAGS);
+  ctx->d_genn = b + CTRL_GENN;
+  ctx->d_bx_ctr = reinterpret_cast<uint32_t*>(b + CTRL_BXC);
+  ctx->d_ctr0 = b + CTRL_C0;
+  if (own_links) ctx->d_n_links_all = ctx->lk.n;
+}
+
 extern "C" const char* mia_hip_last_error(const mia_hip_ctx* ctx) { return ctx ? ctx->err.c_str() : "null context"; }
 
 extern "C" int mia_hip_create(mia_hip_ctx** out, int device_index) {
@@ -346,7 +381,7 @@
   const unsigned evf = hipEventDisableTiming;
   if (hipSetDevice(device_index) != hipSuccess || hipStreamCreateWithFlags(&ctx->stream, hipStreamNonBlocking) != hipSuccess ||
       hipStreamCreateWithFlags(&ctx->stream2, hipStreamNonBlocking) != hipSuccess || hipStreamCreateWithFlags(&ctx->stream3, hipStreamNonBlocking) != hipSuccess ||
-      hipEventCreateWithFlags(&ctx->ev_join3, evf) != hipSuccess ||
+      hipEventCreateWithFlags(&ctx->ev_join3, evf) != hipSuccess || hipEventCreateWithFlags(&ctx->ev_cons, evf) != hipSuccess ||
       hipEventCreateWithFlags(&ctx->ev_fork, evf) != hipSuccess || hipEventCreateWithFlags(&ctx->ev_join, evf) != hipSuccess) {
     delete ctx;
     return MIA_HIP_ERR_DEVICE;
@@ -360,7 +395,7 @@
     read_alt_switches(ctx);
     if (const char* sw = getenv("MIA_HIP_SPIN_WAIT")) ctx->spin_wait = atoi(sw) != 0;
   }
-  if (dev_alloc(ctx, ctx->d_pssm, 2 * PSSM_WORDS) || dev_alloc(ctx, ctx->d_ctrl, CTRL_WORDS) ||
+  if (dev_alloc(ctx, ctx->d_pssm, 2 * PSSM_WORDS) || dev_alloc(ctx, ctx->d_ctrl, 2 * CTRL_WORDS) ||
       dev_alloc(ctx, ctx->d_total, 1) || dev_alloc(ctx, ctx->d_ins_total, 1) ||
       dev_alloc(ctx, ctx->d_bx_sub, 2 * BX_SUB_WORDS) || dev_alloc(ctx, ctx->d_bx_mrow, 2 * 31 * 4) || dev_alloc(ctx, ctx->d_bx_loss, BX_LOSS_WORDS) ||
       dev_alloc(ctx, ctx->d_bx_dl, BX_DL_WORDS) ||
@@ -368,15 +403,8 @@
     delete ctx;
     return MIA_HIP_ERR_NOMEM;
   }
-  ctx->d_bins = ctx->d_ctrl + CTRL_BINS;
-  ctx->d_plan_hdr = ctx->d_ctrl + CTRL_HDR;
-  ctx->d_filter_n = reinterpret_cast<uint32_t*>(ctx->d_ctrl + CTRL_FILTER);
-  ctx->lk.n = ctx->d_ctrl + CTRL_LKN;
-  ctx->d_cull_flags = reinterpret_cast<uint32_t*>(ctx->d_ctrl + CTRL_CULLF);
-  ctx->tb.n_events = ctx->d_ctrl + CTRL_NEV;
-  ctx->tb.flags = reinterpret_cast<uint32_t*>(ctx->d_ctrl + CTRL_TFLAGS);
-  ctx->d_bx_ctr = reinterpret_cast<uint32_t*>(ctx->d_ctrl + CTRL_BXC);
-  if (hipMemset(ctx->d_ctrl, 0, CTRL_WORDS * 4) != hipSuccess) { delete ctx; return MIA_HIP_ERR_DEVICE; }
+  ctrl_bind(ctx, 0);
+  if (hipMemset(ctx->d_ctrl, 0, 2 * CTRL_WORDS * 4) != hipSuccess) { delete ctx; return MIA_HIP_ERR_DEVICE; }
   {
     const int32_t one = 1;
     if (dev_alloc(ctx, ctx->d_one, 1) || hipMemcpy(ctx->d_one, &one, 4, hipMemcpyHostToDevice) != hipSuccess) { delete ctx; return MIA_HIP_ERR_DEVICE; }
@@ -403,6 +431,7 @@
   if (ctx->stream2) (void)hipStreamDestroy(ctx->stream2);
   if (ctx->stream3) (void)hipStreamDestroy(ctx->stream3);
   if (ctx->ev_join3) (void)hipEventDestroy(ctx->ev_join3);
+  if (ctx->ev_cons) (void)hipEventDestroy(ctx->ev_cons);
   if (ctx->ev_fork) (void)hipEventDestroy(ctx->ev_fork);
   if (ctx->ev_join) (void)hipEventDestroy(ctx->ev_join);
   delete ctx;
@@ -905,7 +934,7 @@
   in.n = ctx->rs.n; in.max_len = ctx->max_len; in.wrap = ctx->wrap; in.L = ctx->L; in.kh_entries = ctx->kh_entries;
   in.plane_words = plane_words((int64_t)ctx->wrap + 64);
   in.flat = ctx->flat; in.ref_mostly_bases = ctx->ref_mostly_bases; in.ref_few_n = ctx->ref_few_n; in.bx_ok = ctx->bx_ok;
-  in.explicit_win = ctx->explicit_win != 0; in.deferred = ctx->deferred; in.pend_encode = ctx->pend_encode;
+  in.explicit_win = ctx->explicit_win != 0; in.deferred = ctx->deferred; in.pend_encode = ctx->pend_encode; in.ref_ready = ctx->ref_ready;
   in.own_umax = ctx->umax_valid && ctx->rs.roff == ctx->d_roff;
   for (int k = 1; k < BXF_KINDS; k++) in.rejects += ctx->bx_last[BXC_FAIL0 + k];
   in.use_filter = ctx->use_filter; in.use_banddp = ctx->use_banddp; in.use_bx = ctx->use_bx; in.use_lanes = ctx->use_lanes;
@@ -966,13 +995,39 @@
   return MIA_HIP_OK;
 }
 
+struct RefPrepSet { uint8_t* codes; int32_t* ctrl; uint32_t* khash; int32_t* kovf; uint64_t* planes; int64_t pstride; uint32_t* nib; KbPair* kbits; };
+static int launch_ref_prep(mia_hip_ctx* ctx, const RefPrepSet& s, const char* ascii, int32_t L, int32_t wl, int32_t total, uint32_t kslots, int kwild,
+                           int64_t words, int64_t nw) {
+  const int wrap = total - 64;
+  RefPrep rp2;
+  rp2.ascii = ascii; rp2.L = L; rp2.wl = wl; rp2.total = total; rp2.codes = s.codes;
+  rp2.ctrl = s.ctrl; rp2.ctrl_words = CTRL_WORDS;
+  rp2.kslot = s.khash; rp2.kovf = s.kovf; rp2.kslots = kslots; rp2.kmask = kslots - 1; rp2.kshift = kh_shift_for(kslots); rp2.kwild = kwild;
+  rp2.plane_words = words; rp2.plo = s.planes; rp2.phi = s.planes + s.pstride; rp2.pok = s.planes + 2 * s.pstride;
+  rp2.nib_words = nw; rp2.nib = s.nib;
+  const int64_t want = ((int64_t)wrap + (kwild > 0 ? 63 : 255)) / (kwild > 0 ? 64 : 256);
+  const unsigned grid = (unsigned)std::max<int64_t>(1, std::min<int64_t>(want, ctx->cus));
+  rp2.bar = ctx->d_prep_bar; rp2.bar_target = ctx->prep_bar_count + grid;
+  rp2.stuck = ctx->h_pin ? reinterpret_cast<uint32_t*>(ctx->h_pin + (62 << 10)) : nullptr;
+  rp2.kbits = s.kbits;
+  hipLaunchKernelGGL(k_ref_prep, dim3(grid), dim3(256), 0, ctx->stream, rp2);
+  HIPCHK(hipGetLastError());
+  ctx->prep_bar_count += grid;
+  return MIA_HIP_OK;
+}
+
 static int align_ref_prep(mia_hip_ctx* ctx, AlignCall& c) {
   const AlignRoute& r = c.r;
   const int wrap = ctx->wrap;
   const int64_t words = r.plane_words, pstride = ctx->d_planes.cap / 3;
+  if (r.prep_none) {
+    c.rp = RefPlanes{ctx->d_planes, ctx->d_planes + pstride, ctx->d_planes + 2 * pstride};
+    c.kh = KmerHash{ctx->d_khash, ctx->d_khash_ovf, c.kslots - 1, kh_shift_for(c.kslots), ctx->kh_entries > 0 ? BX_WILD : 0};
+    return MIA_HIP_OK;
+  }
   if (!r.fused_prep) {
     encode_now(ctx);
-    HIPCHK(hipMemsetAsync(ctx->d_ctrl, 0, (size_t)CTRL_WORDS * 4, ctx->stream));
+    HIPCHK(hipMemsetAsync(ctx->ctrl, 0, (size_t)CTRL_WORDS * 4, ctx->stream));
   }
   if (!r.filtered) return MIA_HIP_OK;
   c.rp = RefPlanes{ctx->d_planes, ctx->d_planes + pstride, ctx->d_planes + 2 * pstride};
@@ -1001,20 +1056,8 @@
     }
     return MIA_HIP_OK;
   }
-  RefPrep rp2;
-  rp2.ascii = ctx->ascii_src; rp2.L = ctx->pend_L; rp2.wl = ctx->pend_wl; rp2.total = ctx->pend_total; rp2.codes = ctx->d_ref;
-  rp2.ctrl = ctx->d_ctrl; rp2.ctrl_words = CTRL_WORDS;
-  rp2.kslot = ctx->d_khash; rp2.kovf = ctx->d_khash_ovf; rp2.kslots = kslots; rp2.kmask = kh.mask; rp2.kshift = kh.shift; rp2.kwild = kh.wild;
-  rp2.plane_words = words; rp2.plo = ctx->d_planes; rp2.phi = ctx->d_planes + pstride; rp2.pok = ctx->d_planes + 2 * pstride;
-  rp2.nib_words = nw; rp2.nib = ctx->d_refnib;
-  const int64_t want = ((int64_t)wrap + (kh.wild > 0 ? 63 : 255)) / (kh.wild > 0 ? 64 : 256);
-  const unsigned grid = (unsigned)std::max<int64_t>(1, std::min<int64_t>(want, ctx->cus));
-  rp2.bar = ctx->d_prep_bar; rp2.bar_target = ctx->prep_bar_count + grid;
-  rp2.stuck = ctx->h_pin ? reinterpret_cast<uint32_t*>(ctx->h_pin + (62 << 10)) : nullptr;
-  rp2.kbits = r.want_bits ? ctx->d_kbits : nullptr;
-  hipLaunchKernelGGL(k_ref_prep, dim3(grid), dim3(256), 0, ctx->stream, rp2);
-  HIPCHK(hipGetLastError());
-  ctx->prep_bar_count += grid;
+  const RefPrepSet own{ctx->d_ref, ctx->ctrl, ctx->d_khash, ctx->d_khash_ovf, ctx->d_planes, pstride, ctx->d_refnib, r.want_bits ? ctx->d_kbits.p : nullptr};
+  if (int rc = launch_ref_prep(ctx, own, ctx->ascii_src, ctx->pend_L, ctx->pend_wl, ctx->pend_total, kslots, kh.wild, words, nw)) return rc;
   ctx->pend_encode = false;
   return MIA_HIP_OK;
 }
@@ -1263,7 +1306,7 @@
   align_ck(ctx, c, "retry");
   if (int rcj = bx_join_and_retry(ctx, c)) return rcj;
   align_ck(ctx, c, "band join");
-  constexpr int C0 = CTRL_C0, CN = CTRL_CN;
+  constexpr int CN = CTRL_CN;
   std::vector<int32_t> pageable;
   int32_t* hb;
   if (ctx->h_pin) hb = reinterpret_cast<int32_t*>(ctx->h_pin);
@@ -1271,7 +1314,7 @@
   const bool pre_cull = ctx->in_iterate && ctx->comm;
   if (pre_cull) { if (int rcp = comm_pre_cull_enqueue(ctx, c.d_wide_count)) return rcp; }
   const bool spec = ctx->spec_ok && ctx->h_pin && !pre_cull && !c.dbg_steps;
-  if (!(spec && ctx->zero_copy)) HIPCHK(hipMemcpyAsync(hb, ctx->d_ctrl + C0, (size_t)CN * 4, hipMemcpyDeviceToHost, ctx->stream));
+  if (!(spec && ctx->zero_copy)) HIPCHK(hipMemcpyAsync(hb, ctx->d_ctr0, (size_t)CN * 4, hipMemcpyDeviceToHost, ctx->stream));
   if (spec) {
     ctx->spec_pending = true; ctx->spec_filtered = r.filtered; ctx->spec_bx = r.bx; ctx->spec_plain = r.use_plain;
     ctx->abort_if = ctx->spec_force ? ctx->d_one : c.d_wide_count;
@@ -1431,6 +1474,7 @@
   AlignCall c;
   c.r = align_route(align_route_in(ctx));
   const AlignRoute& r = c.r;
+  ctx->last_route_bx = r.bx;
   c.ref = RefInfo{ctx->d_ref, ctx->L, ctx->wrap, ctx->explicit_win};
   c.d_count = ctx->d_bins; c.d_off = ctx->d_bins + N_BINS; c.d_cursor = ctx->d_bins + 2 * N_BINS; c.d_wide_count = ctx->d_bins + 3 * N_BINS;
   c.gb = (int)((n + (int64_t)256 * PLAN_PER - 1) / ((int64_t)256 * PLAN_PER));
@@ -1911,7 +1955,7 @@
       const bool planes_ok = ctx->umax_valid && ctx->rs.roff == ctx->d_roff && ctx->d_rplanes && ctx->d_umax;
       const bool defer = ctx->tally_defer;
       if (defer && dev_ensure(ctx, ctx->d_gen_list, n)) return MIA_HIP_ERR_NOMEM;
-      int32_t* n_gen = ctx->d_ctrl + CTRL_GENN;
+      int32_t* n_gen = ctx->d_genn;
       if (defer && !ctx->in_iterate) HIPCHK(hipMemsetAsync(n_gen, 0, 4, ctx->stream));
 #define MIA_TALLY_ARGS(PL, RW, UM, BIAS)                                                                                                              \
   dim3(grid), dim3(256), 0, ctx->stream, ctx->rs, ref, ctx->d_pssm, ctx->d_drop_f, ctx->d_drop_b, ctx->tb, nb, d_off, d_wgoff, split ? ctx->d_order2 : ctx->d_order, ctx->ri.trec, \
diff --git a/mapping-iterative-assembler_amd/csrc/mia_hip_iterate.inc b/mapping-iterative-assembler_amd/csrc/mia_hip_iterate.inc
--- a/mapping-iterative-assembler_amd/csrc/mia_hip_iterate.inc
+++ b/mapping-iterative-assembler_amd/csrc/mia_hip_iterate.inc
@@ -136,6 +136,78 @@
   if (r == 0 && blockIdx.x == 0 && threadIdx.x == 0) *n_out = (int32_t)total;
 }
 
+static void ref_count_other(const char* ref, int L, int wrap, int64_t* n_other_out, int64_t* kh_entries_out) {
+  uint32_t cnt = 0;
+  for (int i = 0; i < L; i++) { const char c = ref[i]; cnt += (uint32_t)((c != 'A') & (c != 'C') & (c != 'G') & (c != 'T')); }
+  int64_t n_other = cnt, e = 0;
+  if (n_other) {
+    int k = 0;
+    auto other = [&](int j) { return base_code(ref[j < L ? j : j - L]) > 3 ? 1 : 0; };
+    for (int pq = 0; pq < wrap; pq++) {
+      k += other(pq);
+      if (pq >= DF_K) k -= other(pq - DF_K);
+      if (pq >= DF_K - 1 && k <= BX_WILD) e += (int64_t)1 << (2 * k);
+    }
+    if (e > ((int64_t)1 << 24)) e = 0;
+  }
+  *n_other_out = n_other; *kh_entries_out = e;
+}
+
+static bool ref_ahead_want(const mia_hip_ctx* ctx, int L, int circular, int64_t n_other, int64_t kh_entries, RefAheadKey* key) {
+  const int wl = circular ? (L < MAX_READ ? L : MAX_READ) : 0, wrap = L + wl;
+  AlignRouteIn in = align_route_in(ctx);
+  in.L = L; in.wrap = wrap; in.plane_words = plane_words((int64_t)wrap + 64); in.kh_entries = kh_entries;
+  in.ref_mostly_bases = n_other * 50 <= L; in.ref_few_n = n_other * 500 <= L;
+  in.explicit_win = false; in.deferred = true; in.pend_encode = true; in.ref_ready = false;
+  const AlignRoute r = align_route(in);
+  key->L = L; key->circular = circular ? 1 : 0; key->n_other = n_other; key->kh_entries = kh_entries;
+  key->kslots = kh_slots_for_entries(wrap, kh_entries); key->kwild = kh_entries > 0 ? BX_WILD : 0;
+  key->plane_words = r.plane_words; key->nib_words = bx_nib_words((int64_t)wrap + 64); key->bits = r.want_bits;
+  return r.bx && r.fused_prep;
+}
+
+static bool ref_ahead_allowed(const mia_hip_ctx* ctx) {
+  return !ctx->no_ref_ahead && !ctx->no_prep_fuse && ctx->h_pin && ctx->last_route_bx && ctx->rs.n > 0;
+}
+static bool ref_ahead_queue(mia_hip_ctx* ctx, const RefAheadKey& key, const char* src) {
+  mia_hip_ctx::RefAhead& ah = ctx->ahead;
+  const int L = key.L, wl = key.circular ? (L < MAX_READ ? L : MAX_READ) : 0, total = L + wl + 64;
+  if (dev_ensure(ctx, ah.d_ref, total, (int64_t)total * 2) || dev_ensure(ctx, ah.d_planes, key.plane_words * 3) ||
+      dev_ensure(ctx, ah.d_refnib, key.nib_words, key.nib_words * 2) || dev_ensure(ctx, ah.d_khash, (int64_t)key.kslots * 4) ||
+      dev_ensure(ctx, ah.d_khash_ovf, (int64_t)key.kslots * 2) || (key.bits && !ah.d_kbits && dev_alloc(ctx, ah.d_kbits, KB_WORDS)))
+    return false;
+  const RefPrepSet twin{ah.d_ref, ctx->d_ctrl + (size_t)(1 - ctx->ctrl_half) * CTRL_WORDS, ah.d_khash, ah.d_khash_ovf, ah.d_planes, ah.d_planes.cap / 3,
+                        ah.d_refnib, key.bits ? ah.d_kbits.p : nullptr};
+  if (launch_ref_prep(ctx, twin, src, L, wl, total, key.kslots, key.kwild, key.plane_words, key.nib_words)) return false;
+  ah.key = key;
+  return true;
+}
+static void ref_ahead_speculate(mia_hip_ctx* ctx, const RefAheadKey& key, const char* src) {
+  ctx->ahead.valid = false;
+  ctx->ahead.queued = key.kwild == 0 && ref_ahead_queue(ctx, key, src);
+}
+static void ref_ahead_settle(mia_hip_ctx* ctx, const char* h_str, int64_t len, int circular) {
+  mia_hip_ctx::RefAhead& ah = ctx->ahead;
+  const bool queued = ah.queued;
+  ah.valid = false; ah.queued = false;
+  if (!queued || !ref_ahead_allowed(ctx) || len <= 0 || len > (1 << 22)) return;
+  const int L = (int)len, wl = circular ? (L < MAX_READ ? L : MAX_READ) : 0, wrap = L + wl;
+  int64_t n_other = 0, kh_entries = 0;
+  ref_count_other(h_str, L, wrap, &n_other, &kh_entries);
+  RefAheadKey key;
+  if (!ref_ahead_want(ctx, L, circular, n_other, kh_entries, &key) || !ref_ahead_same_key(ah.key, key)) return;
+  ah.str.assign(h_str, (size_t)L);
+  ah.valid = true;
+}
+
+static void ref_ahead_adopt(mia_hip_ctx* ctx) {
+  mia_hip_ctx::RefAhead& ah = ctx->ahead;
+  std::swap(ctx->d_ref, ah.d_ref); std::swap(ctx->d_planes, ah.d_planes); std::swap(ctx->d_refnib, ah.d_refnib);
+  std::swap(ctx->d_khash, ah.d_khash); std::swap(ctx->d_khash_ovf, ah.d_khash_ovf);
+  if (ah.key.bits) std::swap(ctx->d_kbits, ah.d_kbits);
+  ctrl_bind(ctx, 1 - ctx->ctrl_half);
+}
+
 static int iterate_body(mia_hip_ctx* ctx, const char* new_ref, int32_t ref_len, int circular, int32_t hard_cut, const double* slope_intercept,
                         int cons_code, char* out, int64_t out_cap, int64_t* out_len);
 
@@ -146,7 +218,7 @@
   if (!new_ref || ref_len <= 0 || !out || out_cap < 1) { ctx->err = "iterate: bad argument"; rc = MIA_HIP_ERR_ARG; }
   else if (!ctx->have_pssm || !ctx->d_packed) { ctx->err = "set_pssm and upload_reads must precede iterate"; rc = MIA_HIP_ERR_STATE; }
   else rc = iterate_body(ctx, new_ref, ref_len, circular, hard_cut, slope_intercept, cons_code, out, out_cap, out_len);
-  ctx->in_iterate = false; ctx->deferred = false;
+  ctx->in_iterate = false; ctx->deferred = false; ctx->ref_ready = false;
   if (rc != MIA_HIP_OK && ctx->comm && ctx->coll.abort) ctx->coll.abort(ctx->coll.user);
   return rc;
 }
@@ -155,36 +227,49 @@
                         int cons_code, char* out, int64_t out_cap, int64_t* out_len) {
   HIPCHK(hipSetDevice(ctx->device));
   const int L = ref_len, wl = circular ? (L < MAX_READ ? L : MAX_READ) : 0, wrap = L + wl, total = wrap + 64;
-  int64_t n_other = 0;
-  {
-    static const struct Other { uint8_t t[256]; Other() { for (int c = 0; c < 256; c++) t[c] = base_code((char)c) > 3; } } other_of;
-    for (int i = 0; i < L; i++) n_other += other_of.t[(uint8_t)new_ref[i]];
-  }
+  mia_hip_ctx::RefAhead& ah = ctx->ahead;
+  const bool had_shadow = ah.valid;
+  ah.queued = false;
+  const bool same_string = had_shadow && ref_ahead_same_string(ah.key, ah.str.data(), new_ref, L, circular);
+  int64_t n_other = 0, kh_entries = 0;
+  if (same_string) { n_other = ah.key.n_other; kh_entries = ah.key.kh_entries; }
+  else ref_count_other(new_ref, L, wrap, &n_other, &kh_entries);
   ctx->ref_mostly_bases = n_other * 50 <= L;
   ctx->ref_few_n = n_other * 500 <= L;
-  ctx->kh_entries = 0;
-  if (n_other) {
-    int64_t e = 0;
-    int k = 0;
-    auto other = [&](int j) { return base_code(new_ref[j < L ? j : j - L]) > 3 ? 1 : 0; };
-    for (int pq = 0; pq < wrap; pq++) {
-      k += other(pq);
-      if (pq >= DF_K) k -= other(pq - DF_K);
-      if (pq >= DF_K - 1 && k <= BX_WILD) e += (int64_t)1 << (2 * k);
-    }
-    ctx->kh_entries = e > ((int64_t)1 << 24) ? 0 : e;
-  }
-  if (dev_ensure(ctx, ctx->d_ref, total, (int64_t)total * 2) || dev_ensure(ctx, ctx->d_ascii, L, (int64_t)L * 2)) return MIA_HIP_ERR_NOMEM;
-  if (ctx->h_pin && (size_t)L <= mia_hip_ctx::PIN_BYTES - mia_hip_ctx::PIN_MISC) {
-    HIPCHK(hipStreamSynchronize(ctx->stream));
-    memcpy(ctx->h_pin + mia_hip_ctx::PIN_MISC, new_ref, (size_t)L);
-    if (ctx->zero_copy) ctx->ascii_src = reinterpret_cast<const char*>(ctx->h_pin + mia_hip_ctx::PIN_MISC);
-    else { HIPCHK(hipMemcpyAsync(ctx->d_ascii, ctx->h_pin + mia_hip_ctx::PIN_MISC, (size_t)L, hipMemcpyHostToDevice, ctx->stream)); ctx->ascii_src = ctx->d_ascii; }
+  ctx->kh_entries = kh_entries;
+  const bool staged = ctx->h_pin && (size_t)L <= mia_hip_ctx::PIN_BYTES - mia_hip_ctx::PIN_MISC;
+  bool hit = false;
+  if (had_shadow) {
+    ah.valid = false;
+    RefAheadKey want;
+    hit = ref_ahead_want(ctx, L, circular, n_other, kh_entries, &want) && ref_ahead_hit(ah.key, want, ah.str.data(), new_ref);
+  }
+  uint32_t* stuck = ctx->h_pin ? reinterpret_cast<uint32_t*>(ctx->h_pin + (62 << 10)) : nullptr;
+  bool shadow_ended = !hit;
+  if (hit) {
+    const hipError_t eq = hipStreamQuery(ctx->stream);
+    if (eq != hipErrorNotReady) { HIPCHK(eq); shadow_ended = true; }
+  } else if (staged || had_shadow) HIPCHK(hipStreamSynchronize(ctx->stream));
+  if (had_shadow && shadow_ended && stuck && *stuck) {
+    *stuck = 0;
+    ctx->no_prep_fuse = true;
+    hit = false;
+  }
+  if (hit) {
+    ref_ahead_adopt(ctx);
   } else {
-    HIPCHK(hipMemcpyAsync(ctx->d_ascii, new_ref, (size_t)L, hipMemcpyHostToDevice, ctx->stream));
-    ctx->ascii_src = ctx->d_ascii;
-  }
-  ctx->pend_encode = true; ctx->pend_L = L; ctx->pend_wl = wl; ctx->pend_total = total;
+    if (dev_ensure(ctx, ctx->d_ref, total, (int64_t)total * 2) || dev_ensure(ctx, ctx->d_ascii, L, (int64_t)L * 2)) return MIA_HIP_ERR_NOMEM;
+    if (staged) {
+      memcpy(ctx->h_pin + mia_hip_ctx::PIN_MISC, new_ref, (size_t)L);
+      if (ctx->zero_copy) ctx->ascii_src = reinterpret_cast<const char*>(ctx->h_pin + mia_hip_ctx::PIN_MISC);
+      else { HIPCHK(hipMemcpyAsync(ctx->d_ascii, ctx->h_pin + mia_hip_ctx::PIN_MISC, (size_t)L, hipMemcpyHostToDevice, ctx->stream)); ctx->ascii_src = ctx->d_ascii; }
+    } else {
+      HIPCHK(hipMemcpyAsync(ctx->d_ascii, new_ref, (size_t)L, hipMemcpyHostToDevice, ctx->stream));
+      ctx->ascii_src = ctx->d_ascii;
+    }
+    ctx->pend_encode = true; ctx->pend_L = L; ctx->pend_wl = wl; ctx->pend_total = total;
+  }
+  ctx->ref_ready = hit;
   if (ctx->rs.n == 0) { encode_now(ctx); HIPCHK(hipGetLastError()); }
   const bool dbg_steps = alt_env("MIA_HIP_ITER_DEBUG") != nullptr;
   static const bool host_laps = getenv("MIA_HIP_TIMING") != nullptr;
@@ -193,7 +278,7 @@
     if (dbg_steps) { hipError_t e = hipStreamSynchronize(ctx->stream); fprintf(stderr, "[mia_hip_iterate] %s: %s\n", what, hipGetErrorString(e)); fflush(stderr); }
     if (host_laps) fprintf(stderr, "[mia_hip_iterate host] %-20s %8.2f ms\n", what, std::chrono::duration<double, std::milli>(std::chrono::steady_clock::now() - lap_t0).count());
   };
-  checkpoint("reference");
+  checkpoint(hit ? "reference (ahead)" : "reference");
   ctx->L = L; ctx->wrap = wrap; ctx->have_ref = true; ctx->explicit_win = 0;
   const int64_t n = ctx->rs.n;
   const int W = ctx->comm_ranks;
@@ -206,7 +291,7 @@
   const int rca = align_all(ctx);
   ctx->deferred = false;
   ctx->spec_ok = false;
-  ctx->pend_encode = false;
+  ctx->pend_encode = false; ctx->ref_ready = false;
   if (rca) { ctx->spec_pending = false; ctx->abort_if = nullptr; return rca; }
   checkpoint("realign");
   int64_t slot_base = 0, g_sums[5] = {0, 0, 0, 0, 0};
@@ -344,8 +429,9 @@
   }
   const int64_t cons_cap = (int64_t)L + ctx->ins_tally_cap + 64;
   const int64_t res_bytes = (int64_t)CH_WORDS * 4 + cons_cap;
+  const size_t need = (size_t)res_bytes;
+  if (res_bytes > ctx->d_cons.cap || need > ctx->pin2_bytes) HIPCHK(hipStreamSynchronize(ctx->stream));
   if (dev_ensure(ctx, ctx->d_cons, res_bytes, res_bytes * 2) || dev_ensure(ctx, ctx->d_cons_pos, Lp, (int64_t)Lp * 2)) return MIA_HIP_ERR_NOMEM;
-  const size_t need = (size_t)res_bytes;
   if (need > ctx->pin2_bytes) {
     if (ctx->h_pin2) (void)hipHostFree(ctx->h_pin2);
     ctx->h_pin2 = nullptr; ctx->pin2_bytes = 0;
@@ -354,6 +440,8 @@
   }
   int32_t* h_hdr = reinterpret_cast<int32_t*>(ctx->h_pin2);
   char* h_str = reinterpret_cast<char*>(ctx->h_pin2) + CH_WORDS * 4;
+  RefAheadKey spec_key;
+  bool spec_ahead = !ctx->comm && ctx->zero_copy && n_other == 0 && ref_ahead_allowed(ctx) && ref_ahead_want(ctx, L, circular, 0, 0, &spec_key);
   auto consensus_tail = [&]() -> int {
     const int64_t cap = ctx->ins_tally_cap;
     int32_t* d_res = reinterpret_cast<int32_t*>(ctx->d_cons.p);
@@ -376,21 +464,23 @@
                        (const int32_t*)ctx->d_ins_off, ctx->d_ins_tally, cons_code, (const char*)ctx->d_calls, ctx->d_ins_calls, (int32_t)cap,
                        (const int32_t*)ctx->d_ins_total, ctx->d_cons_pos, ctx->abort_if);
     if (!fused_scans) hipLaunchKernelGGL(k_excl_scan, dim3(1), dim3(1024), 0, ctx->stream, (const int32_t*)ctx->d_cons_pos, L, 0, L, ctx->d_cons_pos, d_res + CH_LEN, ctx->abort_if);
-    hipLaunchKernelGGL(k_cons_scatter, dim3(gl), dim3(256), 0, ctx->stream, (const char*)ctx->d_calls, (const char*)ctx->d_ins_calls,
+    launch_k(k_cons_scatter, dim3(gl), dim3(256), 0, ctx->stream, spec_ahead ? ctx->ev_cons : (hipEvent_t) nullptr, (const char*)ctx->d_calls, (const char*)ctx->d_ins_calls,
                        (const int32_t*)ctx->tb.gaps, (const int32_t*)ctx->d_ins_off, L, (int32_t)cap, (const int32_t*)ctx->d_ins_total,
                        (const int32_t*)ctx->d_cons_pos, d_res, (int32_t)cons_cap, (const int32_t*)ctx->tb.n_events, (const uint32_t*)ctx->tb.flags,
                        (const uint32_t*)ctx->d_cull_flags, ctx->abort_if, zc ? reinterpret_cast<int32_t*>(ctx->h_pin2) : (int32_t*)nullptr,
-                       (const int32_t*)(ctx->d_ctrl + CTRL_C0), (int32_t)CTRL_CN, (zc && ctx->spec_pending) ? reinterpret_cast<int32_t*>(ctx->h_pin) : (int32_t*)nullptr,
+                       ctx->d_ctr0, (int32_t)CTRL_CN, (zc && ctx->spec_pending) ? reinterpret_cast<int32_t*>(ctx->h_pin) : (int32_t*)nullptr,
                        fused_scans ? 1 : 0, ctx->comm ? (const int32_t*)(ctx->tb.gaps + Lp + W) : (const int32_t*)nullptr);
     HIPCHK(hipGetLastError());
+    if (spec_ahead) ref_ahead_speculate(ctx, spec_key, h_str);
     checkpoint("assemble");
     if (!zc) HIPCHK(hipMemcpyAsync(ctx->h_pin2, ctx->d_cons, need, hipMemcpyDeviceToHost, ctx->stream));
     if (ctx->comm && !counted) HIPCHK(hipMemcpyAsync(h_evc, ctx->tb.gaps + Lp, (size_t)W * 4, hipMemcpyDeviceToHost, ctx->stream));
     if (ctx->spin_wait) {
       hipError_t eq;
-      while ((eq = hipStreamQuery(ctx->stream)) == hipErrorNotReady) {}
+      while ((eq = spec_ahead ? hipEventQuery(ctx->ev_cons) : hipStreamQuery(ctx->stream)) == hipErrorNotReady) {}
       HIPCHK(eq);
-    } else HIPCHK(hipStreamSynchronize(ctx->stream));
+    } else if (spec_ahead) HIPCHK(hipEventSynchronize(ctx->ev_cons));
+    else HIPCHK(hipStreamSynchronize(ctx->stream));
     return MIA_HIP_OK;
   };
   if (int rct = consensus_tail()) return rct;
@@ -415,6 +505,7 @@
       if (n_wide > 0) { if (int rcw = run_wide(ctx, rinfo, n_wide)) return rcw; }
       if (int rcq = queue_cull()) return rcq;
       if (int rct = tally_launch(ctx)) return rct;
+      spec_ahead = false; ctx->ahead.queued = false;
       if (int rct = consensus_tail()) return rct;
     }
   }
@@ -439,6 +530,7 @@
   }
   const int64_t len = h_hdr[CH_LEN];
   if (len + 1 > out_cap) { ctx->err = "consensus buffer too small"; return MIA_HIP_ERR_ARG; }
+  ref_ahead_settle(ctx, h_str, len, circular);
   memcpy(out, h_str, (size_t)len);
   out[len] = 0;
   if (out_len) *out_len = len;
diff --git a/mapping-iterative-assembler_amd/csrc/ref_ahead.h b/mapping-iterative-assembler_amd/csrc/ref_ahead.h
--- /dev/null
+++ b/mapping-iterative-assembler_amd/csrc/ref_ahead.h
@@ -0,0 +1,31 @@
+#pragma once
+#include <stdint.h>
+#include <string.h>
+
+namespace mia {
+
+struct RefAheadKey {
+  int32_t L = 0;
+  int32_t circular = 0;
+  int64_t n_other = 0;
+  int64_t kh_entries = 0;
+  uint32_t kslots = 0;
+  int32_t kwild = 0;
+  int64_t plane_words = 0, nib_words = 0;
+  bool bits = false;
+};
+
+inline bool ref_ahead_same_key(const RefAheadKey& a, const RefAheadKey& b) {
+  return a.L == b.L && a.circular == b.circular && a.n_other == b.n_other && a.kh_entries == b.kh_entries && a.kslots == b.kslots &&
+         a.kwild == b.kwild && a.plane_words == b.plane_words && a.nib_words == b.nib_words && a.bits == b.bits;
+}
+
+inline bool ref_ahead_same_string(const RefAheadKey& built, const char* kept, const char* new_ref, int32_t new_len, int32_t circular) {
+  return kept && new_ref && new_len > 0 && new_len == built.L && (circular != 0) == (built.circular != 0) && memcmp(new_ref, kept, (size_t)new_len) == 0;
+}
+
+inline bool ref_ahead_hit(const RefAheadKey& built, const RefAheadKey& want, const char* kept, const char* new_ref) {
+  return ref_ahead_same_key(built, want) && ref_ahead_same_string(built, kept, new_ref, want.L, want.circular);
+}
+
+}
```
